# vga-group/tauray

Hardware: AMD Instinct MI355X
Metric: Mray/s (closest-hit + shadow rays traced) @1920x1080, 4 bounces, 1 spp (higher is better)
Workload: dtype f32

## Files before the change

### include/trhip.h

```cpp
#ifndef TRHIP_H
#define TRHIP_H
#include <stddef.h>
#include <stdint.h>

#ifdef __cplusplus
extern "C" {
#endif

typedef struct trhip_device trhip_device;
typedef struct trhip_pt trhip_pt;

int trhip_device_create(int hip_device, trhip_device** out);
void trhip_device_destroy(trhip_device* dev);
const char* trhip_last_error(void);
int trhip_malloc(trhip_device* dev, size_t bytes, void** out);
int trhip_free(trhip_device* dev, void* ptr);
int trhip_upload(trhip_device* dev, void* dst_dev, const void* src_host, size_t bytes, void* stream);
int trhip_download(trhip_device* dev, void* dst_host, const void* src_dev, size_t bytes, void* stream);
int trhip_memset(trhip_device* dev, void* dst_dev, int value, size_t bytes, void* stream);
int trhip_sync(trhip_device* dev, void* stream);
int trhip_stream_create(trhip_device* dev, void** stream_out);
int trhip_stream_destroy(trhip_device* dev, void* stream);
int trhip_stream_wait(trhip_device* dev, void* stream, void* on);
int trhip_stream_pipe_class(trhip_device* dev, void* stream, int32_t* pipe_class_out);
// ... 121 lines not shown
    int32_t mis_mode;
    float russian_roulette_delta;
    float indirect_clamping;
    float regularization_gamma;
    int32_t depth_of_field;
    float nee_point, nee_directional, nee_envmap, nee_triangles;
    int32_t bounce_mode;
    int32_t tri_light_mode;
    int32_t hide_lights;
    int32_t use_white_albedo_on_first_bounce;
    int32_t transparent_background;
    int32_t pre_transformed_vertices;
} trhip_pt_options;

typedef struct trhip_distribution {
    uint32_t size_x, size_y;
    int32_t strategy;
    uint32_t index, count;
    uint32_t primary;
} trhip_distribution;

typedef struct trhip_counters {
    uint64_t closest_rays, shadow_rays;
    uint64_t node_visits, tri_tests, alpha_tests, surface_hits;
    uint64_t stack_overflows;
} trhip_counters;

typedef struct trhip_timings {
    float path_tracing_ms;
    float trace_closest_ms, trace_shadow_ms, shade_ms, raygen_ms, resolve_ms;
    uint32_t trace_closest_launches, trace_shadow_launches, shade_launches, frames;
} trhip_timings;

int trhip_pt_create(trhip_device* dev, const trhip_pt_options* opt, trhip_pt** out);
int trhip_direct_create(trhip_device* dev, const trhip_pt_options* opt, trhip_pt** out);
void trhip_pt_destroy(trhip_pt* pt);
int trhip_pt_set_distribution(trhip_pt* pt, const trhip_distribution* dist);
int trhip_pt_reset_accumulation(trhip_pt* pt, int reset_sample_counter);
int trhip_pt_set_frame_counter(trhip_pt* pt, uint32_t frame_counter);
int trhip_pt_set_frame_batch(trhip_pt* pt, uint32_t frames);
int trhip_pt_set_lanes(trhip_pt* pt, int lanes);
int trhip_pt_set_frame_slots(trhip_pt* pt, int slots);
int trhip_pt_get_lane_pipes(trhip_pt* pt, int32_t* lanes_out, int32_t pipe_classes_out[4]);
int trhip_pt_set_shard(trhip_pt* pt, uint32_t viewport_base, uint32_t viewport_stride, uint32_t sample_base, uint32_t sample_stride);
int trhip_pt_render(trhip_pt* pt, void* color_dev, uint32_t target_w, uint32_t target_h, uint32_t viewports, void* stream);
typedef struct trhip_pt_targets {
    void* color;
    void* diffuse;
    void* reflection;
    void* albedo;
    void* material;
    void* normal;
    void* pos;
    void* instance_id;
    void* screen_motion;
} trhip_pt_targets;
int trhip_pt_render_targets(trhip_pt* pt, const trhip_pt_targets* targets, uint32_t target_w, uint32_t target_h, uint32_t viewports, void* stream);
int trhip_pt_set_shading_arithmetic(trhip_pt* pt, int ieee);
int trhip_pt_set_specialization(trhip_pt* pt, int enable);
int trhip_pt_precompile(const trhip_pt_options* opt, int shade_tris, int ieee, int count_work, const char* arch);
typedef struct trhip_program_info { int32_t kind, ieee; uint64_t identity; char key[240]; } trhip_program_info;
int trhip_pt_get_program(trhip_pt* pt, trhip_program_info* out);
uint64_t trhip_build_id(void);
const char* trhip_kernel_cache_dir(void);
int trhip_pt_set_profiling(trhip_pt* pt, int count_work, int detailed_timing);
int trhip_pt_get_counters(trhip_pt* pt, trhip_counters* out);
int trhip_pt_reset_counters(trhip_pt* pt);
int trhip_pt_get_timings(trhip_pt* pt, trhip_timings* out);
typedef struct trhip_phase_counters {
    uint64_t lane_node_phases, lane_tri_phases, quad_node_phases, quad_tri_phases;
    uint64_t lane_node_phases_le16, lane_node_visits_le16;
    uint64_t lane_node_phase_hist[8];
    uint64_t closest_node_visits;
} trhip_phase_counters;
int trhip_pt_get_phase_counters(trhip_pt* pt, trhip_phase_counters* out);
typedef struct trhip_light_counters { uint64_t sphere_tests, node_visits, walk_fallbacks; } trhip_light_counters;
int trhip_pt_get_light_counters(trhip_pt* pt, trhip_light_counters* out);
int trhip_pt_get_max_stack_depth(trhip_pt* pt, uint32_t* out);
#define TRHIP_TERMINAL_QUERY_AUTO 0
#define TRHIP_TERMINAL_QUERY_OFF 1
int trhip_pt_set_terminal_query(trhip_pt* pt, int mode);
typedef struct trhip_terminal_counters { uint64_t blocked_rays, fallback_rays; uint32_t in_effect, emitter_triangles, threshold, pad; } trhip_terminal_counters;
int trhip_pt_get_terminal_counters(trhip_pt* pt, trhip_terminal_counters* out);
int trhip_calibrate_valu(trhip_device* dev, float* ginst_per_s);
int trhip_calibrate_l1(trhip_device* dev, float* gaccesses_per_s);

int trhip_feature_render(trhip_device* dev, int feature, const trhip_distribution* dist, int projection,
                         uint32_t viewport, float min_ray_dist, const float default_value[4],
                         void* color_dev, uint32_t target_w, uint32_t target_h, void* stream);

int trhip_trace_closest(trhip_device* dev, uint32_t n, const void* rays_dev, const void* seeds_dev,
                        int include_lights, void* hits_dev, void* stream);
int trhip_trace_terminal(trhip_device* dev, uint32_t n, const void* rays_dev, const void* seeds_dev, const void* fallback_dev,
                         void* hits_dev, void* stream);
int trhip_trace_shadow(trhip_device* dev, uint32_t n, const void* rays_dev, void* visibility_dev, void* stream);

int trhip_stitch(trhip_device* dev, const trhip_distribution* partial_dist, const void* partial_dev,
                 uint32_t partial_w, uint32_t partial_h, void* primary_dev, uint32_t viewports,
                 float blend_ratio, void* stream);
int trhip_stitch_batch(trhip_device* dev, uint32_t count, const trhip_distribution* partial_dists, const void* const* partials_dev,
                       const uint32_t* partial_ws, const uint32_t* partial_hs, void* primary_dev, uint32_t viewports,
                       float blend_ratio, void* stream);

typedef struct trhip_tonemap_info {
    int32_t op;
    float exposure, gamma;
    int32_t alpha_grid_background;
} trhip_tonemap_info;
int trhip_tonemap(trhip_device* dev, const void* in_dev, void* out_dev, uint32_t width, uint32_t height,
                  uint32_t layers, const trhip_tonemap_info* info, void* stream);
int trhip_pt_set_fused_tonemap(trhip_pt* pt, void* display_dev, const trhip_tonemap_info* info);

typedef struct trhip_bmfr trhip_bmfr;
#define TRHIP_BMFR_DIFFUSE_ONLY 0
#define TRHIP_BMFR_DIFFUSE_SPECULAR 1
typedef struct trhip_bmfr_options {
    int32_t settings;
    float noise_amount;
} trhip_bmfr_options;
typedef struct trhip_bmfr_features {
    void* color;
    void* diffuse;
    void* albedo;
    void* normal;
    void* pos;
    void* screen_motion;
    void* instance_id;
} trhip_bmfr_features;
typedef struct trhip_bmfr_timings {
    float preprocess_ms, fit_ms, weighted_sum_ms, accumulate_output_ms, total_ms;
    uint32_t frames;
} trhip_bmfr_timings;
int trhip_bmfr_create(trhip_device* dev, const trhip_bmfr_options* opt, uint32_t width, uint32_t height, uint32_t layers, trhip_bmfr** out);
void trhip_bmfr_destroy(trhip_bmfr* bmfr);
int trhip_bmfr_run(trhip_bmfr* bmfr, const trhip_bmfr_features* features, uint32_t frame_counter, void* stream);
int trhip_bmfr_reset_history(trhip_bmfr* bmfr);
int trhip_bmfr_get_timings(trhip_bmfr* bmfr, trhip_bmfr_timings* out);
int trhip_bmfr_fit_blocks(trhip_device* dev, uint32_t blocks, uint32_t channels, const float* matrix_dev, float* weights_dev, void* stream);
#define TRHIP_BMFR_NOISY_DIFFUSE 0
#define TRHIP_BMFR_NOISY_SPECULAR 1
#define TRHIP_BMFR_FILTERED_DIFFUSE 2
#define TRHIP_BMFR_FILTERED_SPECULAR 3
#define TRHIP_BMFR_FEATURE_ROWS 4
#define TRHIP_BMFR_WEIGHTS 5
#define TRHIP_BMFR_MIN_MAX 6
#define TRHIP_BMFR_ACCEPT_BITS 7
#define TRHIP_BMFR_BLOCK_OFFSETS 8
#define TRHIP_BMFR_PREVIOUS_NORMAL 9
#define TRHIP_BMFR_PREVIOUS_POS 10
int trhip_bmfr_download(trhip_bmfr* bmfr, int which, void* host, size_t bytes);

typedef struct trhip_gbuffer_targets {
    void* normal;
    void* pos;
    void* instance_id;
} trhip_gbuffer_targets;
int trhip_gbuffer_render(trhip_device* dev, int projection, const uint32_t* viewports, uint32_t count, float min_ray_dist,
                         const trhip_gbuffer_targets* targets, uint32_t width, uint32_t height, void* stream);
typedef struct trhip_reprojection_images {
    void* color;
    void* normal;
    void* pos;
    void* instance_id;
    void* screen_motion;
} trhip_reprojection_images;
typedef struct trhip_reprojection_timings { float total_ms; uint32_t frames; } trhip_reprojection_timings;
// ... 22 lines not shown
    float alpha;
    float gamma;
    int32_t edge_dilation, anti_shimmer;
    uint32_t base_camera_index;
    int32_t projection;
} trhip_taa_options;
typedef struct trhip_taa_images {
    const void* src;
    void* dst;
    const void* screen_motion;
    const void* pos;
    const void* instance_id;
} trhip_taa_images;
typedef struct trhip_taa_timings {
    float total_ms;
    uint32_t frames;
    char name[64];
} trhip_taa_timings;
int trhip_taa_create(trhip_device* dev, const trhip_taa_options* opt, uint32_t width, uint32_t height, uint32_t layers, trhip_taa** out);
void trhip_taa_destroy(trhip_taa* stage);
int trhip_taa_run(trhip_taa* stage, const trhip_taa_images* images, void* stream);
int trhip_taa_reset_history(trhip_taa* stage);
int trhip_taa_get_timings(trhip_taa* stage, trhip_taa_timings* out);
#define TRHIP_TAA_HISTORY 0
#define TRHIP_TAA_DECISIONS 1
int trhip_taa_download(trhip_taa* stage, int which, void* host, size_t bytes);

typedef struct trhip_lkg trhip_lkg;
typedef struct trhip_lkg_options {
    uint32_t viewport_count;
    float pitch, tilt, center;
    int32_t invert;
    int32_t record_view_indices;
} trhip_lkg_options;
typedef struct trhip_lkg_timings {
    float total_ms;
    uint32_t frames;
    char name[64];
} trhip_lkg_timings;
int trhip_lkg_create(trhip_device* dev, const trhip_lkg_options* opt, uint32_t view_w, uint32_t view_h, uint32_t out_w, uint32_t out_h, trhip_lkg** out);
void trhip_lkg_destroy(trhip_lkg* stage);
int trhip_lkg_run(trhip_lkg* stage, const void* src, void* dst, void* dst_rgba8, void* stream);
int trhip_lkg_get_timings(trhip_lkg* stage, trhip_lkg_timings* out);
#define TRHIP_LKG_VIEW_INDICES 0
int trhip_lkg_download(trhip_lkg* stage, int which, void* host, size_t bytes);

typedef struct trhip_sh trhip_sh;
typedef struct trhip_sh_options {
    int32_t order;
    uint32_t resolution[3];
    uint32_t samples_per_probe;
    float temporal_ratio;
} trhip_sh_options;
typedef struct trhip_sh_grid_data {
    float transform[16], normal_transform[16];
    uint32_t grid_size[3];
    float mix_ratio;
    float cell_scale[3];
    float rotation_x, rotation_y;
} trhip_sh_grid_data;
typedef struct trhip_sh_timings {
    float total_ms;
    uint32_t frames;
    char name[64];
    float raygen_ms, trace_closest_ms, trace_shadow_ms, shade_ms, project_ms;
} trhip_sh_timings;
int trhip_sh_create(trhip_device* dev, const trhip_pt_options* path, const trhip_sh_options* opt, trhip_sh** out);
void trhip_sh_destroy(trhip_sh* stage);
int trhip_sh_set_transform(trhip_sh* stage, const float transform[16], const float scaling[3]);
int trhip_sh_set_frame_counter(trhip_sh* stage, uint32_t frame_counter);
int trhip_sh_reset_history(trhip_sh* stage);
int trhip_sh_set_lanes(trhip_sh* stage, int lanes);
int trhip_sh_set_batch_probes(trhip_sh* stage, uint32_t probes);
int trhip_sh_set_shading_arithmetic(trhip_sh* stage, int ieee);
int trhip_sh_get_grid_data(trhip_sh* stage, trhip_sh_grid_data* out);
int trhip_sh_pack_grid_data(const float transform[16], const float scaling[3], const uint32_t resolution[3], uint32_t samples_per_probe,
                            uint32_t frame_counter, uint32_t history_length, float temporal_ratio, trhip_sh_grid_data* out);
int trhip_sh_render(trhip_sh* stage, void* stream);
int trhip_sh_get_grids(trhip_sh* stage, void** grid_dev, void** grid_half_dev);
#define TRHIP_SH_GRID 0
#define TRHIP_SH_GRID_HALF 1
int trhip_sh_download(trhip_sh* stage, int which, void* host, size_t bytes);
int trhip_sh_get_counters(trhip_sh* stage, trhip_counters* out);
int trhip_sh_get_timings(trhip_sh* stage, trhip_sh_timings* out);
int trhip_sh_set_profiling(trhip_sh* stage, int count_work, int detailed_timing);
int trhip_sh_reset_counters(trhip_sh* stage);

typedef struct trhip_dshgi trhip_dshgi;
typedef struct trhip_dshgi_options {
    int32_t order;
    int32_t use_probe_visibility;
    int32_t record_surface;
} trhip_dshgi_options;
typedef struct trhip_dshgi_grid {
    const void* grid_half_dev;
    uint32_t resolution[3];
    float transform[16];
    float scaling[3];
} trhip_dshgi_grid;
typedef struct trhip_dshgi_surface {
    float pos[3], smooth_normal[3], mapped_normal[3], view[3], albedo[4];
    float metallic, roughness, f0, transmittance;
    int32_t grid, instance_id;
} trhip_dshgi_surface;
typedef struct trhip_dshgi_timings {
    float total_ms;
    uint32_t frames;
    char name[64];
} trhip_dshgi_timings;
int trhip_dshgi_create(trhip_device* dev, const trhip_dshgi_options* opt, uint32_t width, uint32_t height, uint32_t layers, trhip_dshgi** out);
void trhip_dshgi_destroy(trhip_dshgi* stage);
int trhip_dshgi_set_grids(trhip_dshgi* stage, const trhip_dshgi_grid* grids, uint32_t count);
int trhip_dshgi_set_instance_grids(trhip_dshgi* stage, const int32_t* instance_grids, uint32_t count);
int trhip_dshgi_set_brdf_integration(trhip_dshgi* stage, const void* table_dev, uint32_t w, uint32_t h);
int trhip_dshgi_render(trhip_dshgi* stage, int projection, const uint32_t* viewports, uint32_t count, float min_ray_dist,
                       const void* direct_color_dev, void* out_color_dev, void* stream);
int trhip_dshgi_get_timings(trhip_dshgi* stage, trhip_dshgi_timings* out);
#define TRHIP_DSHGI_INDIRECT 0
#define TRHIP_DSHGI_SURFACE 1
int trhip_dshgi_download(trhip_dshgi* stage, int which, void* host, size_t bytes);
int trhip_dshgi_pick_grid(const float* transforms, const float* scalings, const uint32_t* resolutions, const float* radii, uint32_t count,
                          const float position[3], int32_t* index);
int trhip_brdf_integration_generate(trhip_device* dev, uint32_t size, uint32_t samples, void* out_dev_rg32f, void* stream);

typedef struct trhip_restir_di trhip_restir_di;
typedef struct trhip_restir_di_options {
    uint32_t candidates;
    uint32_t spatial_samples;
    float search_radius;
    float max_confidence;
    int32_t temporal_reuse;
    float min_ray_dist;
    uint32_t rng_seed;
    int32_t record;
} trhip_restir_di_options;
typedef struct trhip_restir_di_surface {
    float pos[3]; int32_t instance_id;
    float mapped_normal[3], metallic;
    float flat_normal[3], roughness;
    float view[3], transmittance;
    float albedo[4];
    float emission[3], f0;
    float ior_in, ior_out, pad[2];
} trhip_restir_di_surface;
typedef struct trhip_restir_di_reservoir {
    float uc_weight, target_function; uint32_t light; float confidence;
    float light_data[2]; uint32_t pad[2];
} trhip_restir_di_reservoir;
typedef struct trhip_restir_di_candidate {
    uint32_t light; float light_data[2], pdf;
    float contribution[3], visibility;
    float weight, draw; uint32_t selected, pad;
} trhip_restir_di_candidate;
typedef struct trhip_restir_di_temporal {
    int32_t px, py; uint32_t reuse; float prev_confidence;
    float target, weight, draw; uint32_t selected;
} trhip_restir_di_temporal;
typedef struct trhip_restir_di_spatial {
    int32_t px, py; uint32_t good, selected;
    float target_n, visibility_n, jacobian_n, m;
    float wi, draw, target_c, visibility_c;
    float jacobian_c, mis_canonical, pad[2];
} trhip_restir_di_spatial;
typedef struct trhip_restir_di_final {
    float contribution[3], visibility;
    float canonical_m, wi, draw; uint32_t selected;
// ... 70 lines not shown
```

### tauray_amd/_lib.py

```python
from __future__ import annotations

import ctypes as C
import os

os.environ.setdefault("GPU_MAX_HW_QUEUES", "8")
os.environ.setdefault("HSA_ENABLE_IPC_MODE_LEGACY", "0")

_HERE = os.path.dirname(os.path.abspath(__file__))
LIB_PATH = os.environ.get("TRHIP_LIB", os.path.join(_HERE, "libtrhip.so"))


class TrhipError(RuntimeError):
    pass


class SceneDescC(C.Structure):
    _fields_ = [
        ("instances", C.c_void_p), ("spans", C.c_void_p), ("instance_count", C.c_uint32),
        ("vertices", C.c_void_p), ("vertex_count", C.c_uint32),
        ("indices", C.c_void_p), ("index_count", C.c_uint32),
        ("point_lights", C.c_void_p), ("point_light_count", C.c_uint32),
        ("directional_lights", C.c_void_p), ("directional_light_count", C.c_uint32),
        ("texture_infos", C.c_void_p), ("texture_count", C.c_uint32), ("texels", C.c_void_p),
        ("envmap", C.c_void_p), ("envmap_width", C.c_uint32), ("envmap_height", C.c_uint32),
        ("alias_table", C.c_void_p), ("environment_factor", C.c_float * 4),
        ("cameras", C.c_void_p), ("camera_count", C.c_uint32),
        ("non_opaque", C.c_void_p), ("gather_emissive_triangles", C.c_uint32)]


class AccelInfoC(C.Structure):
    _fields_ = [("triangle_count", C.c_uint32), ("node_count", C.c_uint32), ("tri_light_count", C.c_uint32),
                ("build_ms", C.c_float), ("bounds_min", C.c_float * 3), ("bounds_max", C.c_float * 3),
                ("node_bytes", C.c_uint32), ("leaf_count", C.c_uint32)]


class AccelLayoutC(C.Structure):
    _fields_ = [("strategy", C.c_int32), ("blas_count", C.c_uint32), ("tlas_leaf_count", C.c_uint32), ("blas_updated", C.c_uint32),
                ("node_bytes", C.c_uint64), ("record_bytes", C.c_uint64), ("blas_ms", C.c_float), ("tlas_ms", C.c_float)]


AS_ALL_MERGED, AS_PER_MESH, AS_STATIC_MERGED_DYNAMIC_PER_MESH = 0, 1, 2


class LightAccelInfoC(C.Structure):
    _fields_ = [("requested", C.c_int32), ("in_effect", C.c_int32), ("sphere_lights", C.c_uint32), ("tree_lights", C.c_uint32),
                ("node_count", C.c_uint32), ("auto_threshold", C.c_uint32), ("tree_bytes", C.c_uint64), ("last_ms", C.c_float),
                ("last_was_refit", C.c_int32)]


class LightCountersC(C.Structure):
    _fields_ = [("sphere_tests", C.c_uint64), ("node_visits", C.c_uint64), ("walk_fallbacks", C.c_uint64)]


LIGHT_ACCEL_AUTO, LIGHT_ACCEL_LOOP, LIGHT_ACCEL_TREE = 0, 1, 2


class TerminalCountersC(C.Structure):
    _fields_ = [("blocked_rays", C.c_uint64), ("fallback_rays", C.c_uint64), ("in_effect", C.c_uint32), ("emitter_triangles", C.c_uint32),
                ("threshold", C.c_uint32), ("pad", C.c_uint32)]


TERMINAL_QUERY_AUTO, TERMINAL_QUERY_OFF = 0, 1
HIT_BLOCKED = -2


class PtOptionsC(C.Structure):
    _fields_ = [
        ("max_bounces", C.c_int32), ("min_ray_dist", C.c_float), ("rng_seed", C.c_uint32), ("sampler", C.c_int32),
        ("samples_per_pixel", C.c_int32), ("samples_per_pass", C.c_int32), ("projection", C.c_int32),
        ("film", C.c_int32), ("film_radius", C.c_float), ("mis_mode", C.c_int32),
        ("russian_roulette_delta", C.c_float), ("indirect_clamping", C.c_float), ("regularization_gamma", C.c_float),
        ("depth_of_field", C.c_int32), ("nee_point", C.c_float), ("nee_directional", C.c_float),
        ("nee_envmap", C.c_float), ("nee_triangles", C.c_float), ("bounce_mode", C.c_int32),
        ("tri_light_mode", C.c_int32), ("hide_lights", C.c_int32), ("use_white_albedo_on_first_bounce", C.c_int32),
        ("transparent_background", C.c_int32), ("pre_transformed_vertices", C.c_int32)]


class DistributionC(C.Structure):
    _fields_ = [("size_x", C.c_uint32), ("size_y", C.c_uint32), ("strategy", C.c_int32),
                ("index", C.c_uint32), ("count", C.c_uint32), ("primary", C.c_uint32)]


class CountersC(C.Structure):
    _fields_ = [(n, C.c_uint64) for n in ("closest_rays", "shadow_rays", "node_visits", "tri_tests", "alpha_tests",
                                          "surface_hits", "stack_overflows")]


class TimingsC(C.Structure):
    _fields_ = ([(n, C.c_float) for n in ("path_tracing_ms", "trace_closest_ms", "trace_shadow_ms", "shade_ms", "raygen_ms", "resolve_ms")]
                + [(n, C.c_uint32) for n in ("trace_closest_launches", "trace_shadow_launches", "shade_launches", "frames")])


class PhaseCountersC(C.Structure):
    _fields_ = ([(n, C.c_uint64) for n in ("lane_node_phases", "lane_tri_phases", "quad_node_phases", "quad_tri_phases",
                                           "lane_node_phases_le16", "lane_node_visits_le16")] + [("lane_node_phase_hist", C.c_uint64 * 8),
                                                                                                 ("closest_node_visits", C.c_uint64)])


class ProgramInfoC(C.Structure):
    _fields_ = [("kind", C.c_int32), ("ieee", C.c_int32), ("identity", C.c_uint64), ("key", C.c_char * 240)]


class PtTargetsC(C.Structure):
    _fields_ = [(n, C.c_void_p) for n in ("color", "diffuse", "reflection", "albedo", "material", "normal", "pos", "instance_id", "screen_motion")]


class TonemapInfoC(C.Structure):
    _fields_ = [("op", C.c_int32), ("exposure", C.c_float), ("gamma", C.c_float), ("alpha_grid_background", C.c_int32)]


class BmfrOptionsC(C.Structure):
    _fields_ = [("settings", C.c_int32), ("noise_amount", C.c_float)]


class BmfrFeaturesC(C.Structure):
    _fields_ = [(n, C.c_void_p) for n in ("color", "diffuse", "albedo", "normal", "pos", "screen_motion", "instance_id")]


class BmfrTimingsC(C.Structure):
    _fields_ = ([(n, C.c_float) for n in ("preprocess_ms", "fit_ms", "weighted_sum_ms", "accumulate_output_ms", "total_ms")]
                + [("frames", C.c_uint32)])


BMFR_DIFFUSE_ONLY, BMFR_DIFFUSE_SPECULAR = 0, 1
(BMFR_NOISY_DIFFUSE, BMFR_NOISY_SPECULAR, BMFR_FILTERED_DIFFUSE, BMFR_FILTERED_SPECULAR, BMFR_FEATURE_ROWS, BMFR_WEIGHTS, BMFR_MIN_MAX,
 BMFR_ACCEPT_BITS, BMFR_BLOCK_OFFSETS, BMFR_PREVIOUS_NORMAL, BMFR_PREVIOUS_POS) = range(11)


class GbufferTargetsC(C.Structure):
    _fields_ = [(n, C.c_void_p) for n in ("normal", "pos", "instance_id")]


class ReprojectionImagesC(C.Structure):
    _fields_ = [(n, C.c_void_p) for n in ("color", "normal", "pos", "instance_id", "screen_motion")]


class ReprojectionTimingsC(C.Structure):
    _fields_ = [("total_ms", C.c_float), ("frames", C.c_uint32)]


REPROJECTION_DECISIONS, REPROJECTION_PREVIOUS_COLOR, REPROJECTION_PREVIOUS_NORMAL, REPROJECTION_PREVIOUS_POS = range(4)
REPROJ_NONE, REPROJ_REPROJECTED, REPROJ_SKY_COPY = 0, 1, 2
REPROJECTION_RECORD = [("kind", "u1"), ("slot", "u1"), ("bits", "u1"), ("zero", "u1"), ("ox", "<i2"), ("oy", "<i2")]


class TaaOptionsC(C.Structure):
# ... 63 lines not shown
    _fields_ = [("candidates", C.c_uint32), ("spatial_samples", C.c_uint32), ("search_radius", C.c_float), ("max_confidence", C.c_float),
                ("temporal_reuse", C.c_int32), ("min_ray_dist", C.c_float), ("rng_seed", C.c_uint32), ("record", C.c_int32)]


class RestirDiTimingsC(C.Structure):
    _fields_ = [("canonical_ms", C.c_float), ("spatial_ms", C.c_float), ("total_ms", C.c_float), ("frames", C.c_uint32),
                ("canonical_name", C.c_char * 64), ("spatial_name", C.c_char * 64)]


(RESTIR_DI_SURFACE, RESTIR_DI_CANONICAL, RESTIR_DI_HISTORY, RESTIR_DI_CANDIDATES, RESTIR_DI_TEMPORAL, RESTIR_DI_SPATIAL,
 RESTIR_DI_FINAL) = range(7)
RESTIR_DI_NULL_INDEX = (1 << 30) - 1
RESTIR_DI_SURFACE_DTYPE = [("pos", "<f4", 3), ("instance_id", "<i4"), ("mapped_normal", "<f4", 3), ("metallic", "<f4"), ("flat_normal", "<f4", 3),
                           ("roughness", "<f4"), ("view", "<f4", 3), ("transmittance", "<f4"), ("albedo", "<f4", 4), ("emission", "<f4", 3),
                           ("f0", "<f4"), ("ior_in", "<f4"), ("ior_out", "<f4"), ("pad", "<f4", 2)]
RESTIR_DI_RESERVOIR_DTYPE = [("uc_weight", "<f4"), ("target_function", "<f4"), ("light", "<u4"), ("confidence", "<f4"), ("light_data", "<f4", 2),
                             ("pad", "<u4", 2)]
RESTIR_DI_CANDIDATE_DTYPE = [("light", "<u4"), ("light_data", "<f4", 2), ("pdf", "<f4"), ("contribution", "<f4", 3), ("visibility", "<f4"),
                             ("weight", "<f4"), ("draw", "<f4"), ("selected", "<u4"), ("pad", "<u4")]
RESTIR_DI_TEMPORAL_DTYPE = [("px", "<i4"), ("py", "<i4"), ("reuse", "<u4"), ("prev_confidence", "<f4"), ("target", "<f4"), ("weight", "<f4"),
                            ("draw", "<f4"), ("selected", "<u4")]
RESTIR_DI_SPATIAL_DTYPE = [("px", "<i4"), ("py", "<i4"), ("good", "<u4"), ("selected", "<u4"), ("target_n", "<f4"), ("visibility_n", "<f4"),
                           ("jacobian_n", "<f4"), ("m", "<f4"), ("wi", "<f4"), ("draw", "<f4"), ("target_c", "<f4"), ("visibility_c", "<f4"),
                           ("jacobian_c", "<f4"), ("mis_canonical", "<f4"), ("pad", "<f4", 2)]
RESTIR_DI_FINAL_DTYPE = [("contribution", "<f4", 3), ("visibility", "<f4"), ("canonical_m", "<f4"), ("wi", "<f4"), ("draw", "<f4"),
                         ("selected", "<u4")]


class RestirGiOptionsC(C.Structure):
    _fields_ = [("spatial_samples", C.c_uint32), ("search_radius", C.c_float), ("max_confidence", C.c_float), ("temporal_reuse", C.c_int32),
                ("min_ray_dist", C.c_float), ("rng_seed", C.c_uint32), ("record", C.c_int32)]


class RestirGiTimingsC(C.Structure):
    _fields_ = [("initial_ms", C.c_float), ("temporal_ms", C.c_float), ("spatial_ms", C.c_float), ("total_ms", C.c_float), ("frames", C.c_uint32),
                ("initial_name", C.c_char * 64), ("temporal_name", C.c_char * 64), ("spatial_name", C.c_char * 64)]


(RESTIR_GI_SURFACE, RESTIR_GI_CANONICAL, RESTIR_GI_HISTORY, RESTIR_GI_INITIAL, RESTIR_GI_SECONDARY, RESTIR_GI_LIGHT, RESTIR_GI_TEMPORAL,
 RESTIR_GI_SPATIAL, RESTIR_GI_FINAL) = range(9)
RESTIR_GI_SAMPLER_W = 0x80000000
RESTIR_GI_RESERVOIR_DTYPE = [("x_s", "<f4", 3), ("uc_weight", "<f4"), ("n_s", "<f4", 3), ("target_function", "<f4"), ("L_o", "<f4", 3),
                             ("confidence", "<f4")]
RESTIR_GI_INITIAL_DTYPE = [("draw", "<f4", 2), ("pdf", "<f4"), ("traced", "<u4"), ("dir", "<f4", 3), ("t", "<f4"), ("instance_id", "<i4"),
                           ("primitive_id", "<i4"), ("u", "<f4"), ("v", "<f4"), ("light_draw", "<u4", 4), ("L_o", "<f4", 3), ("target", "<f4"),
                           ("weight", "<f4"), ("sel_draw", "<f4"), ("selected", "<u4"), ("pad", "<u4")]


_vp, _u32, _i, _f = C.c_void_p, C.c_uint32, C.c_int, C.c_float
SYMBOLS = {
    "trhip_image_decode": (_i, [_vp, C.c_size_t, C.POINTER(_u32), C.POINTER(_u32), C.POINTER(_u32), C.POINTER(C.POINTER(C.c_uint8))]),
    "trhip_image_free": (None, [C.POINTER(C.c_uint8)]),
    "trhip_exr_decode": (_i, [_vp, C.c_size_t, C.POINTER(_u32), C.POINTER(_u32), C.POINTER(_u32), C.POINTER(C.POINTER(C.c_float))]),
    "trhip_exr_encode": (_i, [_vp, _u32, _u32, _i, _i, _i, C.POINTER(C.POINTER(C.c_uint8)), C.POINTER(C.c_size_t)]),
    "trhip_exr_free": (None, [_vp]),
    "trhip_device_create": (_i, [_i, C.POINTER(_vp)]),
    "trhip_device_destroy": (None, [_vp]),
    "trhip_last_error": (C.c_char_p, []),
    "trhip_malloc": (_i, [_vp, C.c_size_t, C.POINTER(_vp)]),
    "trhip_image_decode_texels": (_i, [C.c_char_p, C.c_size_t, C.POINTER(C.c_uint32), C.POINTER(C.c_uint32), C.POINTER(C.c_uint32), C.POINTER(C.c_uint32), C.POINTER(C.POINTER(C.c_uint8))]),
    "trhip_free": (_i, [_vp, _vp]),
    "trhip_upload": (_i, [_vp, _vp, _vp, C.c_size_t, _vp]),
    "trhip_download": (_i, [_vp, _vp, _vp, C.c_size_t, _vp]),
    "trhip_memset": (_i, [_vp, _vp, _i, C.c_size_t, _vp]),
    "trhip_sync": (_i, [_vp, _vp]),
    "trhip_copy_peer": (_i, [_vp, _vp, _vp, _vp, C.c_size_t, _vp]),
    "trhip_scene_upload": (_i, [_vp, C.POINTER(SceneDescC)]),
    "trhip_scene_update_cameras": (_i, [_vp, _vp, _u32]),
    "trhip_scene_set_previous_cameras": (_i, [_vp, _vp, _u32]),
    "trhip_scene_update_instances": (_i, [_vp, _vp, _u32]),
    "trhip_scene_build_accel": (_i, [_vp, C.POINTER(AccelInfoC)]),
    "trhip_scene_refit_accel": (_i, [_vp, C.POINTER(AccelInfoC)]),
    "trhip_pt_set_frame_batch": (_i, [_vp, C.c_uint32]),
    "trhip_scene_update_lights": (_i, [_vp, _vp, C.c_uint32, _vp, C.c_uint32]),
    "trhip_scene_set_build_mode": (_i, [_vp, _i]),
    "trhip_scene_set_accel_strategy": (_i, [_vp, _i]),
    "trhip_scene_set_dynamic_instances": (_i, [_vp, _vp, _u32]),
    "trhip_scene_get_accel_layout": (_i, [_vp, C.POINTER(AccelLayoutC)]),
    "trhip_scene_set_light_accel": (_i, [_vp, _i]),
    "trhip_scene_get_light_accel": (_i, [_vp, C.POINTER(LightAccelInfoC)]),
    "trhip_pt_get_light_counters": (_i, [_vp, C.POINTER(LightCountersC)]),
    "trhip_pt_set_terminal_query": (_i, [_vp, _i]),
    "trhip_pt_get_terminal_counters": (_i, [_vp, C.POINTER(TerminalCountersC)]),
    "trhip_pt_get_max_stack_depth": (_i, [_vp, C.POINTER(C.c_uint32)]),
    "trhip_trace_terminal": (_i, [_vp, _u32, _vp, _vp, _vp, _vp, _vp]),
    "trhip_stitch_batch": (_i, [_vp, _u32, _vp, _vp, _vp, _vp, _vp, _u32, C.c_float, _vp]),
    "trhip_stream_create": (_i, [_vp, C.POINTER(C.c_void_p)]),
    "trhip_stream_destroy": (_i, [_vp, _vp]),
    "trhip_stream_pipe_class": (_i, [_vp, _vp, C.POINTER(C.c_int32)]),
    "trhip_device_get_info": (_i, [_vp, _vp]),
    "trhip_build_id": (C.c_uint64, []),
    "trhip_stream_wait": (_i, [_vp, _vp, _vp]),
    "trhip_stream_wait_peer": (_i, [_vp, _vp, _vp, _vp]),
    "trhip_pt_set_frame_counter": (_i, [_vp, _u32]),
    "trhip_pt_set_lanes": (_i, [_vp, C.c_int]),
    "trhip_pt_set_frame_slots": (_i, [_vp, C.c_int]),
    "trhip_pt_set_fused_tonemap": (_i, [_vp, _vp, _vp]),
    "trhip_pt_get_lane_pipes": (_i, [_vp, C.POINTER(C.c_int32), C.POINTER(C.c_int32)]),
    "trhip_pt_set_shading_arithmetic": (_i, [_vp, C.c_int]),
    "trhip_pt_set_specialization": (_i, [_vp, C.c_int]),
    "trhip_pt_precompile": (_i, [C.POINTER(PtOptionsC), C.c_int, C.c_int, C.c_int, C.c_char_p]),
    "trhip_kernel_cache_dir": (C.c_char_p, []),
    "trhip_pt_set_shard": (_i, [_vp, _u32, _u32, _u32, _u32]),
    "trhip_scene_set_skin": (_i, [_vp, _u32, _vp, _vp, _u32]),
    "trhip_scene_skin": (_i, [_vp, _u32, _vp, _u32]),
    "trhip_scene_set_morph_targets": (_i, [_vp, _u32, _u32, _vp, _vp, _vp, _u32]),
    "trhip_scene_morph": (_i, [_vp, _u32, _vp, _u32]),
    "trhip_scene_get_vertices": (_i, [_vp, _u32, _vp, _u32]),
    "trhip_scene_set_deformation_motion": (_i, [_vp, _i]),
    "trhip_scene_latch_positions": (_i, [_vp]),
    "trhip_scene_get_previous_positions": (_i, [_vp, _u32, _vp, _u32]),
    "trhip_scene_get_tri_lights": (_i, [_vp, _vp, _u32]),
    "trhip_pt_create": (_i, [_vp, C.POINTER(PtOptionsC), C.POINTER(_vp)]),
    "trhip_direct_create": (_i, [_vp, C.POINTER(PtOptionsC), C.POINTER(_vp)]),
    "trhip_pt_destroy": (None, [_vp]),
    "trhip_pt_set_distribution": (_i, [_vp, C.POINTER(DistributionC)]),
    "trhip_pt_reset_accumulation": (_i, [_vp, _i]),
    "trhip_pt_render": (_i, [_vp, _vp, _u32, _u32, _u32, _vp]),
    "trhip_pt_render_targets": (_i, [_vp, C.POINTER(PtTargetsC), _u32, _u32, _u32, _vp]),
    "trhip_pt_set_profiling": (_i, [_vp, _i, _i]),
    "trhip_pt_get_counters": (_i, [_vp, C.POINTER(CountersC)]),
    "trhip_pt_reset_counters": (_i, [_vp]),
    "trhip_pt_get_timings": (_i, [_vp, C.POINTER(TimingsC)]),
    "trhip_pt_get_phase_counters": (_i, [_vp, C.POINTER(PhaseCountersC)]),
    "trhip_pt_get_program": (_i, [_vp, C.POINTER(ProgramInfoC)]),
    "trhip_calibrate_valu": (_i, [_vp, C.POINTER(C.c_float)]),
    "trhip_calibrate_l1": (_i, [_vp, C.POINTER(C.c_float)]),
    "trhip_feature_render": (_i, [_vp, _i, C.POINTER(DistributionC), _i, _u32, _f, C.POINTER(_f), _vp, _u32, _u32, _vp]),
    "trhip_trace_closest": (_i, [_vp, _u32, _vp, _vp, _i, _vp, _vp]),
    "trhip_trace_shadow": (_i, [_vp, _u32, _vp, _vp, _vp]),
    "trhip_stitch": (_i, [_vp, C.POINTER(DistributionC), _vp, _u32, _u32, _vp, _u32, _f, _vp]),
    "trhip_tonemap": (_i, [_vp, _vp, _vp, _u32, _u32, _u32, C.POINTER(TonemapInfoC), _vp]),
    "trhip_bmfr_create": (_i, [_vp, C.POINTER(BmfrOptionsC), _u32, _u32, _u32, C.POINTER(_vp)]),
    "trhip_bmfr_destroy": (None, [_vp]),
    "trhip_bmfr_run": (_i, [_vp, C.POINTER(BmfrFeaturesC), _u32, _vp]),
    "trhip_bmfr_reset_history": (_i, [_vp]),
    "trhip_bmfr_get_timings": (_i, [_vp, C.POINTER(BmfrTimingsC)]),
    "trhip_bmfr_fit_blocks": (_i, [_vp, _u32, _u32, _vp, _vp, _vp]),
    "trhip_bmfr_download": (_i, [_vp, _i, _vp, C.c_size_t]),
    "trhip_gbuffer_render": (_i, [_vp, _i, C.POINTER(_u32), _u32, _f, C.POINTER(GbufferTargetsC), _u32, _u32, _vp]),
    "trhip_spatial_reprojection_create": (_i, [_vp, _u32, _u32, _u32, C.POINTER(_u32), _u32, C.POINTER(_f), C.POINTER(_vp)]),
    "trhip_spatial_reprojection_destroy": (None, [_vp]),
    "trhip_spatial_reprojection_run": (_i, [_vp, C.POINTER(ReprojectionImagesC), C.POINTER(ReprojectionImagesC), _vp, _vp]),
    "trhip_spatial_reprojection_get_timings": (_i, [_vp, C.POINTER(ReprojectionTimingsC)]),
    "trhip_spatial_reprojection_download": (_i, [_vp, _i, _vp, C.c_size_t]),
    "trhip_temporal_reprojection_create": (_i, [_vp, _u32, _u32, _u32, _f, C.POINTER(_vp)]),
    "trhip_temporal_reprojection_destroy": (None, [_vp]),
    "trhip_temporal_reprojection_run": (_i, [_vp, C.POINTER(ReprojectionImagesC), _vp]),
    "trhip_temporal_reprojection_reset_history": (_i, [_vp]),
    "trhip_temporal_reprojection_get_timings": (_i, [_vp, C.POINTER(ReprojectionTimingsC)]),
    "trhip_temporal_reprojection_download": (_i, [_vp, _i, _vp, C.c_size_t]),
    "trhip_taa_create": (_i, [_vp, C.POINTER(TaaOptionsC), _u32, _u32, _u32, C.POINTER(_vp)]),
    "trhip_taa_destroy": (None, [_vp]),
    "trhip_taa_run": (_i, [_vp, C.POINTER(TaaImagesC), _vp]),
    "trhip_taa_reset_history": (_i, [_vp]),
    "trhip_taa_get_timings": (_i, [_vp, C.POINTER(TaaTimingsC)]),
    "trhip_taa_download": (_i, [_vp, _i, _vp, C.c_size_t]),
    "trhip_lkg_create": (_i, [_vp, C.POINTER(LkgOptionsC), _u32, _u32, _u32, _u32, C.POINTER(_vp)]),
    "trhip_lkg_destroy": (None, [_vp]),
    "trhip_lkg_run": (_i, [_vp, _vp, _vp, _vp, _vp]),
    "trhip_lkg_get_timings": (_i, [_vp, C.POINTER(LkgTimingsC)]),
    "trhip_lkg_download": (_i, [_vp, _i, _vp, C.c_size_t]),
    "trhip_sh_create": (_i, [_vp, C.POINTER(PtOptionsC), C.POINTER(ShOptionsC), C.POINTER(_vp)]),
    "trhip_sh_destroy": (None, [_vp]),
    "trhip_sh_set_transform": (_i, [_vp, C.POINTER(_f), C.POINTER(_f)]),
    "trhip_sh_set_frame_counter": (_i, [_vp, _u32]),
    "trhip_sh_reset_history": (_i, [_vp]),
    "trhip_sh_set_lanes": (_i, [_vp, _i]),
    "trhip_sh_set_batch_probes": (_i, [_vp, _u32]),
    "trhip_sh_set_shading_arithmetic": (_i, [_vp, _i]),
    "trhip_sh_get_grid_data": (_i, [_vp, C.POINTER(ShGridDataC)]),
    "trhip_sh_pack_grid_data": (_i, [C.POINTER(_f), C.POINTER(_f), C.POINTER(_u32), _u32, _u32, _u32, _f, C.POINTER(ShGridDataC)]),
    "trhip_sh_render": (_i, [_vp, _vp]),
    "trhip_sh_get_grids": (_i, [_vp, C.POINTER(_vp), C.POINTER(_vp)]),
    "trhip_sh_download": (_i, [_vp, _i, _vp, C.c_size_t]),
    "trhip_sh_get_counters": (_i, [_vp, C.POINTER(CountersC)]),
    "trhip_sh_get_timings": (_i, [_vp, C.POINTER(ShTimingsC)]),
    "trhip_sh_set_profiling": (_i, [_vp, _i, _i]),
    "trhip_sh_reset_counters": (_i, [_vp]),
    "trhip_dshgi_create": (_i, [_vp, C.POINTER(DshgiOptionsC), _u32, _u32, _u32, C.POINTER(_vp)]),
    "trhip_dshgi_destroy": (None, [_vp]),
    "trhip_dshgi_set_grids": (_i, [_vp, C.POINTER(DshgiGridC), _u32]),
    "trhip_dshgi_set_instance_grids": (_i, [_vp, C.POINTER(C.c_int32), _u32]),
    "trhip_dshgi_set_brdf_integration": (_i, [_vp, _vp, _u32, _u32]),
    "trhip_dshgi_render": (_i, [_vp, _i, C.POINTER(_u32), _u32, _f, _vp, _vp, _vp]),
    "trhip_dshgi_get_timings": (_i, [_vp, C.POINTER(DshgiTimingsC)]),
    "trhip_dshgi_download": (_i, [_vp, _i, _vp, C.c_size_t]),
    "trhip_dshgi_pick_grid": (_i, [C.POINTER(_f), C.POINTER(_f), C.POINTER(_u32), C.POINTER(_f), _u32, C.POINTER(_f), C.POINTER(C.c_int32)]),
    "trhip_brdf_integration_generate": (_i, [_vp, _u32, _u32, _vp, _vp]),
    "trhip_restir_di_create": (_i, [_vp, C.POINTER(RestirDiOptionsC), _u32, _u32, _u32, C.POINTER(_vp)]),
    "trhip_restir_di_destroy": (None, [_vp]),
    "trhip_restir_di_reset": (_i, [_vp]),
    "trhip_restir_di_render": (_i, [_vp, _i, C.POINTER(_u32), _u32, _vp, _vp]),
    "trhip_restir_di_get_timings": (_i, [_vp, C.POINTER(RestirDiTimingsC)]),
    "trhip_restir_di_download": (_i, [_vp, _i, _vp, C.c_size_t]),
    "trhip_restir_gi_create": (_i, [_vp, C.POINTER(RestirGiOptionsC), _u32, _u32, _u32, C.POINTER(_vp)]),
    "trhip_restir_gi_destroy": (None, [_vp]),
    "trhip_restir_gi_reset": (_i, [_vp]),
    "trhip_restir_gi_render": (_i, [_vp, _i, C.POINTER(_u32), _u32, _vp, _vp, _vp]),
    "trhip_restir_gi_get_timings": (_i, [_vp, C.POINTER(RestirGiTimingsC)]),
    "trhip_restir_gi_download": (_i, [_vp, _i, _vp, C.c_size_t]),
}

_LIB = None


def lib():
    global _LIB
    if _LIB is None:
        if not os.path.exists(LIB_PATH):
            raise TrhipError(f"{LIB_PATH} is missing: build it with `make -C tauray_amd/csrc` (or __graft_entry__.build())")
        L = C.CDLL(LIB_PATH)
        for name, (res, args) in SYMBOLS.items():
            try:
                fn = getattr(L, name)
            except AttributeError:
                if "TRHIP_LIB" not in os.environ:
                    raise
                continue
            fn.restype = res
            fn.argtypes = args
        _LIB = L
    return _LIB


def check(rc):
    if rc != 0:
        raise TrhipError(lib().trhip_last_error().decode("utf-8", "replace"))
```

### tauray_amd/csrc/api.hip

```cpp
#include <cstdlib>
#include <cstring>
#include <mutex>
#include <string>
#include <vector>

#include "pt.h"
#include "trace.h"
#include "first_hit.h"
#include "trace_quad.h"
#include "specialize.h"
#include "tonemap.h"
#include "../../include/tauray_image.hh"
#include "../../include/tauray_exr.hh"

namespace tr {

static thread_local std::string g_error;
int set_error(const std::string& msg) { g_error = msg; return 1; }

#define HIPCHK(x) do { hipError_t e_ = (x); if (e_ != hipSuccess) return set_error(std::string(#x) + ": " + hipGetErrorString(e_)); } while (0)

namespace {

constexpr int KB = TR_BLOCK;
// ... 842 lines not shown
}
int trhip_pt_set_frame_batch(trhip_pt* pt, uint32_t frames) {
    if (!pt) return set_error("null trhip_pt");
    if (frames == 0) return set_error("trhip_pt_set_frame_batch: at least one frame per launch");
    pt->stage->frame_batch = frames;
    return 0;
}
int trhip_pt_set_lanes(trhip_pt* pt, int lanes) {
    if (!pt) return set_error("null trhip_pt");
    if (lanes < 0) return set_error("trhip_pt_set_lanes: lanes must be >= 0");
    pt->stage->lanes = lanes;
    return 0;
}
int trhip_pt_set_frame_slots(trhip_pt* pt, int slots) {
    if (!pt) return set_error("null trhip_pt");
    if (slots < 0) return set_error("trhip_pt_set_frame_slots: slots must be >= 0");
    pt->stage->frame_slots = slots;
    return 0;
}
int trhip_pt_set_fused_tonemap(trhip_pt* pt, void* display_dev, const trhip_tonemap_info* info) {
    if (!pt) return set_error("null trhip_pt");
    if (display_dev && !info) return set_error("trhip_pt_set_fused_tonemap: null info");
    if (display_dev && pt->stage->direct) return set_error("trhip_pt_set_fused_tonemap: the direct stage resolves its samples in a kernel of its own; run trhip_tonemap");
    pt->stage->tm_display = display_dev;
    if (info) { pt->stage->tm_info = *info; if (info->op == 0) pt->stage->tm_info.gamma = 1.0f; }
    return 0;
}
int trhip_pt_get_lane_pipes(trhip_pt* pt, int32_t* lanes_out, int32_t pipe_classes_out[4]) {
    if (!pt || !lanes_out || !pipe_classes_out) return set_error("trhip_pt_get_lane_pipes: null argument");
    *lanes_out = pt->stage->last_lanes;
    for (int l = 0; l < 4; ++l) pipe_classes_out[l] = l < pt->stage->last_lanes ? pt->stage->last_lane_pipes[l] : -1;
    return 0;
}
int trhip_pt_set_shading_arithmetic(trhip_pt* pt, int ieee) {
    if (!pt) return set_error("null trhip_pt");
    pt->stage->ieee_shading = ieee ? 1 : 0;
    return 0;
}
int trhip_pt_set_specialization(trhip_pt* pt, int enable) {
    if (!pt) return set_error("null trhip_pt");
    pt->stage->specialize = enable ? 1 : 0;
    return 0;
}
int trhip_pt_precompile(const trhip_pt_options* opt, int shade_tris, int ieee, int count_work, const char* arch) {
    if (!opt) return set_error("trhip_pt_precompile: null options");
    if (is_cli_default_set(*opt) && shade_tris) return 0;
    SpecRequest rq{*opt, shade_tris != 0 && !opt->pre_transformed_vertices, ieee != 0, count_work != 0, SPEC_SHADE, false};
    std::string why;
    for (int program : {SPEC_SHADE, SPEC_RAYGEN}) {
        rq.program = program;
        if (spec_precompile(rq, arch, &why)) return set_error("trhip_pt_precompile: " + why);
    }
    return 0;
}
const char* trhip_kernel_cache_dir(void) {
    static const std::string dir = spec_cache_dir();
    return dir.c_str();
}
int trhip_pt_set_profiling(trhip_pt* pt, int count_work, int detailed_timing) {
    if (!pt) return set_error("null trhip_pt");
    pt->stage->count_work = count_work; pt->stage->detailed_timing = detailed_timing;
    return 0;
}
int trhip_pt_get_counters(trhip_pt* pt, trhip_counters* out) { if (!pt) return set_error("null trhip_pt"); DEVCHK(pt->dev); return pt->stage->get_counters(out, pt->stage->last_stream); }
int trhip_pt_get_light_counters(trhip_pt* pt, trhip_light_counters* out) {
    if (!pt) return set_error("null trhip_pt");
    if (!out) return set_error("trhip_pt_get_light_counters: null output");
    DEVCHK(pt->dev);
    return pt->stage->get_light_counters(out, pt->stage->last_stream);
}
int trhip_pt_get_max_stack_depth(trhip_pt* pt, uint32_t* out) {
    if (!pt) return set_error("null trhip_pt");
    if (!out) return set_error("trhip_pt_get_max_stack_depth: null output");
    DEVCHK(pt->dev);
    return pt->stage->get_max_stack_depth(out, pt->stage->last_stream);
}
int trhip_pt_set_terminal_query(trhip_pt* pt, int mode) {
    if (!pt) return set_error("null trhip_pt");
    if (mode != TRHIP_TERMINAL_QUERY_AUTO && mode != TRHIP_TERMINAL_QUERY_OFF)
        return set_error("trhip_pt_set_terminal_query: unknown mode " + std::to_string(mode) + " (0 auto, 1 off)");
    pt->stage->terminal_query = mode;
    return 0;
}
int trhip_pt_get_terminal_counters(trhip_pt* pt, trhip_terminal_counters* out) {
    if (!pt) return set_error("null trhip_pt");
    if (!out) return set_error("trhip_pt_get_terminal_counters: null output");
    DEVCHK(pt->dev);
    if (pt->stage->terminal_query_in_effect() < 0) return set_error("trhip_pt_get_terminal_counters: TRHIP_TERMINAL_QUERY is not auto or off");
    return pt->stage->get_terminal_counters(out, pt->stage->last_stream);
}
int trhip_pt_reset_counters(trhip_pt* pt) { if (!pt) return set_error("null trhip_pt"); DEVCHK(pt->dev); HIPCHK(hipStreamSynchronize(pt->stage->last_stream)); return pt->stage->reset_counters(); }
int trhip_pt_get_timings(trhip_pt* pt, trhip_timings* out) { if (!pt) return set_error("null trhip_pt"); DEVCHK(pt->dev); return pt->stage->get_timings(out); }
int trhip_pt_get_program(trhip_pt* pt, trhip_program_info* out) { if (!pt) return set_error("null trhip_pt"); if (!out) return set_error("trhip_pt_get_program: null out"); DEVCHK(pt->dev); return pt->stage->get_program(out); }
int trhip_pt_get_phase_counters(trhip_pt* pt, trhip_phase_counters* out) { if (!pt) return set_error("null trhip_pt"); DEVCHK(pt->dev); return pt->stage->get_phase_counters(out, pt->stage->last_stream); }

int trhip_calibrate_valu(trhip_device* dev, float* ginst_per_s) {
    DEVCHK(dev);
    if (!ginst_per_s) return set_error("trhip_calibrate_valu: null out");
    int cus = 256;
    HIPCHK(hipDeviceGetAttribute(&cus, hipDeviceAttributeMultiprocessorCount, dev->hip_device));
    const int blocks = cus * 8, iters = 4096;
    hipEvent_t a, b;
    HIPCHK(hipEventCreate(&a)); HIPCHK(hipEventCreate(&b));
    float best = 0.0f;
    for (int rep = 0; rep < 4; ++rep) {
        HIPCHK(hipEventRecord(a, nullptr));
        hipLaunchKernelGGL(k_calibrate_fma, dim3(blocks), dim3(KB), 0, nullptr, reinterpret_cast<float*>(dev->overflow_flag), iters, 1.0001f, 0.5f);
        HIPCHK(hipEventRecord(b, nullptr));
        HIPCHK(hipEventSynchronize(b));
        float ms = 0;
        HIPCHK(hipEventElapsedTime(&ms, a, b));
        const float g = (float)((double)blocks * (KB / 64) * (double)iters * 64.0 / ((double)ms * 1e6));
        if (rep > 0 && g > best) best = g;
    }
    (void)hipEventDestroy(a); (void)hipEventDestroy(b);
    *ginst_per_s = best;
    return 0;
}

int trhip_calibrate_l1(trhip_device* dev, float* gaccesses_per_s) {
    DEVCHK(dev);
    if (!gaccesses_per_s) return set_error("trhip_calibrate_l1: null out");
    int cus = 256;
    HIPCHK(hipDeviceGetAttribute(&cus, hipDeviceAttributeMultiprocessorCount, dev->hip_device));
    const int blocks = cus * 4, iters = 400;
    char* buf = nullptr;
    HIPCHK(hipMalloc(&buf, 16384 + 64));
    HIPCHK(hipMemset(buf, 0, 16384 + 64));
    hipEvent_t a, b;
    HIPCHK(hipEventCreate(&a)); HIPCHK(hipEventCreate(&b));
    float best = 0.0f;
    for (int rep = 0; rep < 4; ++rep) {
        HIPCHK(hipEventRecord(a, nullptr));
        hipLaunchKernelGGL(k_calibrate_l1, dim3(blocks), dim3(KB), 0, nullptr, buf, iters, reinterpret_cast<float*>(dev->overflow_flag));
        HIPCHK(hipEventRecord(b, nullptr));
        HIPCHK(hipEventSynchronize(b));
        float ms = 0;
        HIPCHK(hipEventElapsedTime(&ms, a, b));
        const float g = (float)((double)blocks * (KB / 64) * (double)iters * 8.0 * 64.0 / ((double)ms * 1e6));
        if (rep > 0 && g > best) best = g;
    }
    (void)hipEventDestroy(a); (void)hipEventDestroy(b);
    (void)hipFree(buf);
    *gaccesses_per_s = best;
    return 0;
}

static LaunchCtx make_launch(const trhip_distribution& d) {
    LaunchCtx L{};
    uint lw, lh;
    get_ray_count(d, lw, lh);
    L.size_x = d.size_x; L.size_y = d.size_y; L.strategy = d.strategy; L.index = d.index; L.primary = d.primary;
    L.count = d.count;
    if (d.strategy == 2) { uint n = d.size_x * d.size_y, b = 31; while ((n >> b) < 128 && b > 0) b--; L.count = b; }
    L.launch_w = lw; L.launch_h = lh;
    return L;
}

int trhip_feature_render(trhip_device* dev, int feature, const trhip_distribution* dist, int projection, uint32_t viewport,
                         float min_ray_dist, const float default_value[4], void* color_dev, uint32_t target_w, uint32_t target_h, void* stream) {
    DEVCHK(dev);
    if (!dev->scene.accel_built) return set_error("trhip_feature_render: call trhip_scene_build_accel first");
    if (viewport >= dev->scene.camera_count) return set_error("trhip_feature_render: viewport out of range");
    LaunchCtx L = make_launch(*dist);
    size_t n = (size_t)L.launch_w * L.launch_h;
    if (n == 0) return 0;
// ... 97 lines not shown
```

### tauray_amd/csrc/path_tracer.hip

```cpp
#include <cstdio>
#include <cstdlib>
#include <type_traits>
#include <vector>

#include "pt_kernels.h"
#include "resolve_kernel.h"
#include "specialize.h"
#include "build_id.inc"

namespace tr {

namespace {

#ifndef TR_CLOSEST_WAVES
#define TR_CLOSEST_WAVES 6
#endif
#ifndef TR_SHADOW_WAVES
#define TR_SHADOW_WAVES 8
#endif
#ifndef TR_TERMINAL_WAVES
#define TR_TERMINAL_WAVES TR_CLOSEST_WAVES
#endif
#ifndef TR_CLOSEST_WAVES_2L
#define TR_CLOSEST_WAVES_2L 5
#endif
#ifndef TR_SHADOW_WAVES_2L
#define TR_SHADOW_WAVES_2L 6
#endif

template <bool COUNT, bool SOLO, bool WIDE = true, bool TWO_LEVEL = false>
__global__ __launch_bounds__(KB, TWO_LEVEL ? TR_CLOSEST_WAVES_2L : TR_CLOSEST_WAVES) void k_trace_closest(SceneView sv, PtParams P, PathBuffers pb, int bounce, const uint* queue,
                                                      uint* bc) {
    if (!WIDE) sv.wide_textures = 0;
    __shared__ int s_stack_rows[TR_STACK_WORDS];
    int* const s_stack = s_stack_rows + TR_STACK_ROW0;
    __shared__ int s_owner[(KB / 64) * TR_OWNER_WORDS];
    TL(__shared__ uint s_tl[(KB / 64) * TL_WORDS]; for (uint i = threadIdx.x; i < (KB / 64) * TL_WORDS; i += KB) s_tl[i] = 0; __syncthreads();)
    const QuadCtx qc = make_quad_ctx(s_stack, s_owner, pb TL(, s_tl));
    const uint n = queue ? bc[BC_QUEUE] : P.n_ids;
    TraceStats st = {};
    uint rays = 0, max_vis = 0;
    int overflow = 0;
    const uint wave_id = (blockIdx.x * KB + threadIdx.x) >> 6, n_waves = (gridDim.x * KB) >> 6;
    bool first = true;
    while (true) {
        uint base = 0;
        if (first) base = wave_id * 64u;
        else {
            if (n <= n_waves * 64u) break;
            if ((threadIdx.x & 63) == 0) base = n_waves * 64u + atomicAdd(&bc[BC_CUR_CLOSEST], 64u);
            base = __shfl(base, 0);
        }
        first = false;
        if (base >= n) break;
        closest_lane<COUNT, TWO_LEVEL>(sv, P, pb, bounce, queue, base + (threadIdx.x & 63), n, s_stack + threadIdx.x, qc, st, overflow, max_vis, rays);
    }
    flush_trace_counters<COUNT>(P, pb, overflow, 1000 + bounce, rays, 0u, st, max_vis);
    TL(__syncthreads(); for (uint i = threadIdx.x; i < (KB / 64) * TL_WORDS; i += KB) if (s_tl[i]) atomicAdd(&g_timeline[i % TL_WORDS], (unsigned long long)s_tl[i]);)
}

template <bool COUNT, bool WIDE = true, bool TWO_LEVEL = false>
__global__ __launch_bounds__(KB, TWO_LEVEL ? TR_SHADOW_WAVES_2L : TR_SHADOW_WAVES) void k_trace_shadow(SceneView sv, PtParams P, PathBuffers pb, uint* bc) {
    if (!WIDE) sv.wide_textures = 0;
    __shared__ int s_stack_rows[TR_STACK_WORDS];
    int* const s_stack = s_stack_rows + TR_STACK_ROW0;
    __shared__ int s_owner[(KB / 64) * TR_OWNER_WORDS];
    const QuadCtx qc = make_quad_ctx(s_stack, s_owner, pb);
    const uint n = bc[BC_SHADOW];
    TraceStats st = {};
    uint rays = 0;
    int overflow = 0;
    const uint wave_id = (blockIdx.x * KB + threadIdx.x) >> 6, n_waves = (gridDim.x * KB) >> 6;
    bool first = true;
    while (true) {
        uint base = 0;
        if (first) base = wave_id * 64u;
        else {
            if (n <= n_waves * 64u) break;
            if ((threadIdx.x & 63) == 0) base = n_waves * 64u + atomicAdd(&bc[BC_CUR_SHADOW], 64u);
            base = __shfl(base, 0);
        }
        first = false;
        if (base >= n) break;
        shadow_lane<COUNT, TWO_LEVEL>(sv, P, pb, base + (threadIdx.x & 63), n, s_stack + threadIdx.x, qc, st, overflow, rays);
    }
    flush_trace_counters<COUNT>(P, pb, overflow, 2000, 0u, rays, st, 0u);
}

template <bool WIDE, bool TWO_LEVEL = false>
__global__ __launch_bounds__(KB, TWO_LEVEL ? TR_CLOSEST_WAVES_2L : TR_CLOSEST_WAVES) void k_trace_fused(SceneView sv, PtParams P, PathBuffers pb, int bounce, const uint* queue,
                                                                      uint* bc, uint* bc_prev) {
    if (!WIDE) sv.wide_textures = 0;
    __shared__ int s_stack_rows[TR_STACK_WORDS];
    int* const s_stack = s_stack_rows + TR_STACK_ROW0;
    __shared__ int s_owner[(KB / 64) * TR_OWNER_WORDS];
    const QuadCtx qc = make_quad_ctx(s_stack, s_owner, pb);
    const uint nc = bc[BC_QUEUE], ns = bc_prev[BC_SHADOW];
    const uint chunks_c = (nc + 63u) >> 6, total = chunks_c + ((ns + 63u) >> 6);
    TraceStats st = {};
    uint closest_rays = 0, shadow_rays = 0, max_vis = 0;
    int overflow = 0;
    const uint wave_id = (blockIdx.x * KB + threadIdx.x) >> 6, n_waves = (gridDim.x * KB) >> 6;
    bool first = true;
    while (true) {
        uint g = 0;
        if (first) g = wave_id;
        else {
            if (total <= n_waves) break;
            if ((threadIdx.x & 63) == 0) g = n_waves + atomicAdd(&bc[BC_CUR_CLOSEST], 1u);
            g = __shfl(g, 0);
        }
        first = false;
        if (g >= total) break;
        const uint lane = threadIdx.x & 63;
        if (g < chunks_c) closest_lane<false, TWO_LEVEL>(sv, P, pb, bounce, queue, (g << 6) + lane, nc, s_stack + threadIdx.x, qc, st, overflow, max_vis, closest_rays);
        else shadow_lane<false, TWO_LEVEL>(sv, P, pb, ((g - chunks_c) << 6) + lane, ns, s_stack + threadIdx.x, qc, st, overflow, shadow_rays);
    }
    flush_trace_counters<false>(P, pb, overflow, 3000 + bounce, closest_rays, shadow_rays, st, max_vis);
}


template <bool COUNT, bool SOLO, bool WIDE = true>
__global__ __launch_bounds__(KB, TR_TERMINAL_WAVES) void k_trace_closest_terminal(SceneView sv, PtParams P, PathBuffers pb, int bounce, const uint* queue, uint* bc,
                                                                                   uint* next_queue) {
    if (!WIDE) sv.wide_textures = 0;
    __shared__ int s_stack_rows[TR_STACK_WORDS];
    int* const s_stack = s_stack_rows + TR_STACK_ROW0;
    __shared__ int s_owner[(KB / 64) * TR_OWNER_WORDS];
    TL(__shared__ uint s_tl[(KB / 64) * TL_WORDS]; for (uint i = threadIdx.x; i < (KB / 64) * TL_WORDS; i += KB) s_tl[i] = 0; __syncthreads();)
    const QuadCtx qc = make_quad_ctx(s_stack, s_owner, pb TL(, s_tl));
    const uint n = bc[BC_QUEUE];
    TerminalCounts tc = {0u, 0u};
    TraceStats st = {};
    uint rays = 0, max_vis = 0;
    int overflow = 0;
    const uint wave_id = (blockIdx.x * KB + threadIdx.x) >> 6, n_waves = (gridDim.x * KB) >> 6;
    bool first = true;
    while (true) {
        uint base = 0;
        if (first) base = wave_id * 64u;
        else {
            if (n <= n_waves * 64u) break;
// ... 263 lines not shown
    flush_trace_counters<COUNT>(P, pb, overflow, 5000, 0u, rays, st, 0u);
}

__global__ void k_direct_next_sample(uint* bc) { bc[BC_SHADOW] = 0; }

__global__ __launch_bounds__(KB) void k_resolve_direct(PtParams P, PathBuffers pb) {
    uint i = blockIdx.x * KB + threadIdx.x;
    if (i >= P.n_ids) return;
    i += P.id_offset;
    uint lx, ly, lz;
    launch_coord(P.L, i, lx, ly, lz);
    int wx, wy;
    if (!get_write_pixel_pos(P.L, lx, ly, wx, wy)) return;
    if ((uint)wx >= P.target_w || (uint)wy >= P.target_h) return;
    const float spp = (float)P.opt.samples_per_pass;
    const size_t idx = ((size_t)lz * P.target_h + (uint)wy) * P.target_w + (uint)wx;
    const uint prev_samples = P.samples_accumulated + P.previous_samples;
    const float keep = prev_samples != 0 ? (float)prev_samples / (float)((uint)P.opt.samples_per_pass + prev_samples) : 0.0f;
    auto accumulate = [&](void* image, f4 value) {
        f4* target = reinterpret_cast<f4*>(image);
        if (prev_samples != 0) value = mix4(value, target[idx], keep);
        target[idx] = value;
    };
    if (P.T.color) { const f4 c = pb.first_emis[i]; accumulate(P.T.color, F4(c.x / spp, c.y / spp, c.z / spp, P.opt.transparent_background ? c.w : 1.0f)); }
    if (P.T.diffuse) { const f4 d = pb.diffuse[i]; accumulate(P.T.diffuse, F4(d.x / spp, d.y / spp, d.z / spp, d.w / spp)); }
    if (P.T.reflection) accumulate(P.T.reflection, pb.reflection[i]);
}

uint calculate_shuffled_strips_b(uint sx, uint sy) {
    uint n = sx * sy, b = 31;
    while ((n >> b) < 128 && b > 0) b--;
    return b;
}

#define HIPCHK(x) do { hipError_t e_ = (x); if (e_ != hipSuccess) return set_error(std::string(#x) + ": " + hipGetErrorString(e_)); } while (0)

}

void launch_shade_fast(bool cli, bool count, bool last, uint blocks, hipStream_t stream, const SceneView& sv, const PtParams& P, const PathBuffers& pb, int bounce,
                       const uint* queue, uint* bc, uint* next_queue);
void launch_sh_raygen(uint blocks, hipStream_t stream, const PtParams& P, const PathBuffers& pb, const ShProbeBatch& batch);

void get_ray_count(const trhip_distribution& d, uint& w, uint& h) {
    if (d.strategy == 0) { w = d.size_x; h = d.size_y; }
    else if (d.strategy == 1) { w = d.size_x; h = (d.size_y - d.index + d.count - 1) / d.count; }
    else { w = d.count; h = 1; }
}

#ifndef TR_PT_LANES
#define TR_PT_LANES 4
#endif
constexpr int PT_LANES = TR_PT_LANES;
static uint trace_grid_cap() {
    static const uint cap = getenv("TRHIP_GRID_BLOCKS") ? (uint)atoi(getenv("TRHIP_GRID_BLOCKS")) : 256u * 8u;
    return cap;
}
static uint fused_grid_factor() {
    static const uint f = getenv("TRHIP_FUSED_GRID_FACTOR") ? (uint)std::max(1, atoi(getenv("TRHIP_FUSED_GRID_FACTOR"))) : 2u;
    return f;
}
static size_t qspill_words(size_t blocks) { return std::max<size_t>(blocks, 1) * (KB / 64) * 16u * TR_QSPILL; }
struct TimedSpan { int kind; hipEvent_t a, b; };
enum { T_CLOSEST = 0, T_SHADOW = 1, T_SHADE = 2, T_RAYGEN = 3, T_RESOLVE = 4, T_KINDS = 5 };

struct PtStage::Impl {
    PathBuffers pb{};
    size_t capacity = 0;
    float prev_frame_ms = 0.0f;
    size_t qspill_lane_words = 0;
    size_t qspill_regions = 0;
    hipEvent_t ev[2]{};
    bool ev_init = false;
    std::vector<hipEvent_t> pool;
    std::vector<TimedSpan> pending;
    float acc_ms[T_KINDS] = {0, 0, 0, 0, 0};
    uint acc_launches[T_KINDS] = {0, 0, 0, 0, 0};
    uint frames = 0;
    int main_cls = -1, main_tries = 0;
    hipStream_t side = nullptr;
    hipEvent_t ev_fork = nullptr, ev_join = nullptr;
    hipStream_t lane_stream[PT_LANES] = {};
    hipEvent_t lane_join[PT_LANES] = {};
    hipEvent_t pass_done[PT_LANES] = {};
    hipEvent_t get_event() {
        if (!pool.empty()) { hipEvent_t e = pool.back(); pool.pop_back(); return e; }
        hipEvent_t e; (void)hipEventCreateWithFlags(&e, hipEventDisableSystemFence); return e;
    }
};

PtStage::PtStage(DeviceScene* scene, const trhip_pt_options& o) : scene(scene), opt(o), impl(new Impl()) {
    dist = trhip_distribution{0, 0, 0, 0, 1, 1};
}

PtStage::~PtStage() {
    free_buffers();
    if (impl->pb.counters) (void)hipFree(impl->pb.counters);
    if (impl->pb.bounce) (void)hipFree(impl->pb.bounce);
    if (impl->pb.qspill) (void)hipFree(impl->pb.qspill);
    if (impl->ev_init) for (auto& e : impl->ev) (void)hipEventDestroy(e);
    for (auto& sp : impl->pending) { (void)hipEventDestroy(sp.a); (void)hipEventDestroy(sp.b); }
    for (auto& e : impl->pool) (void)hipEventDestroy(e);
    if (impl->side) { stream_pool_release(impl->side); (void)hipEventDestroy(impl->ev_fork); (void)hipEventDestroy(impl->ev_join); }
    for (int l = 2; l < PT_LANES; ++l) if (impl->lane_stream[l]) { stream_pool_release(impl->lane_stream[l]); (void)hipEventDestroy(impl->lane_join[l]); }
    for (auto& e : impl->pass_done) if (e) (void)hipEventDestroy(e);
    delete impl;
}

void PtStage::free_buffers() {
    PathBuffers& pb = impl->pb;
    void* ptrs[] = {pb.org_pdf, pb.dir_reg, pb.atten_alpha, pb.diffuse, pb.reflection, pb.plobes, pb.first_mat, pb.first_emis, pb.rng, pb.misc, pb.hit,
                    pb.sum_color, pb.sum_diffuse, pb.sum_reflection, pb.sh_org_tmax, pb.sh_dir_id, pb.sh_contrib, pb.sh_lobes, pb.sh_cweight, pb.queue[0], pb.queue[1], pb.first_dist};
    for (void* p : ptrs) if (p) (void)hipFree(p);
    uint *counters = pb.counters, *bounce = pb.bounce;
    int* qspill = pb.qspill;
    pb = PathBuffers{};
    pb.counters = counters; pb.bounce = bounce; pb.qspill = qspill;
    impl->capacity = 0;
}

int PtStage::ensure_buffers(size_t n, bool lobe_sums) {
    PathBuffers& pb = impl->pb;
    if (!pb.counters) {
        HIPCHK(hipMalloc(&pb.counters, PT_LANES * CNT_WORDS * sizeof(uint)));
        HIPCHK(hipMemset(pb.counters, 0, PT_LANES * CNT_WORDS * sizeof(uint)));
        HIPCHK(hipMalloc(&pb.bounce, (size_t)PT_LANES * BC_STRIDE * ((size_t)opt.max_bounces + 2u) * sizeof(uint)));
    }
    if (!impl->ev_init) { for (auto& e : impl->ev) HIPCHK(hipEventCreateWithFlags(&e, hipEventDisableSystemFence)); impl->ev_init = true; }
    if (n <= impl->capacity && (!lobe_sums || pb.sum_diffuse)) return 0;
    free_buffers();
    HIPCHK(hipMalloc(&pb.org_pdf, n * 16)); HIPCHK(hipMalloc(&pb.dir_reg, n * 16)); HIPCHK(hipMalloc(&pb.atten_alpha, n * 16));
    HIPCHK(hipMalloc(&pb.diffuse, n * 16)); HIPCHK(hipMalloc(&pb.reflection, n * 16)); HIPCHK(hipMalloc(&pb.plobes, n * 8));
    HIPCHK(hipMalloc(&pb.first_mat, n * 16)); HIPCHK(hipMalloc(&pb.first_emis, n * 16)); HIPCHK(hipMalloc(&pb.rng, n * 16));
    HIPCHK(hipMalloc(&pb.misc, n * 16)); HIPCHK(hipMalloc(&pb.hit, n * 16)); HIPCHK(hipMalloc(&pb.sum_color, n * 16));
    HIPCHK(hipMalloc(&pb.sh_org_tmax, n * 16)); HIPCHK(hipMalloc(&pb.sh_dir_id, n * 16)); HIPCHK(hipMalloc(&pb.sh_contrib, n * 16));
    HIPCHK(hipMalloc(&pb.sh_lobes, n * 8));
    if (lobe_sums) { HIPCHK(hipMalloc(&pb.sum_diffuse, n * 16)); HIPCHK(hipMalloc(&pb.sum_reflection, n * 16)); }
    HIPCHK(hipMalloc(&pb.queue[0], n * 4)); HIPCHK(hipMalloc(&pb.queue[1], n * 4));
    impl->capacity = n;
    return 0;
}

static int ensure_qspill(PathBuffers& pb, size_t& lane_words, size_t& regions_have, size_t regions, size_t blocks) {
    const size_t words = qspill_words(blocks);
    if (words <= lane_words && regions <= regions_have) return 0;
    if (pb.qspill) HIPCHK(hipFree(pb.qspill));
    pb.qspill = nullptr;
    lane_words = std::max(lane_words, words);
    regions_have = std::max(regions_have, regions);
    HIPCHK(hipMalloc(&pb.qspill, regions_have * lane_words * sizeof(int)));
    return 0;
}

PtStage::Program PtStage::choose_program() {
    static const bool cli_instances = !(getenv("TRHIP_SHADE_CLI") && atoi(getenv("TRHIP_SHADE_CLI")) == 0);
    const bool wide = scene->wide_textures != 0;
    const bool cli_set = cli_instances && !probe_mode && is_cli_default_set(opt) && scene->shade_tris != nullptr && !wide;
    static const bool shade_fast_env = !(getenv("TRHIP_SHADE_FAST") && atoi(getenv("TRHIP_SHADE_FAST")) == 0);
    const bool shade_fast = ieee_shading < 0 ? shade_fast_env : ieee_shading == 0;
    static const bool specialize_env = !(getenv("TRHIP_SPECIALIZE") && atoi(getenv("TRHIP_SPECIALIZE")) == 0);
    const SpecKernels *spec_shade = nullptr, *spec_raygen = nullptr;
    if (!cli_set && !direct && !probe_mode && (specialize < 0 ? specialize_env : specialize != 0)) {
        SpecRequest rq{opt, scene->shade_tris != nullptr && !opt.pre_transformed_vertices, !shade_fast, count_work != 0, SPEC_SHADE, wide};
        std::string why;
        spec_shade = spec_kernels(rq, &why);
        if (spec_shade) { rq.program = SPEC_RAYGEN; spec_raygen = spec_kernels(rq, &why); }
        if (!spec_shade || !spec_raygen) {
            static bool warned = false;
            if (!warned) fprintf(stderr, "[trhip] no specialised shading program for {%s}: %s - rendering with the general kernels\n", spec_key(rq).c_str(), why.c_str());
            warned = true;
            spec_shade = nullptr; spec_raygen = nullptr;
        }
    }
    return Program{cli_set, shade_fast, wide, spec_shade, spec_raygen};
}

int PtStage::get_program(trhip_program_info* out) {
    memset(out, 0, sizeof(*out));
    const Program p = choose_program();
    out->kind = p.shade ? 2 : (p.cli_set ? 1 : 0);
    out->ieee = p.shade_fast ? 0 : 1;
    SpecRequest rq{opt, scene->shade_tris != nullptr && !opt.pre_transformed_vertices, !p.shade_fast, count_work != 0, SPEC_SHADE, p.wide};
    const std::string key = (out->kind == 2 ? "compiled: " : out->kind == 1 ? "command-line set, ahead of time: " : "general kernels: ") + spec_key(rq);
    snprintf(out->key, sizeof(out->key), "%s", key.c_str());
    unsigned long long h = spec_sources_hash();
    const unsigned long long build = TRHIP_BUILD_ID;
    h = spec_fnv1a(h, &build, sizeof(build));
    h = spec_fnv1a(h, &out->kind, sizeof(out->kind)); h = spec_fnv1a(h, &out->ieee, sizeof(out->ieee));
    const int dir = direct ? 1 : 0;
    h = spec_fnv1a(h, &dir, sizeof(dir));
    if (out->kind != 0) { const std::string k = spec_key(rq); h = spec_fnv1a(h, k.c_str(), k.size()); }
    if (p.shade) { h = spec_fnv1a(h, &p.shade->code_hash, 8); h = spec_fnv1a(h, &p.raygen->code_hash, 8); }
    out->identity = h;
    return 0;
}

int PtStage::render(const trhip_pt_targets& targets, uint target_w, uint target_h, uint viewports, hipStream_t stream) {
    if (!scene->accel_built) return set_error("trhip_pt_render: call trhip_scene_build_accel first");
    const bool probe = probes != nullptr;
    if (probe != probe_mode) return set_error("trhip_pt_render: a probe stage renders batches of probes (trhip_sh_render), a camera stage pixels");
    if (viewports == 0 || viewports % frame_batch != 0) return set_error("trhip_pt_render: the layers of a launch are a whole number of frames (trhip_pt_set_frame_batch)");
    const uint frame_views = viewports / frame_batch;
    if (!probe && (uint64_t)shard_vp_base + (uint64_t)(frame_views - 1) * shard_vp_stride >= scene->camera_count)
        return set_error("trhip_pt_render: viewport count exceeds uploaded cameras");
    if (frame_batch > 1 && (accumulated_samples != 0 || direct)) return set_error("trhip_pt_render: a frame batch renders independent frames of the path tracer (reset the accumulation first)");
    if (opt.samples_per_pass <= 0 || opt.samples_per_pixel % opt.samples_per_pass != 0)
        return set_error("trhip_pt_render: samples_per_pixel must be a multiple of samples_per_pass");
    if (!probe && (dist.size_x == 0 || dist.size_y == 0)) return set_error("trhip_pt_render: distribution not set");
    PtParams P{};
    P.opt = opt;
    uint lw, lh;
    if (probe) { lw = probes->n_paths(); lh = 1; }
    else get_ray_count(dist, lw, lh);
    if (probe) { P.opt.hide_lights = 1; P.clamp_first_bounce = 1; }
    P.L.size_x = dist.size_x; P.L.size_y = dist.size_y; P.L.strategy = dist.strategy; P.L.index = dist.index;
    P.L.count = dist.strategy == 2 ? calculate_shuffled_strips_b(dist.size_x, dist.size_y) : dist.count;
    P.L.primary = dist.primary; P.L.launch_w = lw; P.L.launch_h = lh;
    P.viewports = viewports;
    const size_t n = (size_t)lw * lh * viewports;
    if (n == 0) return 0;
    if (n > 0xFFFFFFF0ull) return set_error("trhip_pt_render: launch too large");
    P.n_launch = (uint)n; P.id_offset = 0; P.n_ids = (uint)n;
    P.max_sobol_bounces = (uint)(opt.max_bounces > 8 ? 8 : opt.max_bounces);
    P.sample_counter = frame_counter * (uint)opt.samples_per_pixel * shard_sample_stride;
    P.vp_base = shard_vp_base; P.vp_stride = shard_vp_stride;
    P.frame_views = frame_views; P.frame_counter_step = (uint)opt.samples_per_pixel * shard_sample_stride;
    { uint s = opt.rng_seed; P.rng_seed = s != 0 ? pcg(s) : 0; }
    P.samples_accumulated = accumulated_samples;
    P.target_w = target_w; P.target_h = target_h;
    P.nee_point = opt.nee_point > 0; P.nee_dir = opt.nee_directional > 0; P.nee_env = opt.nee_envmap > 0; P.nee_tri = opt.nee_triangles > 0;
    nee_probabilities(*scene, opt.nee_point, opt.nee_triangles, opt.nee_directional, opt.nee_envmap, P.prob_point, P.prob_tri, P.prob_dir, P.prob_env);
    P.count_work = 1;
    P.bounce_words = (uint)BC_STRIDE * ((uint)opt.max_bounces + 2u);
    P.fused_resolve = opt.samples_per_pass == 1;
    P.T = targets;
    P.tm_display = nullptr; P.tm_op = tm_info.op; P.tm_exposure = tm_info.exposure; P.tm_gamma = tm_info.gamma; P.tm_grid = tm_info.alpha_grid_background;
    const bool timing = detailed_timing != 0;
    static const bool sample_lanes_enabled = !(getenv("TRHIP_SAMPLE_LANES") && atoi(getenv("TRHIP_SAMPLE_LANES")) == 0);
    const int passes_total = opt.samples_per_pixel / opt.samples_per_pass;
    const int sample_lane_count = std::min(passes_total, PT_LANES);
    const bool sample_lanes = sample_lanes_enabled && !direct && !timing && lanes == 0 && opt.samples_per_pass == 1 && passes_total >= 2 &&
                              n * (size_t)sample_lane_count * 224u <= ((size_t)8 << 30);
    if (int rc = ensure_buffers(sample_lanes ? n * (size_t)sample_lane_count : n, targets.diffuse || targets.reflection)) return rc;
    PathBuffers& pb = impl->pb;
    if (probe && !pb.first_dist) HIPCHK(hipMalloc(&pb.first_dist, impl->capacity * sizeof(float)));
    SceneView sv = scene->view();
    if (opt.pre_transformed_vertices) {
        if (int rc = ensure_world_vertices(*scene, stream)) return rc;
        sv.vertices = scene->world_vertices; sv.spans = scene->world_spans;
    }
    const bool count = count_work != 0;
    const bool two_level = scene->two_level;
    const int tq_in_effect = terminal_query_in_effect();
    if (tq_in_effect < 0) return set_error("trhip_pt_render: TRHIP_TERMINAL_QUERY is not auto or off");
    const bool terminal_query = tq_in_effect != 0;
    const Program prog = choose_program();
    const bool wide = prog.wide, cli_set = prog.cli_set, shade_fast = prog.shade_fast;
    const SpecKernels *spec_shade = prog.shade, *spec_raygen = prog.raygen;
    auto launch_raygen = [&](uint blocks, hipStream_t on, const PtParams& LP, const PathBuffers& lb) {
        if (probe) launch_sh_raygen(blocks, on, LP, lb, *probes);
        else if (spec_raygen) {
            SceneView a0 = sv; PtParams a1 = LP; PathBuffers a2 = lb;
            void* args[] = {&a0, &a1, &a2};
            (void)hipModuleLaunchKernel(spec_raygen->raygen, blocks, 1, 1, KB, 1, 1, 0, on, args, nullptr);
        } else hipLaunchKernelGGL(k_raygen<SpecGeneral>, dim3(blocks), dim3(KB), 0, on, sv, LP, lb);
    };
    auto launch_shade = [&](bool count, bool last, uint blocks, hipStream_t on, const PtParams& LP, const PathBuffers& lb, int bounce, const uint* q, uint* bc, uint* qn) {
        if (spec_shade) {
            SceneView a0 = sv; PtParams a1 = LP; PathBuffers a2 = lb;
            void* args[] = {&a0, &a1, &a2, &bounce, &q, &bc, &qn};
            (void)hipModuleLaunchKernel(last ? spec_shade->shade_last : spec_shade->shade, blocks, 1, 1, KB, 1, 1, 0, on, args, nullptr);
        } else if (shade_fast) launch_shade_fast(cli_set, count, last, blocks, on, sv, LP, lb, bounce, q, bc, qn);
        else if (last) {
            if (count) hipLaunchKernelGGL((k_shade<true, true>), dim3(blocks), dim3(KB), 0, on, sv, LP, lb, bounce, q, bc, qn);
            else if (cli_set) hipLaunchKernelGGL((k_shade<false, true, SpecCli>), dim3(blocks), dim3(KB), 0, on, sv, LP, lb, bounce, q, bc, qn);
            else hipLaunchKernelGGL((k_shade<false, true>), dim3(blocks), dim3(KB), 0, on, sv, LP, lb, bounce, q, bc, qn);
        }
        else if (count) hipLaunchKernelGGL((k_shade<true, false>), dim3(blocks), dim3(KB), 0, on, sv, LP, lb, bounce, q, bc, qn);
        else if (cli_set) hipLaunchKernelGGL((k_shade<false, false, SpecCli>), dim3(blocks), dim3(KB), 0, on, sv, LP, lb, bounce, q, bc, qn);
        else hipLaunchKernelGGL((k_shade<false, false>), dim3(blocks), dim3(KB), 0, on, sv, LP, lb, bounce, q, bc, qn);
    };
    static const int lanes_env = getenv("TRHIP_LANES") ? atoi(getenv("TRHIP_LANES")) : PT_LANES;
    static const bool overlap_enabled = !(getenv("TRHIP_OVERLAP") && atoi(getenv("TRHIP_OVERLAP")) == 0);
    static const size_t lanes_min_paths = getenv("TRHIP_LANES_MIN_PATHS") ? (size_t)atol(getenv("TRHIP_LANES_MIN_PATHS")) : (size_t)100000;
    static const size_t slots2_min_paths = getenv("TRHIP_SLOTS2_MIN_PATHS") ? (size_t)atol(getenv("TRHIP_SLOTS2_MIN_PATHS")) : (size_t)50000;
    const int auto_lanes = frame_slots >= 3 ? 1
                         : frame_slots == 2 ? (n < slots2_min_paths ? 1 : std::min(lanes_env, 2))
                         : (n < lanes_min_paths ? 1 : std::max(1, std::min(n < 2 * lanes_min_paths ? std::min(lanes_env, 2) : lanes_env, PT_LANES)));
    const int n_lanes = sample_lanes ? sample_lane_count : (timing ? 1 : (lanes > 0 ? std::min(lanes, PT_LANES) : auto_lanes));
    static const bool fused_enabled = !(getenv("TRHIP_FUSED") && atoi(getenv("TRHIP_FUSED")) == 0);
    const bool first_hit_targets = targets.albedo || targets.material || targets.normal || targets.pos || targets.instance_id || targets.screen_motion;
    const bool fused = fused_enabled && !timing && !count;
    const bool overlap = overlap_enabled && !timing && !fused && n_lanes == 1;
    if (!direct && (overlap || n_lanes > 1)) {
        int main_cls = -1;
        if (stream == last_main && impl->main_cls >= 0) main_cls = impl->main_cls;
        else if (stream != last_main || impl->main_tries < 16) {
            (void)stream_pool_class(stream, &main_cls, false);
            impl->main_tries = stream != last_main ? 1 : impl->main_tries + 1;
        }
        const bool main_changed = stream != last_main || main_cls != impl->main_cls;
        impl->main_cls = main_cls;
        if (main_changed && main_cls >= 0 && impl->side) {
            bool collide = false;
            for (int l = 1; l < PT_LANES; ++l) {
                hipStream_t ls = l == 1 ? impl->side : impl->lane_stream[l];
                int c = -1;
                if (ls && stream_pool_class(ls, &c, false) == 0 && c == main_cls) collide = true;
            }
            if (collide) {
                stream_pool_release(impl->side); impl->side = nullptr;
                (void)hipEventDestroy(impl->ev_fork); (void)hipEventDestroy(impl->ev_join);
                for (int l = 2; l < PT_LANES; ++l) if (impl->lane_stream[l]) { stream_pool_release(impl->lane_stream[l]); impl->lane_stream[l] = nullptr; (void)hipEventDestroy(impl->lane_join[l]); }
            }
        }
        if (!impl->side) {
            if (int rc = stream_pool_acquire(&impl->side, &stream, 1)) return rc;
            HIPCHK(hipEventCreateWithFlags(&impl->ev_fork, hipEventDisableTiming));
            HIPCHK(hipEventCreateWithFlags(&impl->ev_join, hipEventDisableTiming));
        }
        for (int l = 2; l < n_lanes; ++l) if (!impl->lane_stream[l]) {
            hipStream_t taken[PT_LANES] = {stream, impl->side};
            for (int k = 2; k < l; ++k) taken[k] = impl->lane_stream[k];
            if (int rc = stream_pool_acquire(&impl->lane_stream[l], taken, l)) return rc;
            HIPCHK(hipEventCreateWithFlags(&impl->lane_join[l], hipEventDisableTiming));
        }
    }
    if (n_lanes != last_lanes || stream != last_main || impl->main_cls != last_lane_pipes[0]) {
        last_lanes = n_lanes; last_main = stream;
        bool shared = false;
        for (int l = 0; l < n_lanes && l < 4; ++l) {
            int c = -1;
            if (l == 0) { c = impl->main_cls; if (c < 0) { (void)stream_pool_class(stream, &c, false); impl->main_cls = c; } }
            else (void)stream_pool_class(l == 1 ? impl->side : impl->lane_stream[l], &c, false);
            last_lane_pipes[l] = c;
            for (int k = 0; k < l; ++k) if (c >= 0 && last_lane_pipes[k] == c) shared = true;
        }
        static bool warned = false;
        if (shared && !warned && getenv("TRHIP_DEBUG") && atoi(getenv("TRHIP_DEBUG")) != 0) {
            warned = true;
            fprintf(stderr, "trhip: %d lanes of a frame on pipes %d %d %d %d - two lanes share a hardware pipe and will not overlap "
                            "(GPU_MAX_HW_QUEUES=%s; include/trhip.h, \"process requirements\")\n", n_lanes, last_lane_pipes[0], last_lane_pipes[1],
                    last_lane_pipes[2], last_lane_pipes[3], getenv("GPU_MAX_HW_QUEUES") ? getenv("GPU_MAX_HW_QUEUES") : "unset");
        }
    }
    const bool pixel_lanes = n_lanes >= 3 && !sample_lanes;
    const bool few_slots = (n_lanes == 1 && (frame_slots == 2 || frame_slots == 3)) || (n_lanes == 2 && frame_slots == 2);
    const uint grid_cap = (!timing && !getenv("TRHIP_GRID_BLOCKS")) ? ((pixel_lanes || few_slots) ? 768u : 1024u) : trace_grid_cap();
    static const uint n_cu = [] { int dev = 0, cu = 256; (void)hipGetDevice(&dev); (void)hipDeviceGetAttribute(&cu, hipDeviceAttributeMultiprocessorCount, dev); return (uint)std::max(cu, 1); }();
    const uint closest_cap = (timing && !getenv("TRHIP_GRID_BLOCKS")) ? std::min(n_cu * (uint)TR_CLOSEST_WAVES, trace_grid_cap()) : grid_cap;
    const uint shadow_cap = (timing && !getenv("TRHIP_GRID_BLOCKS")) ? std::min(n_cu * (uint)TR_SHADOW_WAVES, trace_grid_cap()) : grid_cap;
    {
        const size_t lane_paths = sample_lanes ? n : (n + (size_t)n_lanes - 1) / (size_t)n_lanes;
        const size_t lane_blocks = std::min<size_t>(std::max(std::max(closest_cap, shadow_cap), grid_cap), fused_grid_factor() * ((lane_paths + KB - 1) / KB) + 1);
        if (int rc = ensure_qspill(impl->pb, impl->qspill_lane_words, impl->qspill_regions, (size_t)std::max(n_lanes, overlap ? 2 : 1), lane_blocks)) return rc;
    }
    auto& ev = impl->ev;
    auto timed = [&](int kind, hipStream_t on, auto&& launch) {
        if (!timing) { launch(); return; }
        TimedSpan sp{kind, impl->get_event(), impl->get_event()};
        (void)hipEventRecord(sp.a, on);
        launch();
        (void)hipEventRecord(sp.b, on);
        impl->pending.push_back(sp);
    };
    if (timing_pending) {
        float ms = 0;
        if (hipEventElapsedTime(&ms, ev[0], ev[1]) == hipSuccess) impl->prev_frame_ms = ms;
        else (void)hipGetLastError();
    }
    HIPCHK(hipEventRecord(ev[0], stream));
    if (direct) {
        if (!pb.sh_cweight) HIPCHK(hipMalloc(&pb.sh_cweight, impl->capacity * 16));
        PtParams LP = P;
        LP.opt.hide_lights = 1;
        LP.opt.mis_mode = 0;
        PathBuffers lb = pb;
        const uint blocks_all = (LP.n_ids + KB - 1) / KB;
        const uint blocks_q = blocks_all < grid_cap ? blocks_all : grid_cap;
        const int passes = opt.samples_per_pixel / opt.samples_per_pass;
        for (int pass = 0; pass < passes; ++pass) {
            LP.previous_samples = (uint)pass * (uint)opt.samples_per_pass;
            LP.sample_in_pass = 0;
            LP.rng_sample = shard_sample_base + shard_sample_stride * LP.previous_samples;
            timed(T_RAYGEN, stream, [&] { hipLaunchKernelGGL(k_raygen<SpecGeneral>, dim3(blocks_all), dim3(KB), 0, stream, sv, LP, lb); });
            timed(T_CLOSEST, stream, [&] {
                auto kc = two_level ? (count ? k_trace_closest<true, false, true, true> : k_trace_closest<false, false, true, true>)
                                    : (count ? k_trace_closest<true, false> : k_trace_closest<false, false>);
                hipLaunchKernelGGL(kc, dim3(blocks_q), dim3(KB), 0, stream, sv, LP, lb, 0, (const uint*)nullptr, lb.bounce);
            });
            for (int smp = 0; smp < opt.samples_per_pass; ++smp) {
                if (smp > 0) hipLaunchKernelGGL(k_direct_next_sample, dim3(1), dim3(1), 0, stream, lb.bounce);
                timed(T_SHADE, stream, [&] {
                    if (count) hipLaunchKernelGGL(k_direct<true>, dim3(blocks_q), dim3(KB), 0, stream, sv, LP, lb, smp, lb.bounce);
                    else hipLaunchKernelGGL(k_direct<false>, dim3(blocks_q), dim3(KB), 0, stream, sv, LP, lb, smp, lb.bounce);
                });
                timed(T_SHADOW, stream, [&] {
                    auto ks = two_level ? (count ? k_trace_shadow_direct<true, true> : k_trace_shadow_direct<false, true>)
                                        : (count ? k_trace_shadow_direct<true> : k_trace_shadow_direct<false>);
                    hipLaunchKernelGGL(ks, dim3(blocks_q), dim3(KB), 0, stream, sv, LP, lb, lb.bounce);
                });
            }
            timed(T_RESOLVE, stream, [&] { hipLaunchKernelGGL(k_resolve_direct, dim3(blocks_all), dim3(KB), 0, stream, LP, lb); });
        }
        HIPCHK(hipEventRecord(ev[1], stream));
        HIPCHK(hipGetLastError());
        timing_pending = true;
        impl->frames++;
        frame_counter++;
        accumulated_samples += (uint)opt.samples_per_pixel;
        return 0;
    }
    static const int slices_env = getenv("TRHIP_LANE_SLICES") ? std::max(1, std::min(atoi(getenv("TRHIP_LANE_SLICES")), 4)) : 1;
    const int n_slices = (sample_lanes || n_lanes < 2) ? n_lanes : n_lanes * slices_env;
    const uint per_lane = sample_lanes ? (uint)n : (uint)((((n + n_slices - 1) / n_slices + 63) / 64) * 64);
    {
        const size_t tiles = n / 64;
        const bool even = !sample_lanes && viewports == 1 && (lw & 7u) == 0 && (lh & 7u) == 0 && n_slices > 1 && tiles % (size_t)n_slices == 0 &&
                          (size_t)per_lane * (size_t)n_slices == n;
        P.L.tile_lanes = even ? (uint)n_slices : 1u;
        P.L.tiles_per_lane = even ? (uint)(tiles / (size_t)n_slices) : 0u;
    }
    if (sample_lanes) for (int l = 0; l < n_lanes; ++l) if (!impl->pass_done[l]) HIPCHK(hipEventCreateWithFlags(&impl->pass_done[l], hipEventDisableTiming));
    struct LaneCtx { hipStream_t ls; PtParams LP; PathBuffers lb; uint blocks_all, blocks_q, blocks_f; bool shadow_in_flight; };
    LaneCtx lane_ctx[PT_LANES * 4];
    int lanes_used = 0;
    for (int slice = 0; slice < n_slices; ++slice) {
        const int lane = slice % n_lanes;
        LaneCtx& c = lane_ctx[slice];
        c.ls = lane == 0 ? stream : (lane == 1 ? impl->side : impl->lane_stream[lane]);
        c.LP = P;
        c.LP.id_offset = sample_lanes ? 0u : (uint)slice * per_lane;
        if (c.LP.id_offset >= n) break;
        c.LP.n_ids = std::min(per_lane, (uint)n - c.LP.id_offset);
        PathBuffers& lb = c.lb;
        lb = pb;
        lb.counters = pb.counters + lane * CNT_WORDS;
        lb.bounce = pb.bounce + (size_t)lane * P.bounce_words;
        lb.qspill = pb.qspill + (size_t)lane * impl->qspill_lane_words;
        const size_t q0 = sample_lanes ? (size_t)lane * n : (size_t)c.LP.id_offset;
        lb.queue[0] = pb.queue[0] + q0; lb.queue[1] = pb.queue[1] + q0;
        lb.sh_org_tmax = pb.sh_org_tmax + q0; lb.sh_dir_id = pb.sh_dir_id + q0;
        lb.sh_contrib = pb.sh_contrib + q0; lb.sh_lobes = pb.sh_lobes + q0;
        if (sample_lanes) {
            const size_t o = (size_t)lane * n;
            lb.org_pdf += o; lb.dir_reg += o; lb.atten_alpha += o; lb.diffuse += o; lb.reflection += o; lb.plobes += o; lb.first_mat += o; lb.first_emis += o;
            lb.rng += o; lb.misc += o; lb.hit += o;
        }
        c.blocks_all = (c.LP.n_ids + KB - 1) / KB;
        c.blocks_q = c.blocks_all < grid_cap ? c.blocks_all : grid_cap;
        c.blocks_f = std::min(grid_cap, c.blocks_all * fused_grid_factor());
        c.shadow_in_flight = false;
        lanes_used = slice + 1;
    }
    const int passes = passes_total;
    bool merged_raygen = false;
    auto enqueue_pass = [&](int lane, int pass, int only) -> int {
        LaneCtx& c = lane_ctx[lane];
        const hipStream_t ls = c.ls;
        PtParams& LP = c.LP;
        PathBuffers& lb = c.lb;
        const uint blocks_all = c.blocks_all, blocks_q = c.blocks_q, blocks_f = c.blocks_f;
        bool& shadow_in_flight = c.shadow_in_flight;
        {
            LP.previous_samples = (uint)pass * (uint)opt.samples_per_pass;
            for (int s = 0; s < opt.samples_per_pass; ++s) {
                LP.sample_in_pass = (uint)s;
                LP.rng_sample = shard_sample_base + shard_sample_stride * (LP.previous_samples + LP.sample_in_pass);
                if ((only == -2 || only == -1) && !merged_raygen) timed(T_RAYGEN, ls, [&] {
                    launch_raygen(blocks_all, ls, LP, lb);
                });
                for (int bounce = 0; bounce < opt.max_bounces; ++bounce) {
                    if (only != -2 && only != bounce) continue;
                    const uint* q = bounce == 0 ? nullptr : lb.queue[bounce & 1];
                    uint* qn = lb.queue[(bounce + 1) & 1];
                    uint* bc = lb.bounce + BC_STRIDE * bounce;
                    const bool tq = terminal_query && bounce == opt.max_bounces - 1;
                    if (fused && tq) {
                        hipLaunchKernelGGL((wide ? k_trace_fused_terminal<true> : k_trace_fused_terminal<false>), dim3(blocks_f), dim3(KB), 0, ls, sv, LP, lb, bounce, q, bc, bc - BC_STRIDE, qn);
                    } else if (fused && bounce > 0) {
                        hipLaunchKernelGGL((two_level ? k_trace_fused<true, true> : (wide ? k_trace_fused<true> : k_trace_fused<false>)), dim3(blocks_f), dim3(KB), 0, ls, sv, LP, lb, bounce, q, bc, bc - BC_STRIDE);
                    } else {
                        timed(T_CLOSEST, ls, [&] {
                            if (tq) {
                                auto kt = count ? k_trace_closest_terminal<true, false> : (timing ? (wide ? k_trace_closest_terminal<false, true, true> : k_trace_closest_terminal<false, true, false>)
                                                                                                  : (wide ? k_trace_closest_terminal<false, false, true> : k_trace_closest_terminal<false, false, false>));
                                hipLaunchKernelGGL(kt, dim3(std::min(blocks_all, closest_cap)), dim3(KB), 0, ls, sv, LP, lb, bounce, q, bc, qn);
                                return;
                            }
                            auto kc = two_level ? (count ? k_trace_closest<true, false, true, true> : k_trace_closest<false, false, true, true>)
                                    : count ? k_trace_closest<true, false> : (timing ? (wide ? k_trace_closest<false, true, true> : k_trace_closest<false, true, false>)
                                                                                     : (wide ? k_trace_closest<false, false, true> : k_trace_closest<false, false, false>));
                            hipLaunchKernelGGL(kc, dim3(std::min(blocks_all, closest_cap)), dim3(KB), 0, ls, sv, LP, lb, bounce, q, bc);
                        });
                    }
                    if (shadow_in_flight) { HIPCHK(hipStreamWaitEvent(ls, impl->ev_join, 0)); shadow_in_flight = false; }
                    timed(T_SHADE, ls, [&] {
                        static const uint shade_cap_env = getenv("TRHIP_SHADE_BLOCKS") ? (uint)atoi(getenv("TRHIP_SHADE_BLOCKS")) : 0u;
                        const uint shade_cap = shade_cap_env ? shade_cap_env : ((pixel_lanes || (n_lanes == 2 && frame_slots == 2)) ? 768u : 2048u);
                        const uint blocks_s = timing ? blocks_q : (blocks_all < shade_cap ? blocks_all : shade_cap);
                        static const bool last_variant = !(getenv("TRHIP_SHADE_LAST") && atoi(getenv("TRHIP_SHADE_LAST")) == 0);
                        const bool last = last_variant && bounce == opt.max_bounces - 1;
                        if (tq) launch_shade(count, last, blocks_s, ls, LP, lb, bounce, qn, bc + BC_STRIDE, const_cast<uint*>(q));
                        else launch_shade(count, last, blocks_s, ls, LP, lb, bounce, q, bc, qn);
                    });
                    if (bounce == 0 && first_hit_targets && s == opt.samples_per_pass - 1 && LP.samples_accumulated + LP.previous_samples == 0)
                        hipLaunchKernelGGL(k_first_hit_gbuffer, dim3(blocks_all), dim3(KB), 0, ls, sv, LP, lb);
                    if (bounce < opt.max_bounces - 1 && !fused) {
                        hipStream_t ss = ls;
                        if (overlap) {
                            HIPCHK(hipEventRecord(impl->ev_fork, ls));
                            HIPCHK(hipStreamWaitEvent(impl->side, impl->ev_fork, 0));
                            ss = impl->side;
                        }
                        timed(T_SHADOW, ss, [&] {
                            auto ks = two_level ? (count ? k_trace_shadow<true, true, true> : k_trace_shadow<false, true, true>)
                                                : count ? k_trace_shadow<true> : (wide ? k_trace_shadow<false, true> : k_trace_shadow<false, false>);
                            PathBuffers sb = lb;
                            if (overlap) sb.qspill = pb.qspill + impl->qspill_lane_words;
                            hipLaunchKernelGGL(ks, dim3(std::min(blocks_all, shadow_cap)), dim3(KB), 0, ss, sv, LP, sb, bc);
                        });
                        if (overlap) { HIPCHK(hipEventRecord(impl->ev_join, impl->side)); shadow_in_flight = true; }
                    }
                }
                if (only != -2 && only != opt.max_bounces) continue;
                if (shadow_in_flight) { HIPCHK(hipStreamWaitEvent(ls, impl->ev_join, 0)); shadow_in_flight = false; }
                if (!LP.fused_resolve) hipLaunchKernelGGL(k_accumulate_sample, dim3(blocks_all), dim3(KB), 0, ls, LP, lb);
            }
            if (only != -2 && only != opt.max_bounces) return 0;
            if (sample_lanes && pass > 0) HIPCHK(hipStreamWaitEvent(ls, impl->pass_done[(pass - 1) % n_lanes], 0));
            LP.tm_display = (pass == passes - 1 && !direct) ? reinterpret_cast<f4*>(tm_display) : nullptr;
            if (!probe) timed(T_RESOLVE, ls, [&] { hipLaunchKernelGGL(k_resolve, dim3(blocks_all), dim3(KB), 0, ls, LP, lb); });
            if (sample_lanes && pass + 1 < passes) HIPCHK(hipEventRecord(impl->pass_done[lane], ls));
        }
        return 0;
    };
    static const char* order_env = getenv("TRHIP_ENQUEUE");
    const bool interleave = order_env ? strcmp(order_env, "lanes") != 0 : (impl->prev_frame_ms > 0.0f && impl->prev_frame_ms < 3.0f);
    static const bool merged_raygen_enabled = !(getenv("TRHIP_MERGED_RAYGEN") && atoi(getenv("TRHIP_MERGED_RAYGEN")) == 0);
    merged_raygen = merged_raygen_enabled && interleave && !sample_lanes && lanes_used > 1 && lanes_used == n_lanes && passes == 1 &&
                               opt.samples_per_pass == 1;
    if (merged_raygen) {
        PtParams RP = lane_ctx[0].LP;
        RP.id_offset = 0; RP.n_ids = (uint)n;
        RP.bounce_words = P.bounce_words * (uint)n_lanes;
        RP.previous_samples = 0; RP.sample_in_pass = 0;
        RP.rng_sample = shard_sample_base;
        launch_raygen((RP.n_ids + KB - 1) / KB, stream, RP, lane_ctx[0].lb);
    }
    if (n_lanes > 1) {
        HIPCHK(hipEventRecord(impl->ev_fork, stream));
        HIPCHK(hipStreamWaitEvent(impl->side, impl->ev_fork, 0));
        for (int l = 2; l < n_lanes; ++l) HIPCHK(hipStreamWaitEvent(impl->lane_stream[l], impl->ev_fork, 0));
    }
    if (sample_lanes) {
        for (int pass = 0; pass < passes; ++pass) if (int rc = enqueue_pass(pass % lanes_used, pass, -2)) return rc;
    } else if (interleave && lanes_used > 1 && passes == 1 && opt.samples_per_pass == 1) {
        static const int skew = (order_env && !strncmp(order_env, "skew", 4)) ? atoi(order_env + 4) : 0;
        const int n_steps = opt.max_bounces + 2;
        for (int first = 0; first < lanes_used; first += n_lanes) {
            const int here = std::min(n_lanes, lanes_used - first);
            for (int t = 0; t < n_steps + skew * (here - 1); ++t)
                for (int lane = 0; lane < here; ++lane) {
                    const int step = t - skew * lane;
                    if (step < 0 || step >= n_steps) continue;
                    if (int rc = enqueue_pass(first + lane, 0, step - 1)) return rc;
                }
        }
    } else {
        for (int lane = 0; lane < lanes_used; ++lane)
            for (int pass = 0; pass < passes; ++pass) if (int rc = enqueue_pass(lane, pass, -2)) return rc;
    }
    if (n_lanes > 1) {
        HIPCHK(hipEventRecord(impl->ev_join, impl->side));
        HIPCHK(hipStreamWaitEvent(stream, impl->ev_join, 0));
        for (int l = 2; l < n_lanes; ++l) {
            HIPCHK(hipEventRecord(impl->lane_join[l], impl->lane_stream[l]));
            HIPCHK(hipStreamWaitEvent(stream, impl->lane_join[l], 0));
        }
    }
    HIPCHK(hipEventRecord(ev[1], stream));
    HIPCHK(hipGetLastError());
    timing_pending = true;
    impl->frames++;
    frame_counter += frame_batch;
    accumulated_samples += (uint)opt.samples_per_pixel;
    return 0;
}

const PathBuffers* PtStage::path_buffers() const { return &impl->pb; }

int PtStage::get_counters(trhip_counters* out, hipStream_t stream) {
    memset(out, 0, sizeof(*out));
    if (!impl->pb.counters) return 0;
    HIPCHK(hipStreamSynchronize(stream));
    uint hl[PT_LANES][CNT_WORDS];
    HIPCHK(hipMemcpy(hl, impl->pb.counters, sizeof(hl), hipMemcpyDeviceToHost));
    uint* h = hl[0];
    auto rd = [&](int i) { uint64_t v = 0; for (int l = 0; l < PT_LANES; ++l) v += (uint64_t)hl[l][i] | ((uint64_t)hl[l][i + 1] << 32); return v; };
    out->closest_rays = rd(CNT_CLOSEST); out->shadow_rays = rd(CNT_SHADOWRAYS); out->node_visits = rd(CNT_NODES);
    out->tri_tests = rd(CNT_TRIS); out->alpha_tests = rd(CNT_ALPHA); out->surface_hits = rd(CNT_SURF);
    for (int l = 1; l < PT_LANES; ++l) { h[CNT_OVERFLOW] |= hl[l][CNT_OVERFLOW]; h[CNT_MAXSP] = std::max(h[CNT_MAXSP], hl[l][CNT_MAXSP]); h[CNT_MAXVIS] = std::max(h[CNT_MAXVIS], hl[l][CNT_MAXVIS]); }
    out->stack_overflows = h[CNT_OVERFLOW];
    if (getenv("TRHIP_DEBUG"))
        fprintf(stderr, "[trhip] closest-hit loop: %llu node phases (%llu with <= 16 active rays serving %llu visits, %llu with <= 8), %llu triangle phases; quad tail: %llu node phases, %llu triangle phases; %llu node visits\n",
                (unsigned long long)rd(CNT_PH_NODE), (unsigned long long)rd(CNT_PH_NODE16), (unsigned long long)rd(CNT_LV_NODE16), (unsigned long long)rd(CNT_PH_NODE8),
                (unsigned long long)rd(CNT_PH_TRI), (unsigned long long)rd(CNT_PH_QNODE), (unsigned long long)rd(CNT_PH_QTRI), (unsigned long long)rd(CNT_NODES));
    if (getenv("TRHIP_DEBUG")) {
        fprintf(stderr, "[trhip] per-lane node phases by live rays (1-8, 9-16, ..., 57-64):");
        for (int b = 0; b < 8; ++b) fprintf(stderr, " %llu", (unsigned long long)rd(CNT_PH_HIST + 2 * b));
        fprintf(stderr, "\n");
    }
    if (getenv("TRHIP_DEBUG")) { float* f = (float*)(h + CNT_DBG); fprintf(stderr, "[trhip] overflow %u src %u; max stack depth %u; max node visits per ray %u; worst ray o=(%g %g %g) d=(%g %g %g) bounce %g id %g pdf %g reg %g\n", h[CNT_OVERFLOW], h[CNT_DBG + 12], h[CNT_MAXSP], h[CNT_MAXVIS], f[0], f[1], f[2], f[3], f[4], f[5], f[6], f[7], f[8], f[9]); }
    return 0;
}

int PtStage::get_phase_counters(trhip_phase_counters* out, hipStream_t stream) {
    memset(out, 0, sizeof(*out));
    if (!impl->pb.counters) return 0;
    HIPCHK(hipStreamSynchronize(stream));
    uint hl[PT_LANES][CNT_WORDS];
    HIPCHK(hipMemcpy(hl, impl->pb.counters, sizeof(hl), hipMemcpyDeviceToHost));
    auto rd = [&](int i) { uint64_t v = 0; for (int l = 0; l < PT_LANES; ++l) v += (uint64_t)hl[l][i] | ((uint64_t)hl[l][i + 1] << 32); return v; };
    out->lane_node_phases = rd(CNT_PH_NODE); out->lane_tri_phases = rd(CNT_PH_TRI);
    out->quad_node_phases = rd(CNT_PH_QNODE); out->quad_tri_phases = rd(CNT_PH_QTRI);
    out->lane_node_phases_le16 = rd(CNT_PH_NODE16); out->lane_node_visits_le16 = rd(CNT_LV_NODE16);
    out->closest_node_visits = rd(CNT_CNODES);
    for (int b = 0; b < 8; ++b) out->lane_node_phase_hist[b] = rd(CNT_PH_HIST + 2 * b);
    return 0;
}

int PtStage::get_light_counters(trhip_light_counters* out, hipStream_t stream) {
    memset(out, 0, sizeof(*out));
    if (!impl->pb.counters) return 0;
    HIPCHK(hipStreamSynchronize(stream));
    uint hl[PT_LANES][CNT_WORDS];
    HIPCHK(hipMemcpy(hl, impl->pb.counters, sizeof(hl), hipMemcpyDeviceToHost));
    auto rd = [&](int i) { uint64_t v = 0; for (int l = 0; l < PT_LANES; ++l) v += (uint64_t)hl[l][i] | ((uint64_t)hl[l][i + 1] << 32); return v; };
    out->sphere_tests = rd(CNT_LTESTS); out->node_visits = rd(CNT_LNODES); out->walk_fallbacks = rd(CNT_LFALLBACKS);
    return 0;
}

int PtStage::get_max_stack_depth(uint32_t* out, hipStream_t stream) {
    *out = 0;
    if (!impl->pb.counters) return 0;
    HIPCHK(hipStreamSynchronize(stream));
    uint hl[PT_LANES][CNT_WORDS];
    HIPCHK(hipMemcpy(hl, impl->pb.counters, sizeof(hl), hipMemcpyDeviceToHost));
    for (int l = 0; l < PT_LANES; ++l) *out = std::max(*out, hl[l][CNT_MAXSP]);
    return 0;
}

int PtStage::terminal_query_in_effect() const {
    int mode = terminal_query;
    if (mode < 0) {
        const char* e = getenv("TRHIP_TERMINAL_QUERY");
        std::string v = e ? e : "";
        for (char& c : v) c = (char)tolower((unsigned char)c);
        if (v.empty() || v == "auto") mode = TRHIP_TERMINAL_QUERY_AUTO;
        else if (v == "off") mode = TRHIP_TERMINAL_QUERY_OFF;
        else return -1;
    }
    if (mode != TRHIP_TERMINAL_QUERY_AUTO) return 0;
    return (!direct && opt.max_bounces >= 2 && scene->accel_built && !scene->two_level && scene->tris && scene->emitter_count <= TR_EMITTER_MAX &&
            scene->sphere_light_count() == 0) ? 1 : 0;
}

int PtStage::get_terminal_counters(trhip_terminal_counters* out, hipStream_t stream) {
    memset(out, 0, sizeof(*out));
    out->in_effect = terminal_query_in_effect() > 0 ? 1u : 0u;
    out->emitter_triangles = scene->emitter_count;
    out->threshold = TR_EMITTER_MAX;
    if (!impl->pb.counters) return 0;
    HIPCHK(hipStreamSynchronize(stream));
    uint hl[PT_LANES][CNT_WORDS];
    HIPCHK(hipMemcpy(hl, impl->pb.counters, sizeof(hl), hipMemcpyDeviceToHost));
    auto rd = [&](int i) { uint64_t v = 0; for (int l = 0; l < PT_LANES; ++l) v += (uint64_t)hl[l][i] | ((uint64_t)hl[l][i + 1] << 32); return v; };
    out->blocked_rays = rd(CNT_TQ_BLOCKED); out->fallback_rays = rd(CNT_TQ_FALLBACK);
    return 0;
}

int PtStage::reset_counters() {
    if (impl->pb.counters) HIPCHK(hipMemset(impl->pb.counters, 0, PT_LANES * CNT_WORDS * sizeof(uint)));
    if (int rc = resolve_pending()) return rc;
    for (int k = 0; k < T_KINDS; ++k) { impl->acc_ms[k] = 0; impl->acc_launches[k] = 0; }
    impl->frames = 0;
    return 0;
}

int PtStage::resolve_pending() {
    for (auto& sp : impl->pending) {
        HIPCHK(hipEventSynchronize(sp.b));
        float ms = 0;
        HIPCHK(hipEventElapsedTime(&ms, sp.a, sp.b));
        impl->acc_ms[sp.kind] += ms;
        impl->acc_launches[sp.kind]++;
        impl->pool.push_back(sp.a); impl->pool.push_back(sp.b);
    }
    impl->pending.clear();
    return 0;
}

int PtStage::get_timings(trhip_timings* out) {
    memset(out, 0, sizeof(*out));
    if (timing_pending) {
        HIPCHK(hipEventSynchronize(impl->ev[1]));
        HIPCHK(hipEventElapsedTime(&out->path_tracing_ms, impl->ev[0], impl->ev[1]));
    }
    if (int rc = resolve_pending()) return rc;
    out->trace_closest_ms = impl->acc_ms[T_CLOSEST]; out->trace_shadow_ms = impl->acc_ms[T_SHADOW]; out->shade_ms = impl->acc_ms[T_SHADE];
    out->raygen_ms = impl->acc_ms[T_RAYGEN]; out->resolve_ms = impl->acc_ms[T_RESOLVE];
    out->trace_closest_launches = impl->acc_launches[T_CLOSEST]; out->trace_shadow_launches = impl->acc_launches[T_SHADOW];
    out->shade_launches = impl->acc_launches[T_SHADE]; out->frames = impl->frames;
    return 0;
}

}

extern "C" uint64_t trhip_build_id(void) { return (uint64_t)TRHIP_BUILD_ID; }

#if TR_TIMELINE
extern "C" int trhip_debug_timeline(unsigned long long* out, int reset) {
    if (hipDeviceSynchronize() != hipSuccess) return 1;
    if (out && hipMemcpyFromSymbol(out, HIP_SYMBOL(tr::g_timeline), sizeof(unsigned long long) * tr::TL_WORDS) != hipSuccess) return 1;
    if (reset) { static unsigned long long zero[tr::TL_WORDS]; if (hipMemcpyToSymbol(HIP_SYMBOL(tr::g_timeline), zero, sizeof(zero)) != hipSuccess) return 1; }
    return 0;
}
#endif
```

### tauray_amd/csrc/pt.h

```cpp
#pragma once
#include "build.h"
#include "sh_probes.h"

namespace tr {

void get_ray_count(const trhip_distribution& d, uint& w, uint& h);

inline void nee_probabilities(const DeviceScene& scene, float w_point, float w_tri, float w_dir, float w_env, float& prob_point, float& prob_tri,
                              float& prob_dir, float& prob_env) {
    float point = (w_point > 0 && scene.point_light_count > 0) ? w_point : 0.0f;
    float tri = (w_tri > 0 && scene.tri_light_count > 0) ? w_tri : 0.0f;
    float dir = (w_dir > 0 && scene.directional_light_count > 0) ? w_dir : 0.0f;
    float env = (w_env > 0 && scene.environment_proj >= 0) ? w_env : 0.0f;
    float sum = point + tri + dir + env;
    float inv_sum = sum <= 0.0f ? 0.0f : (1.0f / sum + 1e-5f);
    prob_point = point * inv_sum; prob_tri = tri * inv_sum; prob_dir = dir * inv_sum; prob_env = env * inv_sum;
}

int stream_pool_acquire(hipStream_t* out, const hipStream_t* overlap_with = nullptr, int n_overlap = 0);
void stream_pool_release(hipStream_t s);
int stream_pool_class(hipStream_t s, int* cls, bool blocking = false);
int stream_pool_pipe_classes(int* classes_out, int* streams_out);

struct PathBuffers;

class PtStage {
public:
    PtStage(DeviceScene* scene, const trhip_pt_options& opt);
    ~PtStage();
    int render(const trhip_pt_targets& targets, uint target_w, uint target_h, uint viewports, hipStream_t stream);
    int get_counters(trhip_counters* out, hipStream_t stream);
    int reset_counters();
    int get_timings(trhip_timings* out);
    int get_phase_counters(trhip_phase_counters* out, hipStream_t stream);
    int get_light_counters(trhip_light_counters* out, hipStream_t stream);
    int get_max_stack_depth(uint32_t* out, hipStream_t stream);
    int get_terminal_counters(trhip_terminal_counters* out, hipStream_t stream);
    int get_program(trhip_program_info* out);
    int terminal_query_in_effect() const;

    DeviceScene* scene;
    trhip_pt_options opt;
    trhip_distribution dist;
    uint frame_counter = 0;
    uint accumulated_samples = 0;
    int count_work = 0, detailed_timing = 0;
    uint shard_vp_base = 0, shard_vp_stride = 1, shard_sample_base = 0, shard_sample_stride = 1;
    int frame_slots = 0;
    int lanes = 0;
    int last_lanes = 0, last_lane_pipes[4] = {-1, -1, -1, -1};
    hipStream_t last_main = nullptr;
    void* tm_display = nullptr;
    trhip_tonemap_info tm_info{};
    uint frame_batch = 1;
    int ieee_shading = -1;
    int specialize = -1;
    int terminal_query = -1;
    bool direct = false;
    bool probe_mode = false;
    const ShProbeBatch* probes = nullptr;
    const PathBuffers* path_buffers() const;
    hipStream_t last_stream = nullptr;

    struct Program { bool cli_set, shade_fast, wide; const struct SpecKernels *shade, *raygen; };
    Program choose_program();

private:
    struct Impl;
    Impl* impl;
    bool timing_pending = false;
    int ensure_buffers(size_t n, bool lobe_sums);
    int resolve_pending();
    void free_buffers();
};

}
```

### tauray_amd/csrc/resolve_kernel.h

```cpp
#pragma once
#include "pt_state.h"
#include "tonemap.h"

namespace tr {

namespace {

TR_DEV f4 sample_color(const PtParams& P, f4 d, f4 r, f4 fm, f4 fe) {
    const f3 albedo = P.opt.use_white_albedo_on_first_bounce ? F3(1) : F3(fm);
    const float metallic = fm.w;
    const float approx_fresnel = 0.02f;
    const f3 dd = F3(d) * albedo * (1 - metallic);
    const f3 rr = F3(r) * mix3(F3(approx_fresnel), albedo, metallic) / mixf(approx_fresnel, 1.0f, metallic);
    return F4(F3(fe) + (dd + rr), fe.w);
}

TR_DEV void accumulate_sample_path(const PtParams& P, const PathBuffers& pb, uint i) {
    u4 misc = pb.misc[i];
    if (misc.w & 1u) return;
    const f4 s = pb.sum_color[i], d = pb.diffuse[i], r = pb.reflection[i];
    const f4 c = sample_color(P, d, r, pb.first_mat[i], pb.first_emis[i]);
    pb.sum_color[i] = F4(s.x + c.x, s.y + c.y, s.z + c.z, c.w);
    if (pb.sum_diffuse) {
        const f4 sd = pb.sum_diffuse[i], sr = pb.sum_reflection[i];
        pb.sum_diffuse[i] = F4(sd.x + d.x, sd.y + d.y, sd.z + d.z, sd.w + d.w);
        pb.sum_reflection[i] = F4(sr.x + r.x, sr.y + r.y, sr.z + r.z, sr.w + r.w);
    }
}

TR_DEV void resolve_path(const PtParams& P, const PathBuffers& pb, uint i) {
    uint lx, ly, lz;
    launch_coord(P.L, i, lx, ly, lz);
    int wx, wy;
    if (!get_write_pixel_pos(P.L, lx, ly, wx, wy)) return;
    if ((uint)wx >= P.target_w || (uint)wy >= P.target_h) return;
    const float spp = (float)P.opt.samples_per_pass;
    const size_t idx = ((size_t)lz * P.target_h + (uint)wy) * P.target_w + (uint)wx;
    const uint prev_samples = P.samples_accumulated + P.previous_samples;
    const float keep = prev_samples != 0 ? (float)prev_samples / (float)((uint)P.opt.samples_per_pass + prev_samples) : 0.0f;
    auto accumulate = [&](void* image, f4 value) {
        f4* target = reinterpret_cast<f4*>(image);
        if (prev_samples != 0) value = mix4(value, target[idx], keep);
        target[idx] = value;
        if (P.tm_display && image == P.T.color) P.tm_display[idx] = tonemap_pixel(value, P.tm_op, P.tm_exposure, P.tm_gamma, P.tm_grid, (uint)wx, (uint)wy);
    };
    if (P.fused_resolve) {
        const f4 d = pb.diffuse[i], r = pb.reflection[i];
        if (P.T.color) {
            const f4 c = sample_color(P, d, r, pb.first_mat[i], pb.first_emis[i]);
            accumulate(P.T.color, F4(c.x, c.y, c.z, P.opt.transparent_background ? c.w : 1.0f));
        }
        if (P.T.diffuse) accumulate(P.T.diffuse, d);
        if (P.T.reflection) accumulate(P.T.reflection, r);
        return;
    }
    if (P.T.color) {
        const f4 s = pb.sum_color[i];
        accumulate(P.T.color, F4(s.x / spp, s.y / spp, s.z / spp, P.opt.transparent_background ? s.w : 1.0f));
    }
    if (P.T.diffuse) { const f4 s = pb.sum_diffuse[i]; accumulate(P.T.diffuse, F4(s.x / spp, s.y / spp, s.z / spp, s.w / spp)); }
    if (P.T.reflection) { const f4 s = pb.sum_reflection[i]; accumulate(P.T.reflection, F4(s.x / spp, s.y / spp, s.z / spp, s.w / spp)); }
}

__global__ __launch_bounds__(KB) void k_accumulate_sample(PtParams P, PathBuffers pb) {
    const uint i = blockIdx.x * KB + threadIdx.x;
    if (i < P.n_ids) accumulate_sample_path(P, pb, i + P.id_offset);
}
__global__ __launch_bounds__(KB) void k_resolve(PtParams P, PathBuffers pb) {
    const uint i = blockIdx.x * KB + threadIdx.x;
    if (i < P.n_ids) resolve_path(P, pb, i + P.id_offset);
}

}

}
```

### tauray_amd/csrc/sh_probes.hip

```cpp
#include <algorithm>
#include <cmath>
#include <cstring>
#include <string>

#include "pt_state.h"
#include "pt.h"
#include "sh_probes.h"
#include "stage_host.h"

namespace tr {
namespace {

__global__ __launch_bounds__(KB) void k_sh_raygen(PtParams P, PathBuffers pb, ShProbeBatch B) {
    if (blockIdx.x == 0) for (uint k = threadIdx.x; k < P.bounce_words; k += KB) pb.bounce[k] = 0;
    uint i = blockIdx.x * KB + threadIdx.x;
    if (i >= P.n_ids) return;
    i += P.id_offset;
    uint q, s;
    sh_path_of_id(B, i, q, s);
    const ShGridData& G = B.grid;
    const uint p = B.probe_base + q;
    const uint x = p % G.grid_size[0], y = (p / G.grid_size[0]) % G.grid_size[1], z = p / (G.grid_size[0] * G.grid_size[1]);
    LocalSampler ls = init_local_sampler(u4{x, y, z, s}, B.sample_counter, B.rng_seed, SAMPLER_UNIFORM);
    f3 offset = F3(0.0f);
// ... 246 lines not shown
    m4 t;
    memcpy(&t, transform, sizeof(t));
    unpack_grid_data(pack_grid_data(t, F3(scaling[0], scaling[1], scaling[2]), resolution, samples_per_probe, frame_counter, history_length, temporal_ratio), out);
    return 0;
}

int trhip_sh_render(trhip_sh* s, void* stream) {
    if (!s) return set_error("trhip_sh_render: null stage");
    DEVCHK(s->hip_device);
    DeviceScene* scene = device_scene(s->dev);
    if (int r = check_scene_ready("trhip_sh_render", scene->instance_count, scene->accel_built)) return r;
    hipStream_t st = (hipStream_t)stream;
    s->last_stream = st;
    const uint32_t n = s->opt.samples_per_probe;
    const size_t probes = s->probes();
    const uint32_t fit = SH_MAX_BATCH_PATHS / n;
    const uint32_t per_batch = (uint32_t)std::min<size_t>(probes, s->batch_probes ? s->batch_probes : fit);
    ShProjectParams PP{};
    PP.batch.grid = grid_data_of(s, s->history_length + 1);
    PP.batch.samples = n;
    PP.batch.sample_counter = s->frame_counter * n;
    { uint seed = s->path.rng_seed; PP.batch.rng_seed = seed != 0 ? pcg(seed) : 0; }
    PP.coef_mult = (4.0f * SH_PI) / (float)n;
    PP.previous = s->grid; PP.grid = s->grid; PP.grid_half = s->grid_half;
    const bool timing = s->pt->detailed_timing != 0;
    size_t used_events = 0;
    auto project_event = [&]() -> hipError_t {
        if (used_events == s->project_events.size()) { hipEvent_t e; if (hipError_t r = hipEventCreate(&e)) return r; s->project_events.push_back(e); }
        return hipEventRecord(s->project_events[used_events++], st);
    };
    HIPCHK(hipEventRecord(s->ev[0], st));
    for (size_t base = 0; base < probes; base += per_batch) {
        PP.batch.probe_base = (uint32_t)base;
        PP.batch.n_probes = (uint32_t)std::min<size_t>(per_batch, probes - base);
        s->pt->probes = &PP.batch;
        const int rc = s->pt->render(trhip_pt_targets{}, 0, 0, 1, st);
        s->pt->probes = nullptr;
        if (rc) return rc;
        const PathBuffers pb = *s->pt->path_buffers();
        const dim3 grid(PP.batch.n_probes), block(SH_BLOCK);
        if (timing) HIPCHK(project_event());
        switch (s->opt.order) {
            case 0: hipLaunchKernelGGL(k_sh_project<0>, grid, block, 0, st, pb, PP); break;
            case 1: hipLaunchKernelGGL(k_sh_project<1>, grid, block, 0, st, pb, PP); break;
            case 2: hipLaunchKernelGGL(k_sh_project<2>, grid, block, 0, st, pb, PP); break;
            case 3: hipLaunchKernelGGL(k_sh_project<3>, grid, block, 0, st, pb, PP); break;
            default: hipLaunchKernelGGL(k_sh_project<4>, grid, block, 0, st, pb, PP); break;
        }
        if (timing) HIPCHK(project_event());
    }
    s->timed_events = used_events;
    HIPCHK(hipEventRecord(s->ev[1], st));
    HIPCHK(hipGetLastError());
    s->history_length += 1;
    s->frame_counter += 1;
    s->frames += 1;
    return 0;
}

int trhip_sh_get_grids(trhip_sh* s, void** grid_dev, void** grid_half_dev) {
    if (!s) return set_error("trhip_sh_get_grids: null stage");
    if (grid_dev) *grid_dev = s->grid;
    if (grid_half_dev) *grid_half_dev = s->grid_half;
    return 0;
}

int trhip_sh_download(trhip_sh* s, int which, void* host, size_t bytes) {
    return stage_download("trhip_sh_download", s, host, bytes, [&](const void*& src, size_t& size) {
        switch (which) {
            case TRHIP_SH_GRID: src = s->grid; size = s->entries() * sizeof(f4); break;
            case TRHIP_SH_GRID_HALF: src = s->grid_half; size = s->entries() * 4 * sizeof(__half); break;
            default: return set_error("trhip_sh_download: unknown buffer");
        }
        return 0;
    });
}

int trhip_sh_get_counters(trhip_sh* s, trhip_counters* out) {
    if (!s || !out) return set_error("trhip_sh_get_counters: null argument");
    DEVCHK(s->hip_device);
    return s->pt->get_counters(out, s->last_stream);
}

int trhip_sh_set_profiling(trhip_sh* s, int count_work, int detailed_timing) {
    if (!s) return set_error("trhip_sh_set_profiling: null stage");
    s->pt->count_work = count_work; s->pt->detailed_timing = detailed_timing;
    if (!detailed_timing) s->timed_events = 0;
    return 0;
}

int trhip_sh_get_timings(trhip_sh* s, trhip_sh_timings* out) {
    if (int r = stage_total_ms("trhip_sh_get_timings", s, out)) return r;
    snprintf(out->name, sizeof(out->name), "SH path tracing");
    if (s->frames == 0) return 0;
    trhip_timings t;
    if (int r = s->pt->get_timings(&t)) return r;
    out->raygen_ms = t.raygen_ms; out->trace_closest_ms = t.trace_closest_ms; out->trace_shadow_ms = t.trace_shadow_ms; out->shade_ms = t.shade_ms;
    for (size_t i = 0; i + 1 < s->timed_events; i += 2) {
        float ms = 0.0f;
        HIPCHK(hipEventElapsedTime(&ms, s->project_events[i], s->project_events[i + 1]));
        out->project_ms += ms;
    }
    return 0;
}

int trhip_sh_reset_counters(trhip_sh* s) {
    if (!s) return set_error("trhip_sh_reset_counters: null stage");
    DEVCHK(s->hip_device);
    HIPCHK(hipStreamSynchronize(s->last_stream));
    return s->pt->reset_counters();
}

}
```

### tauray_amd/csrc/shade_kernel.h

```cpp
#pragma once
#include "pt_state.h"

namespace tr {

namespace {

TR_DEV float bsdf_mis_pdf(const SceneView& sv, const PtParams& P, float pl_pdf, float dl_pdf, float tri_pdf, float env_pdf, float bsdf_pdf) {
    if (bsdf_pdf == 0.0f) return 1.0f;
    float avg_nee_pdf =
        dl_pdf * P.prob_dir / (float)max(sv.directional_light_count, 1u) +
        tri_pdf * P.prob_tri / (float)max(sv.tri_light_count, 1u) +
        env_pdf * P.prob_env +
        pl_pdf * P.prob_point / (float)max(sv.point_light_count, 1u);
    if (P.opt.mis_mode == 2) return (avg_nee_pdf * avg_nee_pdf + bsdf_pdf * bsdf_pdf) / bsdf_pdf;
    if (P.opt.mis_mode == 1) return avg_nee_pdf + bsdf_pdf;
    return avg_nee_pdf > 0 ? __builtin_huge_valf() : bsdf_pdf;
}
TR_DEV float nee_mis_pdf(const PtParams& P, float nee_pdf, float bsdf_pdf) {
    if (nee_pdf <= 0.0f) return -nee_pdf;
    if (P.opt.mis_mode == 2) return (nee_pdf * nee_pdf + bsdf_pdf * bsdf_pdf) / nee_pdf;
    if (P.opt.mis_mode == 1) return nee_pdf + bsdf_pdf;
    return nee_pdf;
}
TR_DEV float clamp_contribution_mul(const PtParams& P, f3 contrib) {
// ... 79 lines not shown
        out_length = ray_plane_intersection_dist(out_dir, A, B, C);
        if (isinf(tri_pdf) || tri_pdf <= 0 || out_length <= P.opt.min_ray_dist || any_nan(out_dir)) {
            pdf = 1.0f; out_dir = F3(0);
            return F3(0);
        }
        if (emission_tex_id >= 0) {
            f3 bary = get_barycentric_coords(out_dir * out_length, A, B, C);
            f2 uv = bary.x * unpack_half2x16(r3.x) + bary.y * unpack_half2x16(r3.y) + bary.z * unpack_half2x16(r3.z);
            color = color * F3(sample_texture(sv, emission_tex_id, uv));
        }
        out_length -= P.opt.min_ray_dist;
        pdf = P.prob_tri * tri_pdf / light_count;
        STL(STL_L_TRI);
        return color;
    }
    if (kind == ENV) {
        const AliasEntry at = {r0.x, r0.y, TR_F(r0.z), TR_F(r0.w)};
        f3 color = sample_environment_map(sv, rnd, alias_i, at, out_dir, out_length, pdf);
        pdf *= P.prob_env;
        STL(STL_L_ENV);
        return color;
    }
    if (kind == DIR) {
        DirectionalLight dl;
        dl.color = F3(TR_F(r0.x), TR_F(r0.y), TR_F(r0.z)); dl.shadow_map_index = (int)r0.w; dl.dir = F3(TR_F(r1.x), TR_F(r1.y), TR_F(r1.z)); dl.dir_cutoff = TR_F(r1.w);
        out_length = __builtin_huge_valf();
        out_dir = sample_cone(F2(u.x, u.y), -dl.dir, dl.dir_cutoff);
        pdf = dl.dir_cutoff >= 1.0f ? -1.0f : 1.0f / (2.0f * TR_PI * (1.0f - dl.dir_cutoff));
        f3 color = pdf > 0 ? dl.color * pdf : dl.color;
        pdf *= P.prob_dir / light_count;
        STL(STL_L_DIR);
        return color;
    }
#undef TR_F
    out_dir = F3(0); out_length = 0; pdf = 1.0f;
    return F3(0);
}

TR_DEV void correct_lobes_for_normal_map(f3 sample_dir, f3 geometric_normal, Lobes& l) {
    if (dot(geometric_normal, sample_dir) < 0) { l.diffuse = 0; l.dielectric_reflection = 0; l.metallic_reflection = 0; }
    else l.transmission = 0;
}

#ifndef TR_SHADE_WAVES
#define TR_SHADE_WAVES 3
#endif
#ifndef TR_SHADE_LAST_WAVES
#define TR_SHADE_LAST_WAVES 5
#endif
struct SpecGeneral {
    static constexpr bool pinned = false, shade_tris = false, wide_textures = true;
    TR_DEV static void pin(PtParams&) {}
};
struct SpecCli {
    static constexpr bool pinned = true, shade_tris = true, wide_textures = false;
    TR_DEV static void pin(PtParams& P) {
        P.opt.sampler = 0; P.opt.film = 0; P.opt.mis_mode = 2; P.opt.bounce_mode = 2; P.opt.tri_light_mode = 1;
        P.opt.russian_roulette_delta = 0.0f; P.opt.indirect_clamping = 0.0f; P.opt.regularization_gamma = 0.0f;
        P.opt.depth_of_field = 0; P.opt.hide_lights = 0; P.opt.use_white_albedo_on_first_bounce = 0; P.opt.transparent_background = 0;
        P.opt.pre_transformed_vertices = 0;
        P.clamp_first_bounce = 0;
    }
};
#ifdef TR_SPEC_SAMPLER
struct SpecMacros {
    static constexpr bool pinned = true, shade_tris = TR_SPEC_SHADE_TRIS != 0, wide_textures = TR_SPEC_WIDE_TEXTURES != 0;
    TR_DEV static void pin(PtParams& P) {
        P.opt.sampler = TR_SPEC_SAMPLER; P.opt.film = TR_SPEC_FILM; P.opt.mis_mode = TR_SPEC_MIS; P.opt.bounce_mode = TR_SPEC_BOUNCE_MODE;
        P.opt.tri_light_mode = TR_SPEC_TRI_LIGHT_MODE; P.opt.projection = TR_SPEC_PROJECTION;
        if (!TR_SPEC_ROULETTE) P.opt.russian_roulette_delta = 0.0f;
        if (!TR_SPEC_CLAMPING) P.opt.indirect_clamping = 0.0f;
        if (!TR_SPEC_REGULARIZATION) P.opt.regularization_gamma = 0.0f;
        P.opt.depth_of_field = TR_SPEC_DOF; P.opt.hide_lights = TR_SPEC_HIDE_LIGHTS; P.opt.use_white_albedo_on_first_bounce = TR_SPEC_WHITE_ALBEDO;
        P.opt.transparent_background = TR_SPEC_TRANSPARENT; P.opt.pre_transformed_vertices = TR_SPEC_PRE_TRANSFORMED;
        P.nee_point = TR_SPEC_NEE_POINT; P.nee_tri = TR_SPEC_NEE_TRI; P.nee_dir = TR_SPEC_NEE_DIR; P.nee_env = TR_SPEC_NEE_ENV;
        if (!TR_SPEC_NEE_POINT) P.prob_point = 0.0f;
        if (!TR_SPEC_NEE_TRI) P.prob_tri = 0.0f;
        if (!TR_SPEC_NEE_DIR) P.prob_dir = 0.0f;
        if (!TR_SPEC_NEE_ENV) P.prob_env = 0.0f;
        P.clamp_first_bounce = 0;
    }
};
#endif
struct ShadeOut {
    bool alive = false;
    bool want_shadow = false;
    f3 sh_o = {0, 0, 0}, sh_d = {0, 0, 0}, sh_c = {0, 0, 0};
    f2 sh_w = {0, 0};
    float sh_tmax = 0, sh_lum = 0;
};

template <bool COUNT, bool LAST, typename S>
TR_DEV void shade_path(const SceneView& sv, const PtParams& P, const PathBuffers& pb, int bounce, uint id, u4 misc, ShadeOut& o, uint& surf) {
    bool& alive = o.alive;
    bool& want_shadow = o.want_shadow;
    f3 &sh_o = o.sh_o, &sh_d = o.sh_d, &sh_c = o.sh_c;
    f2& sh_w = o.sh_w;
    float &sh_tmax = o.sh_tmax, &sh_lum = o.sh_lum;
        const f4 o4 = pb.org_pdf[id], d4 = pb.dir_reg[id], a4 = pb.atten_alpha[id];
        const int4 h = pb.hit[id];
        f3 pos = F3(o4), view = F3(d4);
        float bsdf_pdf = o4.w, regularization = d4.w;
        f3 attenuation = F3(a4);
        f4 dif = F4(0), ref = F4(0);
        bool have = bounce == 0;
        f2 pl = bounce == 0 ? F2(0.0f, 1.0f) : pb.plobes[id];
        u4 rs = pb.rng[id];
        STL(STL_STATE);

        SampledMaterial mat;
        mat.albedo = F4(0); mat.metallic = 1; mat.roughness = 0; mat.emission = F3(0);
        mat.transmittance = 0; mat.ior_in = 1; mat.ior_out = 1; mat.f0 = 0;
        SurfacePoint v;
        v.pos = pos; v.hard_normal = F3(0); v.smooth_normal = F3(0); v.mapped_normal = F3(0); v.tri_light_pdf = 0;
        float pl_pdf = 0, dl_pdf = 0, tri_pdf = 0, env_pdf = 0;
        f3 light = F3(0);
        bool surface = false;
        if (h.x >= 0) {
            surface = true;
            if (COUNT) surf++;
            shade_surface(sv, h.x, h.y, __int_as_float(h.z), __int_as_float(h.w), view, pos, P.nee_tri != 0, P.opt.tri_light_mode, P.opt.pre_transformed_vertices != 0, v, mat, S::shade_tris);
            mat.albedo.w = 1.0f;
            if (P.nee_tri) {
                tri_pdf = v.tri_light_pdf;
                light = mat.emission;
                mat.emission = F3(0);
            }
        } else if (h.y >= 0) {
            const PointLight pl = sv.point_lights[h.y];
            f3 c = get_spotlight_intensity(pl, view) * pl.color / (pl.radius * pl.radius * TR_PI);
            if (P.nee_point) { light = c; pl_pdf = sample_point_light_pdf(pl, pos); }
            else mat.emission = c;
            v.pos = pos + __int_as_float(h.z) * view;
            v.mapped_normal = normalize(v.pos - pl.pos);
            mat.albedo = F4(0, 0, 0, 1);
        } else {
            f4 c = sv.environment_factor;
            if (sv.environment_proj >= 0) {
                f2 uv;
                uv.y = asinf(-view.y) / TR_PI + 0.5f;
                uv.x = atan2f(view.z, view.x) / (2 * TR_PI) + 0.5f;
                f4 t = sample_envmap(sv, uv);
                c.x *= t.x; c.y *= t.y; c.z *= t.z;
            }
            for (uint i = 0; i < sv.directional_light_count; ++i) {
                const DirectionalLight dl = sv.directional_lights[i];
                if (dl.dir_cutoff >= 1.0f) continue;
                float visible = stepf(dl.dir_cutoff, dot(view, -dl.dir));
                f3 dc = visible * dl.color / (2.0f * TR_PI * (1.0f - dl.dir_cutoff));
                if (P.nee_dir) { light += dc; dl_pdf += visible * sample_directional_light_pdf(dl); }
                else mat.emission += dc;
            }
            v.pos = pos;
            v.mapped_normal = -view;
            mat.albedo = F4(0);
            if (P.nee_env) {
                light += F3(c);
                env_pdf = sv.environment_proj >= 0 ? sample_environment_map_pdf(sv, view) : 0.0f;
            } else mat.emission += F3(c);
        }
        if (!surface) { STL(STL_NOSURFACE); }
        if (bounce == 0 && pb.first_dist) pb.first_dist[id] = length(v.pos - pos);
        const bool terminal = LAST || !surface || bounce == P.opt.max_bounces - 1;

        float mis_pdf = bsdf_mis_pdf(sv, P, pl_pdf, dl_pdf, tri_pdf, env_pdf, bsdf_pdf);
        float mis_weight = 1.0f;
// ... 98 lines not shown

struct ShadeKernArgs { SceneView sv; PtParams P; PathBuffers pb; int bounce; const uint* queue; uint* bc; uint* next_queue; };
#ifndef TR_SHADE_FRESH_ARGS
#define TR_SHADE_FRESH_ARGS 1
#endif
template <typename T>
TR_DEV void load_kernarg(T& dst, const T __attribute__((address_space(4)))* src) {
    static_assert(sizeof(T) % 4 == 0, "kernel arguments are whole words");
    uint* d = reinterpret_cast<uint*>(&dst);
    const uint __attribute__((address_space(4)))* s = (const uint __attribute__((address_space(4)))*)src;
#pragma unroll
    for (uint i = 0; i < sizeof(T) / 4; ++i) d[i] = s[i];
}

template <bool COUNT, bool LAST, typename S>
TR_DEV void shade_bounce(const SceneView& sv_, const PtParams& P_, const PathBuffers& pb, int bounce, const uint* queue, uint* bc, uint* next_queue) {
    PtParams P = P_;
    S::pin(P);
    SceneView sv = sv_;
    if (!S::wide_textures) sv.wide_textures = 0;
    const bool misc_needed = !S::pinned || P.opt.sampler == SAMPLER_SOBOL_Z2 || P.opt.sampler == SAMPLER_SOBOL_Z3;
    const uint n = queue ? bc[BC_QUEUE] : P.n_ids;
    const uint n_round = LAST ? n : ((n + (uint)KB - 1u) & ~((uint)KB - 1u));
    uint surf = 0;
#if TR_SHADE_TIMELINE
    stl_begin();
#endif
    for (uint qi = blockIdx.x * KB + threadIdx.x; qi < n_round; qi += gridDim.x * KB) {
#if TR_SHADE_FRESH_ARGS
        typedef const ShadeKernArgs __attribute__((address_space(4)))* KernArgPtr;
        KernArgPtr ka = (KernArgPtr)__builtin_amdgcn_kernarg_segment_ptr();
        asm volatile("" : "+s"(ka));
        PtParams P;
        load_kernarg(P, &ka->P);
        S::pin(P);
        SceneView sv;
        load_kernarg(sv, &ka->sv);
        if (!S::wide_textures) sv.wide_textures = 0;
#endif
        STL(STL_ITER);
        STL(STL_CALIBRATION);
        bool active = qi < n;
        uint id = 0;
        u4 misc = {0, 0, 0, 1};
        if (active) {
            id = queue ? queue[qi] : qi + P.id_offset;
            if (!misc_needed && queue) misc = u4{0u, 0u, id, 0u};
            else { misc = pb.misc[id]; active = !(misc.w & 1u); }
        }
        STL(STL_ID);
        ShadeOut o;
        if (active) shade_path<COUNT, LAST, S>(sv, P, pb, bounce, id, misc, o, surf);
        const bool alive = o.alive, want_shadow = o.want_shadow;
        if (LAST) continue;
        uint sslot, nslot;
        block_append2(&bc[BC_SHADOW], want_shadow, sslot, &bc[BC_STRIDE + BC_QUEUE], alive, nslot);
        STL(STL_APPEND);
        if (want_shadow) {
            pb.sh_org_tmax[sslot] = F4(o.sh_o, o.sh_tmax);
            pb.sh_dir_id[sslot] = F4(o.sh_d, __uint_as_float(id));
            pb.sh_contrib[sslot] = F4(o.sh_c, o.sh_lum);
            pb.sh_lobes[sslot] = o.sh_w;
        }
        if (alive) next_queue[nslot] = id;
        STL(STL_QUEUE);
    }
#if TR_SHADE_TIMELINE
    stl_end(bounce);
#endif
    if (COUNT && P.count_work) {
        for (int off = 32; off > 0; off >>= 1) surf += __shfl_xor(surf, off);
        if ((threadIdx.x & 63) == 0) add64(pb.counters, CNT_SURF, surf);
    }
}

template <typename S>
TR_DEV void raygen_paths(const SceneView& sv, const PtParams& P_, const PathBuffers& pb) {
    PtParams P = P_;
    S::pin(P);
    if (blockIdx.x == 0) for (uint k = threadIdx.x; k < P.bounce_words; k += KB) pb.bounce[k] = 0;
    uint i = blockIdx.x * KB + threadIdx.x;
    if (i >= P.n_ids) return;
    i += P.id_offset;
    uint lx, ly, lz;
    launch_coord(P.L, i, lx, ly, lz);
    int px, py;
    bool valid = get_pixel_pos(P.L, lx, ly, px, py);
    u4 misc = {0, 0, i, valid ? 0u : 1u};
    if (P.sample_in_pass == 0 && !P.fused_resolve) {
        pb.sum_color[i] = F4(0, 0, 0, 1);
        if (pb.sum_diffuse) { pb.sum_diffuse[i] = F4(0); pb.sum_reflection[i] = F4(0); }
    }
    if (!valid) { pb.misc[i] = misc; return; }
    LocalSampler ls = init_local_sampler(u4{(uint)px, (uint)py, global_viewport(P, lz), P.rng_sample}, sample_counter_of(P, lz),
                                         P.rng_seed, P.opt.sampler);
    f2 cam_offset = F2(0.0f);
    if (P.opt.film != 0) {
        f4 r = u4_to_unit(pcg4d(ls.rs));
        if (P.opt.film == 1) cam_offset = F2(r.x, r.y) * 2.0f - 1.0f;
        else cam_offset = sample_blackman_harris_concentric_disk(F2(r.x, r.y)) * 2.0f;
        cam_offset = cam_offset * (2.0f * P.opt.film_radius);
    }
    f2 dof_u = F2(0.5f);
    if (P.opt.depth_of_field) { f4 r = u4_to_unit(pcg4d(ls.rs)); dof_u = F2(r.x, r.y); }
    f3 origin, dir;
    get_screen_camera_ray(P.L, px, py, sv.cameras[global_viewport(P, lz)], P.opt.projection, P.opt.depth_of_field != 0, cam_offset, dof_u, origin, dir);
    misc.x = pcg4d(ls.rs).x;
    misc.y = ls.sobol_index;
    pb.org_pdf[i] = F4(origin, 0.0f);
    pb.dir_reg[i] = F4(dir, 1.0f);
    pb.atten_alpha[i] = F4(1, 1, 1, 1);
    pb.rng[i] = ls.rs;
    pb.misc[i] = misc;
}
template <typename S = SpecGeneral>
__global__ __launch_bounds__(KB) void k_raygen(SceneView sv, PtParams P, PathBuffers pb) { raygen_paths<S>(sv, P, pb); }

constexpr unsigned long long kernarg_next(unsigned long long off, unsigned long long size, unsigned long long align) { return (off + size + align - 1) / align * align; }
#define TR_KERNARG_OFF(m) __builtin_offsetof(ShadeKernArgs, m)
#define TR_ASSERT_SHADE_KERNARGS(kernel) \
    static_assert(__is_same(decltype(&kernel), void (*)(SceneView, PtParams, PathBuffers, int, const uint*, uint*, uint*)), \
                  #kernel " does not have the signature ShadeKernArgs mirrors"); \
    static_assert(TR_KERNARG_OFF(sv) == 0 && \
                  TR_KERNARG_OFF(P) == kernarg_next(TR_KERNARG_OFF(sv), sizeof(SceneView), alignof(PtParams)) && \
                  TR_KERNARG_OFF(pb) == kernarg_next(TR_KERNARG_OFF(P), sizeof(PtParams), alignof(PathBuffers)) && \
                  TR_KERNARG_OFF(bounce) == kernarg_next(TR_KERNARG_OFF(pb), sizeof(PathBuffers), alignof(int)) && \
                  TR_KERNARG_OFF(queue) == kernarg_next(TR_KERNARG_OFF(bounce), sizeof(int), alignof(const uint*)) && \
                  TR_KERNARG_OFF(bc) == kernarg_next(TR_KERNARG_OFF(queue), sizeof(const uint*), alignof(uint*)) && \
                  TR_KERNARG_OFF(next_queue) == kernarg_next(TR_KERNARG_OFF(bc), sizeof(uint*), alignof(uint*)) && \
                  sizeof(ShadeKernArgs) == TR_KERNARG_OFF(next_queue) + sizeof(uint*), \
                  "ShadeKernArgs is not the argument layout of " #kernel)

template <bool COUNT, bool LAST, typename S = SpecGeneral>
__global__ __launch_bounds__(KB, LAST ? TR_SHADE_LAST_WAVES : TR_SHADE_WAVES) void k_shade(SceneView sv, PtParams P, PathBuffers pb, int bounce, const uint* queue,
                                              uint* bc, uint* next_queue) {
    shade_bounce<COUNT, LAST, S>(sv, P, pb, bounce, queue, bc, next_queue);
}
TR_ASSERT_SHADE_KERNARGS((k_shade<false, false>));

}

}
```

### tauray_amd/csrc/trace_lanes.h

```cpp
#pragma once
#include "trace.h"
#include "trace_quad.h"
#include "pt_state.h"

namespace tr {

namespace {

struct TerminalCounts { uint blocked, fallback; };
template <bool COUNT, bool TWO_LEVEL = false, bool TERMINAL = false>
TR_DEV void closest_lane(const SceneView& sv, const PtParams& P, const PathBuffers& pb, int bounce, const uint* queue, uint qi, uint n, int* lds_stack,
                         const QuadCtx& qc, TraceStats& st, int& overflow, uint& max_vis, uint& rays, uint* next_queue = nullptr, uint* next_count = nullptr,
                         TerminalCounts* tc = nullptr) {
    bool valid = qi < n;
    uint id = 0;
    u4 misc = {0, 0, 0, 1};
    f4 o = F4(0), d = F4(0);
    if constexpr (TERMINAL) {
        f4 a = F4(0);
        if (valid) { id = queue[qi]; misc = pb.misc[id]; o = pb.org_pdf[id]; d = pb.dir_reg[id]; a = pb.atten_alpha[id]; }
        for (int b = 0; b < bounce; ++b) pcg(misc.x);
        TerminalRay term = {valid && terminal_early_ok(o.w, F3(a)), false};
        HitRecord hit;
        const uint before = st.nodes;
        trace_closest_wave4<0, COUNT, false, true>(sv, valid, F3(o), F3(d), P.opt.min_ray_dist, __builtin_huge_valf(), misc.x, lds_stack, qc, hit, st, overflow, &term);
        if (COUNT) st.cnodes += st.nodes - before;
        const bool keep = valid && !term.blocked;
        const uint slot = wave_append(next_count, keep);
        if (keep) {
            next_queue[slot] = id;
            pb.hit[id] = make_int4(hit.instance_id, hit.primitive_id, __float_as_int(hit.u), __float_as_int(hit.v));
        }
        if (valid) {
            rays++;
            if (COUNT) { tc->blocked += term.blocked ? 1u : 0u; tc->fallback += term.early ? 0u : 1u; }
        }
        return;
    }
    TL(const unsigned long long tl_chunk = tl_now();)
    if (valid) { id = queue ? queue[qi] : qi + P.id_offset; misc = pb.misc[id]; o = pb.org_pdf[id]; d = pb.dir_reg[id]; valid = !(misc.w & 1u); }
    TL(tl_data_arrived(); tl_misc(qc.tl, 3, tl_now() - tl_chunk);)
    for (int b = 0; b < bounce; ++b) pcg(misc.x);
    HitRecord hit;
    const uint before = st.nodes;
#if TR_QUAD_SWITCH > 0
    trace_closest_wave4<0, COUNT, TWO_LEVEL>(sv, valid, F3(o), F3(d), bounce == 0 ? 0.0f : P.opt.min_ray_dist, __builtin_huge_valf(), misc.x,
                                  lds_stack, qc, hit, st, overflow);
#else
    if (valid) trace_closest4<0, COUNT, TWO_LEVEL>(sv, F3(o), F3(d), bounce == 0 ? 0.0f : P.opt.min_ray_dist, __builtin_huge_valf(),
                                        misc.x, lds_stack, hit, st, overflow);
#endif
    if (COUNT) st.cnodes += st.nodes - before;
    if (!valid) return;
    if (COUNT) {
        const uint vis = st.nodes - before;
        max_vis = max(max_vis, vis);
        if (vis > 100000u && vis > atomicMax(&pb.counters[CNT_MAXVIS], vis)) {
            float* dbg = reinterpret_cast<float*>(pb.counters + CNT_DBG);
            dbg[0] = o.x; dbg[1] = o.y; dbg[2] = o.z; dbg[3] = d.x; dbg[4] = d.y; dbg[5] = d.z; dbg[6] = (float)bounce; dbg[7] = (float)id;
            dbg[8] = o.w; dbg[9] = d.w;
        }
    }
    const float tri_t = hit.instance_id >= 0 ? hit.t : __builtin_huge_valf();
    pb.hit[id] = make_int4(hit.instance_id, hit.primitive_id, __float_as_int(hit.u), __float_as_int(hit.v));
    if (sv.point_light_count != 0 && !(P.opt.hide_lights && bounce == 0)) {
        uint rid = id;
        asm volatile("" : "+v"(rid));
        const f3 lo = F3(pb.org_pdf[rid]), ld = F3(pb.dir_reg[rid]);
        if (ray_is_finite(lo, ld)) {
            const LightHit lh = trace_sphere_lights<COUNT>(sv, lo, ld, bounce == 0 ? 0.0f : P.opt.min_ray_dist, tri_t, lds_stack, st);
            if (lh.light >= 0) pb.hit[rid] = make_int4(-1, lh.light, __float_as_int(lh.t), 0);
        }
    }
    rays++;
    TL(tl_misc(qc.tl, 5, tl_now() - tl_chunk);)
}

TR_DEV QuadCtx make_quad_ctx(int* s_stack, int* s_owner, const PathBuffers& pb TL(, uint* s_tl = nullptr)) {
    QuadCtx qc;
    TL(qc.tl = s_tl ? s_tl + (threadIdx.x >> 6) * TL_WORDS : nullptr;)
    const uint wave = threadIdx.x >> 6;
    qc.wave_stack = s_stack + (threadIdx.x & ~63u);
    qc.owner_tab = s_owner + wave * TR_OWNER_WORDS;
    qc.spill = pb.qspill + ((size_t)blockIdx.x * (KB / 64) + wave) * (16u * TR_QSPILL);
    return qc;
}

template <bool COUNT, bool TWO_LEVEL, typename CONTRIB, typename LOBES>
TR_DEV void shadow_ray(const SceneView& sv, const PtParams& P, const PathBuffers& pb, bool valid, f4 o, f4 d, CONTRIB&& contrib, LOBES&& lobes, int* lds_stack, const QuadCtx& qc,
                       TraceStats& st, int& overflow, uint& rays) {
#if TR_QUAD_SWITCH > 0
    float vis = trace_shadow_wave4<COUNT, TWO_LEVEL>(sv, valid, F3(o), F3(d), P.opt.min_ray_dist, o.w, lds_stack, qc, st, overflow);
#else
    float vis = 1.0f;
    if (valid) vis = trace_shadow4<COUNT, TWO_LEVEL>(sv, F3(o), F3(d), P.opt.min_ray_dist, o.w, lds_stack, st, overflow);
#endif
    if (!valid) return;
    const uint id = __float_as_uint(d.w);
    if (vis != 0.0f) {
        const f4 c = contrib();
        float m = c.w * vis;
        if (c.w > 0.0f && m > P.opt.indirect_clamping) vis *= P.opt.indirect_clamping / m;
        const f3 radiance = F3(c.x * vis, c.y * vis, c.z * vis);
        const f2 w = lobes();
        if (w.x != 0.0f) { f4 d4 = pb.diffuse[id]; d4.x += radiance.x * w.x; d4.y += radiance.y * w.x; d4.z += radiance.z * w.x; pb.diffuse[id] = d4; }
        if (w.y != 0.0f) { f4 r4 = pb.reflection[id]; r4.x += radiance.x * w.y; r4.y += radiance.y * w.y; r4.z += radiance.z * w.y; pb.reflection[id] = r4; }
    }
    rays++;
}
template <bool COUNT, bool TWO_LEVEL = false>
TR_DEV void shadow_lane(const SceneView& sv, const PtParams& P, const PathBuffers& pb, uint qi, uint n, int* lds_stack, const QuadCtx& qc,
                        TraceStats& st, int& overflow, uint& rays) {
    const bool valid = qi < n;
    f4 o = F4(0), d = F4(0);
    if (valid) { o = pb.sh_org_tmax[qi]; d = pb.sh_dir_id[qi]; }
    shadow_ray<COUNT, TWO_LEVEL>(sv, P, pb, valid, o, d, [&] { return pb.sh_contrib[qi]; }, [&] { return pb.sh_lobes[qi]; }, lds_stack, qc, st, overflow, rays);
}

TR_DEV void flush_terminal_counters(const PtParams& P, const PathBuffers& pb, TerminalCounts tc) {
    if (!P.count_work) return;
    for (int off = 32; off > 0; off >>= 1) { tc.blocked += __shfl_xor(tc.blocked, off); tc.fallback += __shfl_xor(tc.fallback, off); }
    if ((threadIdx.x & 63) == 0) {
        add64(pb.counters, CNT_SURF, tc.blocked);
        add64(pb.counters, CNT_TQ_BLOCKED, tc.blocked);
        add64(pb.counters, CNT_TQ_FALLBACK, tc.fallback);
    }
}

template <bool COUNT>
TR_DEV void flush_trace_counters(const PtParams& P, const PathBuffers& pb, int overflow, int overflow_tag, uint closest_rays, uint shadow_rays,
                                 TraceStats st, uint max_vis) {
    if (overflow) { pb.counters[CNT_OVERFLOW] = 1; pb.counters[CNT_DBG + 12] = (uint)overflow_tag; }
    if (!P.count_work) return;
    for (int off = 32; off > 0; off >>= 1) {
        closest_rays += __shfl_xor(closest_rays, off); shadow_rays += __shfl_xor(shadow_rays, off);
        if (COUNT) {
            st.nodes += __shfl_xor(st.nodes, off); st.tris += __shfl_xor(st.tris, off); st.alpha += __shfl_xor(st.alpha, off);
            st.ph_node += __shfl_xor(st.ph_node, off); st.ph_tri += __shfl_xor(st.ph_tri, off); st.ph_node16 += __shfl_xor(st.ph_node16, off);
            st.ph_node8 += __shfl_xor(st.ph_node8, off); st.lv_node16 += __shfl_xor(st.lv_node16, off);
            st.ph_qnode += __shfl_xor(st.ph_qnode, off); st.ph_qtri += __shfl_xor(st.ph_qtri, off); st.cnodes += __shfl_xor(st.cnodes, off);
            st.ltests += __shfl_xor(st.ltests, off); st.lnodes += __shfl_xor(st.lnodes, off); st.lfallbacks += __shfl_xor(st.lfallbacks, off);
            for (int b = 0; b < 8; ++b) st.ph_hist[b] += __shfl_xor(st.ph_hist[b], off);
            st.maxsp = max(st.maxsp, (uint)__shfl_xor(st.maxsp, off)); max_vis = max(max_vis, (uint)__shfl_xor(max_vis, off));
        }
    }
    if ((threadIdx.x & 63) == 0) {
        add64(pb.counters, CNT_CLOSEST, closest_rays);
        add64(pb.counters, CNT_SHADOWRAYS, shadow_rays);
        if (COUNT) {
            add64(pb.counters, CNT_NODES, st.nodes); add64(pb.counters, CNT_TRIS, st.tris); add64(pb.counters, CNT_ALPHA, st.alpha);
            add64(pb.counters, CNT_PH_NODE, st.ph_node); add64(pb.counters, CNT_PH_TRI, st.ph_tri); add64(pb.counters, CNT_PH_NODE16, st.ph_node16);
            add64(pb.counters, CNT_PH_NODE8, st.ph_node8); add64(pb.counters, CNT_LV_NODE16, st.lv_node16);
            add64(pb.counters, CNT_PH_QNODE, st.ph_qnode); add64(pb.counters, CNT_PH_QTRI, st.ph_qtri); add64(pb.counters, CNT_CNODES, st.cnodes);
            add64(pb.counters, CNT_LTESTS, st.ltests); add64(pb.counters, CNT_LNODES, st.lnodes); add64(pb.counters, CNT_LFALLBACKS, st.lfallbacks);
            for (int b = 0; b < 8; ++b) add64(pb.counters, CNT_PH_HIST + 2 * b, st.ph_hist[b]);
            atomicMax(&pb.counters[CNT_MAXSP], st.maxsp); atomicMax(&pb.counters[CNT_MAXVIS], max_vis);
        }
    }
}

// ... 4 lines not shown
```

### tauray_amd/renderer.py

```python
from __future__ import annotations

import ctypes as C
import os
from dataclasses import dataclass, field
from typing import List, Optional

import numpy as np

from . import _lib
from ._lib import (AccelInfoC, AccelLayoutC, CountersC, DistributionC, LightAccelInfoC, LightCountersC, PtOptionsC, TerminalCountersC, SceneDescC, TimingsC,
                   TonemapInfoC, TrhipError, check)
from .distribution import (DISTRIBUTION_DUPLICATE, DISTRIBUTION_SCANLINE, DISTRIBUTION_SHUFFLED_STRIPS, DistributionParams,
                           get_device_distribution_params, get_distribution_target_size)
from .scene import SceneDesc, ShGrid, build_alias_table

FILM_POINT, FILM_BOX, FILM_BLACKMAN_HARRIS = 0, 1, 2
MIS_DISABLED, MIS_BALANCE_HEURISTIC, MIS_POWER_HEURISTIC = 0, 1, 2
BOUNCE_HEMISPHERE, BOUNCE_COSINE_HEMISPHERE, BOUNCE_MATERIAL = 0, 1, 2
TRI_LIGHT_AREA, TRI_LIGHT_SOLID_ANGLE, TRI_LIGHT_HYBRID = 0, 1, 2
SAMPLER_UNIFORM_RANDOM, SAMPLER_SOBOL_OWEN, SAMPLER_SOBOL_Z_ORDER_2D, SAMPLER_SOBOL_Z_ORDER_3D = 0, 1, 2, 3
TONEMAP_LINEAR, TONEMAP_GAMMA_CORRECTION, TONEMAP_FILMIC, TONEMAP_REINHARD, TONEMAP_REINHARD_LUMINANCE = 0, 1, 2, 3, 4
FEATURE_ALBEDO, FEATURE_WORLD_NORMAL, FEATURE_VIEW_NORMAL, FEATURE_WORLD_POS, FEATURE_VIEW_POS, FEATURE_DISTANCE = 0, 1, 2, 3, 4, 5
FEATURE_INSTANCE_ID = 9

# ... 421 lines not shown
    def set_frame_counter(self, frame_counter: int):
        check(_lib.lib().trhip_pt_set_frame_counter(self.h, frame_counter))

    def set_frame_batch(self, frames: int):
        check(_lib.lib().trhip_pt_set_frame_batch(self.h, int(frames)))

    def set_shading_arithmetic(self, ieee: bool):
        check(_lib.lib().trhip_pt_set_shading_arithmetic(self.h, int(bool(ieee))))

    def set_specialization(self, enable: bool):
        check(_lib.lib().trhip_pt_set_specialization(self.h, int(bool(enable))))

    def set_lanes(self, lanes: int):
        check(_lib.lib().trhip_pt_set_lanes(self.h, lanes))

    def set_fused_tonemap(self, display, info):
        check(_lib.lib().trhip_pt_set_fused_tonemap(self.h, None if display is None else _ptr(display), None if info is None else C.byref(info)))

    def lane_pipes(self):
        if not hasattr(_lib.lib(), "trhip_pt_get_lane_pipes"):
            return 0, []
        n = C.c_int32(0)
        cls = (C.c_int32 * 4)()
        check(_lib.lib().trhip_pt_get_lane_pipes(self.h, C.byref(n), cls))
        return n.value, [cls[i] for i in range(n.value)]

    def set_frame_slots(self, slots: int):
        if hasattr(_lib.lib(), "trhip_pt_set_frame_slots"):
            check(_lib.lib().trhip_pt_set_frame_slots(self.h, slots))

    def reset_accumulated_samples(self):
        check(_lib.lib().trhip_pt_reset_accumulation(self.h, 0))

    def reset_sample_counter(self):
        check(_lib.lib().trhip_pt_reset_accumulation(self.h, 1))

    def run(self, color_target, viewports=1, stream=None):
        tw, th = get_distribution_target_size(self.distribution)
        check(_lib.lib().trhip_pt_render(self.h, _ptr(color_target), tw, th, viewports, stream))

    TARGETS = {"color": (4, np.float32), "diffuse": (4, np.float32), "reflection": (4, np.float32), "albedo": (4, np.float32),
               "material": (4, np.float32), "normal": (2, np.float32), "pos": (4, np.float32), "instance_id": (1, np.int32),
               "screen_motion": (2, np.float32)}

    def run_targets(self, targets: dict, viewports=1, stream=None):
        unknown = set(targets) - set(self.TARGETS)
        if unknown:
            raise ValueError(f"unknown gbuffer targets: {sorted(unknown)}")
        t = _lib.PtTargetsC()
        for name, buf in targets.items():
            setattr(t, name, _ptr(buf))
        tw, th = get_distribution_target_size(self.distribution)
        check(_lib.lib().trhip_pt_render_targets(self.h, C.byref(t), tw, th, viewports, stream))

    def set_profiling(self, count_work=False, detailed_timing=False):
        check(_lib.lib().trhip_pt_set_profiling(self.h, int(count_work), int(detailed_timing)))

    def counters(self) -> dict:
        c = CountersC()
        check(_lib.lib().trhip_pt_get_counters(self.h, C.byref(c)))
        return {n: int(getattr(c, n)) for n, _ in CountersC._fields_}

    def reset_counters(self):
        check(_lib.lib().trhip_pt_reset_counters(self.h))

    def light_counters(self) -> dict:
        c = LightCountersC()
        check(_lib.lib().trhip_pt_get_light_counters(self.h, C.byref(c)))
        return {n: int(getattr(c, n)) for n, _ in LightCountersC._fields_}

    def max_stack_depth(self) -> int:
        d = C.c_uint32(0)
        check(_lib.lib().trhip_pt_get_max_stack_depth(self.h, C.byref(d)))
        return int(d.value)

    def set_terminal_query(self, mode: int):
        check(_lib.lib().trhip_pt_set_terminal_query(self.h, mode))

    def terminal_counters(self) -> dict:
        c = TerminalCountersC()
        check(_lib.lib().trhip_pt_get_terminal_counters(self.h, C.byref(c)))
        return {n: int(getattr(c, n)) for n, _ in TerminalCountersC._fields_ if n != "pad"}

    def timings(self) -> dict:
        t = TimingsC()
        check(_lib.lib().trhip_pt_get_timings(self.h, C.byref(t)))
        return {n: float(getattr(t, n)) for n, _ in TimingsC._fields_}

    def program(self) -> dict:
        from ._lib import ProgramInfoC
        p = ProgramInfoC()
        if not hasattr(_lib.lib(), "trhip_pt_get_program"):
            return {"kind": "general", "ieee": False, "identity": 0, "key": "unknown: the library predates trhip_pt_get_program"}
        check(_lib.lib().trhip_pt_get_program(self.h, C.byref(p)))
        return {"kind": ("general", "cli", "compiled")[p.kind], "ieee": bool(p.ieee), "identity": int(p.identity), "key": p.key.decode()}

    def phase_counters(self) -> dict:
        from ._lib import PhaseCountersC
        p = PhaseCountersC()
        check(_lib.lib().trhip_pt_get_phase_counters(self.h, C.byref(p)))
        out = {n: int(getattr(p, n)) for n, _ in PhaseCountersC._fields_ if n != "lane_node_phase_hist"}
        out["lane_node_phase_hist"] = [int(x) for x in p.lane_node_phase_hist]
        return out

    def close(self):
        if self.h:
            _lib.lib().trhip_pt_destroy(self.h)
            self.h = None

    def __del__(self):
        try:
            self.close()
        except Exception:
            pass


class DirectStage(PathTracerStage):
    _create = "trhip_direct_create"


class FeatureStage:

    def __init__(self, ctx: Context, scene_stage: SceneStage, feature: int, distribution: DistributionParams, projection=0,
                 min_ray_dist=1e-4, default_value=(np.nan,) * 4):
        self.ctx, self.ss, self.feature, self.distribution = ctx, scene_stage, feature, distribution
        self.projection, self.min_ray_dist, self.default_value = projection, min_ray_dist, default_value

    def run(self, color_target, viewport=0, stream=None):
        tw, th = get_distribution_target_size(self.distribution)
        d = _dist_c(self.distribution)
        dv = (C.c_float * 4)(*self.default_value)
        check(_lib.lib().trhip_feature_render(self.ctx.h, self.feature, C.byref(d), self.projection, viewport, self.min_ray_dist, dv,
                                              _ptr(color_target), tw, th, stream))


class StitchStage:

    def __init__(self, ctx: Context, size, blend_ratio=1.0):
        self.ctx, self.size, self.blend_ratio = ctx, tuple(size), blend_ratio

    def set_blend_ratio(self, r):
        self.blend_ratio = r

    def run_one(self, partial_dist: DistributionParams, partial, primary, viewports=1, stream=None):
        pw, ph = get_distribution_target_size(partial_dist)
        d = _dist_c(partial_dist)
        check(_lib.lib().trhip_stitch(self.ctx.h, C.byref(d), _ptr(partial), pw, ph, _ptr(primary), viewports, self.blend_ratio, stream))


    def run_all(self, partial_dists, partials, primary, viewports=1, stream=None):
        n = len(partial_dists)
        if n == 0:
            return
        key = tuple((id(p), d.index, d.count, d.strategy) for d, p in zip(partial_dists, partials))
        if getattr(self, "_batch_key", None) != key:
            ds = (DistributionC * n)(*[_dist_c(d) for d in partial_dists])
            ptrs = (C.c_void_p * n)(*[_ptr(p) for p in partials])
            sizes = [get_distribution_target_size(d) for d in partial_dists]
            pws = (C.c_uint32 * n)(*[w for w, _ in sizes])
            phs = (C.c_uint32 * n)(*[h for _, h in sizes])
            self._batch_key, self._batch_args = key, (ds, ptrs, pws, phs)
        ds, ptrs, pws, phs = self._batch_args
        check(_lib.lib().trhip_stitch_batch(self.ctx.h, n, ds, ptrs, pws, phs, _ptr(primary), viewports, self.blend_ratio, stream))


class TonemapStage:
# ... 283 lines not shown

def _sh_grid_data_dict(g) -> dict:
    return dict(transform=np.array(g.transform, dtype=np.float32).reshape(4, 4).T, normal_transform=np.array(g.normal_transform, dtype=np.float32).reshape(4, 4).T,
                grid_size=tuple(g.grid_size), mix_ratio=float(g.mix_ratio), cell_scale=np.array(g.cell_scale, dtype=np.float32),
                rotation_x=float(g.rotation_x), rotation_y=float(g.rotation_y))


def sh_grid_parameters(grid: ShGrid, samples_per_probe: int, frame_counter: int, history_length: int, temporal_ratio: float) -> dict:
    t = np.ascontiguousarray(np.asarray(grid.transform, dtype=np.float64).T, dtype=np.float32).reshape(16)
    sc = np.asarray(grid.scaling, dtype=np.float32).reshape(3)
    res = (C.c_uint32 * 3)(*[int(r) for r in grid.resolution])
    g = _lib.ShGridDataC()
    check(_lib.lib().trhip_sh_pack_grid_data(t.ctypes.data_as(C.POINTER(C.c_float)), sc.ctypes.data_as(C.POINTER(C.c_float)), res, int(samples_per_probe),
                                             int(frame_counter) & 0xFFFFFFFF, int(history_length), float(temporal_ratio), C.byref(g)))
    return _sh_grid_data_dict(g)


class ShPathTracerStage(_PostStage):

    PREFIX, TIMINGS = "sh", _lib.ShTimingsC

    def __init__(self, ctx: Context, scene_stage: Optional[SceneStage], grid: ShGrid, options: Optional[dict] = None):
        self.options = sh_options(**(options or {}))
        self.ctx, self.scene_stage, self.grid = ctx, scene_stage, grid
        o = self.options
        self.order, self.samples = int(o["sh_order"]), int(o["samples_per_probe"])
        self.resolution = tuple(int(r) for r in grid.resolution)
        path = make_options(**{k: o[k] for k in ("max_bounces", "min_ray_dist", "rng_seed", "sampler", "film", "film_radius", "mis_mode",
                                                 "russian_roulette_delta", "indirect_clamping", "regularization_gamma", "nee_point",
                                                 "nee_directional", "nee_envmap", "nee_triangles", "bounce_mode", "tri_light_mode")})
        opt = _lib.ShOptionsC(self.order, (C.c_uint32 * 3)(*[max(r, 0) for r in self.resolution]), max(self.samples, 0), float(o["temporal_ratio"]))
        self._create(getattr(ctx, "h", None), C.byref(path), C.byref(opt))
        self.set_transform(grid.transform, grid.scaling)

    def set_transform(self, transform, scaling):
        t = np.ascontiguousarray(np.asarray(transform, dtype=np.float64).T, dtype=np.float32).reshape(16)
        sc = np.asarray(scaling, dtype=np.float32).reshape(3)
        check(_lib.lib().trhip_sh_set_transform(self.h, t.ctypes.data_as(C.POINTER(C.c_float)), sc.ctypes.data_as(C.POINTER(C.c_float))))

    def set_frame_counter(self, frame_counter: int):
        check(_lib.lib().trhip_sh_set_frame_counter(self.h, frame_counter))

    def reset_history(self):
        check(_lib.lib().trhip_sh_reset_history(self.h))

    def set_lanes(self, lanes: int):
        check(_lib.lib().trhip_sh_set_lanes(self.h, lanes))

    def set_batch_probes(self, probes: int):
        check(_lib.lib().trhip_sh_set_batch_probes(self.h, probes))

    def set_shading_arithmetic(self, ieee: bool):
        check(_lib.lib().trhip_sh_set_shading_arithmetic(self.h, 1 if ieee else 0))

    def grid_data(self) -> dict:
        g = _lib.ShGridDataC()
        check(_lib.lib().trhip_sh_get_grid_data(self.h, C.byref(g)))
        return _sh_grid_data_dict(g)

    def run(self, stream=None):
        check(_lib.lib().trhip_sh_render(self.h, stream))

    @property
    def shape(self):
        rx, ry, rz = self.resolution
        return (rz, ry * sh_coef_count(self.order), rx, 4)

    def download(self, name: str = "grid") -> np.ndarray:
        if name == "grid":
            return self._download(_lib.SH_GRID, self.shape)
        if name == "half":
            return self._download(_lib.SH_GRID_HALF, self.shape, np.float16)
        raise KeyError(name)

    def device_grids(self):
        a, b = C.c_void_p(), C.c_void_p()
        check(_lib.lib().trhip_sh_get_grids(self.h, C.byref(a), C.byref(b)))
        return a.value, b.value

    def counters(self) -> dict:
        c = CountersC()
        check(_lib.lib().trhip_sh_get_counters(self.h, C.byref(c)))
        return {n: getattr(c, n) for n, _ in c._fields_}

    def set_profiling(self, count_work=False, detailed_timing=False):
        check(_lib.lib().trhip_sh_set_profiling(self.h, int(count_work), int(detailed_timing)))

    def reset_counters(self):
        check(_lib.lib().trhip_sh_reset_counters(self.h))


class ShRenderer:

    def __init__(self, ctx: Context, scene_stage: SceneStage, grids, options: Optional[dict] = None):
        if not grids:
            raise ValueError("ShRenderer: the scene has no light-probe grid (TR_data.light_probe of type GRID)")
        self.stages = [ShPathTracerStage(ctx, scene_stage, g, options) for g in grids]

    def render(self, stream=None):
        for st in self.stages:
            st.run(stream)

    def download(self, name: str = "grid"):
        return [st.download(name) for st in self.stages]

    def close(self):
        for st in self.stages:
            st.close()


def dshgi_pick_grid(grids, position) -> int:
    n = len(grids)
    if n == 0:
        return -1
    t = np.ascontiguousarray([np.asarray(g.transform, dtype=np.float64).T for g in grids], dtype=np.float32).reshape(n * 16)
    sc = np.ascontiguousarray([g.scaling for g in grids], dtype=np.float32).reshape(n * 3)
    res = np.ascontiguousarray([g.resolution for g in grids], dtype=np.uint32).reshape(n * 3)
    rad = np.ascontiguousarray([g.radius for g in grids], dtype=np.float32)
    pos = np.ascontiguousarray(position, dtype=np.float32).reshape(3)
    fp, index = C.POINTER(C.c_float), C.c_int32(-1)
    check(_lib.lib().trhip_dshgi_pick_grid(t.ctypes.data_as(fp), sc.ctypes.data_as(fp), res.ctypes.data_as(C.POINTER(C.c_uint32)), rad.ctypes.data_as(fp), n,
                                           pos.ctypes.data_as(fp), C.byref(index)))
    return index.value


def dshgi_instance_grids(grids, instances: np.ndarray) -> np.ndarray:
    return np.array([dshgi_pick_grid(grids, inst["model"][3][:3]) for inst in instances], dtype=np.int32)


def brdf_integration_table(ctx: "Context", size=256, samples=1024, stream=None) -> "DeviceBuffer":
    buf = ctx.alloc(size * size * 8)
    check(_lib.lib().trhip_brdf_integration_generate(ctx.h, size, samples, buf.data_ptr(), stream))
    return buf


def load_brdf_integration(path: str) -> np.ndarray:
    from .exr import load_exr
    img = load_exr(path)
    if img.shape[2] < 2:
        raise ValueError(f"{path}: {img.shape[2]} channel; a BRDF-integration table has R (scale) and G (bias)")
    return np.ascontiguousarray(img[..., :2], dtype=np.float32)


class DshgiStage(_PostStage):

    PREFIX, TIMINGS = "dshgi", _lib.DshgiTimingsC

    def __init__(self, ctx: Context, scene_stage: Optional[SceneStage], size, layers=1, order=2, use_probe_visibility=False, record_surface=False,
                 projection=0, min_ray_dist=1e-4):
        self.ctx, self.scene_stage, self.size, self.layers = ctx, scene_stage, tuple(size), int(layers)
        self.order, self.projection, self.min_ray_dist = int(order), int(projection), float(min_ray_dist)
        opt = _lib.DshgiOptionsC(self.order, int(bool(use_probe_visibility)), int(bool(record_surface)))
        self._create(getattr(ctx, "h", None), C.byref(opt), max(int(self.size[0]), 0), max(int(self.size[1]), 0), max(self.layers, 0))

    def set_grids(self, grids, images):
        n = len(grids)
        arr = (_lib.DshgiGridC * max(n, 1))()
        for g, img, a in zip(grids, images, arr):
            a.grid_half_dev = _ptr(img)
            a.resolution = (C.c_uint32 * 3)(*[int(r) for r in g.resolution])
            a.transform = (C.c_float * 16)(*np.asarray(g.transform, dtype=np.float64).T.astype(np.float32).reshape(16).tolist())
            a.scaling = (C.c_float * 3)(*[float(s) for s in g.scaling])
        check(_lib.lib().trhip_dshgi_set_grids(self.h, arr, n))

    def set_instance_grids(self, instance_grids):
        a = np.ascontiguousarray(instance_grids, dtype=np.int32)
# ... 843 lines not shown
```

Measured before the change: 3955.

## Fuse primary ray generation into first-bounce closest-hit trace kernel

Adds a primary-start mode where the bounce-0 closest-hit kernel generates camera rays itself, storing the path state and tracing straight from registers, so the separate raygen launch and its buffer round-trip go away. It uses a persistent-wave scheme with an atomic work counter, which is why bounce counters must be zeroed up front; the resolve kernel now clears them for the next frame instead of a memset. The mode is auto-enabled for the default CLI shading set with one sample per pass and no two-level scene. It adds extra register pressure to the trace kernel and disables merged raygen when active.

```diff
diff --git a/include/trhip.h b/include/trhip.h
--- a/include/trhip.h
+++ b/include/trhip.h
@@ -227,6 +227,11 @@
 int trhip_pt_set_terminal_query(trhip_pt* pt, int mode);
 typedef struct trhip_terminal_counters { uint64_t blocked_rays, fallback_rays; uint32_t in_effect, emitter_triangles, threshold, pad; } trhip_terminal_counters;
 int trhip_pt_get_terminal_counters(trhip_pt* pt, trhip_terminal_counters* out);
+#define TRHIP_PRIMARY_START_AUTO 0
+#define TRHIP_PRIMARY_START_OFF 1
+int trhip_pt_set_primary_start(trhip_pt* pt, int mode);
+typedef struct trhip_primary_start_info { int32_t mode, in_effect, last_frame, pad; } trhip_primary_start_info;
+int trhip_pt_get_primary_start(trhip_pt* pt, trhip_primary_start_info* out);
 int trhip_calibrate_valu(trhip_device* dev, float* ginst_per_s);
 int trhip_calibrate_l1(trhip_device* dev, float* gaccesses_per_s);
 
@@ -415,6 +420,7 @@
 #define TRHIP_SH_GRID_HALF 1
 int trhip_sh_download(trhip_sh* stage, int which, void* host, size_t bytes);
 int trhip_sh_get_counters(trhip_sh* stage, trhip_counters* out);
+int trhip_sh_get_primary_start(trhip_sh* stage, trhip_primary_start_info* out);
 int trhip_sh_get_timings(trhip_sh* stage, trhip_sh_timings* out);
 int trhip_sh_set_profiling(trhip_sh* stage, int count_work, int detailed_timing);
 int trhip_sh_reset_counters(trhip_sh* stage);
diff --git a/tauray_amd/_lib.py b/tauray_amd/_lib.py
--- a/tauray_amd/_lib.py
+++ b/tauray_amd/_lib.py
@@ -62,6 +62,13 @@
 
 TERMINAL_QUERY_AUTO, TERMINAL_QUERY_OFF = 0, 1
 HIT_BLOCKED = -2
+
+
+PRIMARY_START_AUTO, PRIMARY_START_OFF = 0, 1
+
+
+class PrimaryStartInfoC(C.Structure):
+    _fields_ = [("mode", C.c_int32), ("in_effect", C.c_int32), ("last_frame", C.c_int32), ("pad", C.c_int32)]
 
 
 class PtOptionsC(C.Structure):
@@ -291,6 +298,8 @@
     "trhip_pt_get_light_counters": (_i, [_vp, C.POINTER(LightCountersC)]),
     "trhip_pt_set_terminal_query": (_i, [_vp, _i]),
     "trhip_pt_get_terminal_counters": (_i, [_vp, C.POINTER(TerminalCountersC)]),
+    "trhip_pt_set_primary_start": (_i, [_vp, _i]),
+    "trhip_pt_get_primary_start": (_i, [_vp, C.POINTER(PrimaryStartInfoC)]),
     "trhip_pt_get_max_stack_depth": (_i, [_vp, C.POINTER(C.c_uint32)]),
     "trhip_trace_terminal": (_i, [_vp, _u32, _vp, _vp, _vp, _vp, _vp]),
     "trhip_stitch_batch": (_i, [_vp, _u32, _vp, _vp, _vp, _vp, _vp, _u32, C.c_float, _vp]),
@@ -385,6 +394,7 @@
     "trhip_sh_download": (_i, [_vp, _i, _vp, C.c_size_t]),
     "trhip_sh_get_counters": (_i, [_vp, C.POINTER(CountersC)]),
     "trhip_sh_get_timings": (_i, [_vp, C.POINTER(ShTimingsC)]),
+    "trhip_sh_get_primary_start": (_i, [_vp, C.POINTER(PrimaryStartInfoC)]),
     "trhip_sh_set_profiling": (_i, [_vp, _i, _i]),
     "trhip_sh_reset_counters": (_i, [_vp]),
     "trhip_dshgi_create": (_i, [_vp, C.POINTER(DshgiOptionsC), _u32, _u32, _u32, C.POINTER(_vp)]),
diff --git a/tauray_amd/csrc/api.hip b/tauray_amd/csrc/api.hip
--- a/tauray_amd/csrc/api.hip
+++ b/tauray_amd/csrc/api.hip
@@ -948,6 +948,21 @@
     pt->stage->terminal_query = mode;
     return 0;
 }
+int trhip_pt_set_primary_start(trhip_pt* pt, int mode) {
+    if (!pt) return set_error("null trhip_pt");
+    if (mode != TRHIP_PRIMARY_START_AUTO && mode != TRHIP_PRIMARY_START_OFF)
+        return set_error("trhip_pt_set_primary_start: unknown mode " + std::to_string(mode) + " (0 auto, 1 off)");
+    pt->stage->primary_start = mode;
+    return 0;
+}
+int trhip_pt_get_primary_start(trhip_pt* pt, trhip_primary_start_info* out) {
+    if (!pt) return set_error("null trhip_pt");
+    if (!out) return set_error("trhip_pt_get_primary_start: null output");
+    const int e = pt->stage->primary_start_in_effect();
+    if (e < 0) return set_error("trhip_pt_get_primary_start: TRHIP_PRIMARY_START is not auto or off");
+    out->mode = pt->stage->primary_start; out->in_effect = e; out->last_frame = pt->stage->last_primary_start; out->pad = 0;
+    return 0;
+}
 int trhip_pt_get_terminal_counters(trhip_pt* pt, trhip_terminal_counters* out) {
     if (!pt) return set_error("null trhip_pt");
     if (!out) return set_error("trhip_pt_get_terminal_counters: null output");
diff --git a/tauray_amd/csrc/path_tracer.hip b/tauray_amd/csrc/path_tracer.hip
--- a/tauray_amd/csrc/path_tracer.hip
+++ b/tauray_amd/csrc/path_tracer.hip
@@ -58,6 +58,39 @@
     flush_trace_counters<COUNT>(P, pb, overflow, 1000 + bounce, rays, 0u, st, max_vis);
     TL(__syncthreads(); for (uint i = threadIdx.x; i < (KB / 64) * TL_WORDS; i += KB) if (s_tl[i]) atomicAdd(&g_timeline[i % TL_WORDS], (unsigned long long)s_tl[i]);)
 }
+
+__global__ __launch_bounds__(KB, TR_CLOSEST_WAVES) void k_trace_closest_primary(SceneView sv, PtParams P, PathBuffers pb, uint* bc) {
+    sv.wide_textures = 0;
+    __shared__ int s_stack_rows[TR_STACK_WORDS];
+    int* const s_stack = s_stack_rows + TR_STACK_ROW0;
+    __shared__ int s_owner[(KB / 64) * TR_OWNER_WORDS];
+    const uint n = P.n_ids;
+    TraceStats st = {};
+    uint rays = 0, max_vis = 0;
+    int overflow = 0;
+    const uint wave_id = (blockIdx.x * KB + threadIdx.x) >> 6, n_waves = (gridDim.x * KB) >> 6;
+    bool first = true;
+    while (true) {
+        uint base = 0;
+        if (first) base = wave_id * 64u;
+        else {
+            if (n <= n_waves * 64u) break;
+            if ((threadIdx.x & 63) == 0) base = n_waves * 64u + atomicAdd(&bc[BC_CUR_CLOSEST], 64u);
+            base = __shfl(base, 0);
+        }
+        first = false;
+        if (base >= n) break;
+        const PrimaryRay pr = primary_ray<SpecCli>(sv, pb, base + (threadIdx.x & 63), n);
+        uint tid = threadIdx.x;
+        asm volatile("" : "+v"(tid));
+        const QuadCtx qc = make_quad_ctx_of(s_stack, s_owner, pb, tid);
+        closest_lane<false, false, false, true>(sv, P, pb, 0, nullptr, base + (tid & 63), n, s_stack + tid, qc, st, overflow, max_vis, rays, nullptr, nullptr, nullptr, &pr);
+    }
+    flush_trace_counters<false>(P, pb, overflow, 1000, rays, 0u, st, max_vis);
+}
+static_assert(__is_same(decltype(&k_trace_closest_primary), void (*)(SceneView, PtParams, PathBuffers, uint*)) &&
+              __builtin_offsetof(PrimaryKernArgs, sv) == 0 && __builtin_offsetof(PrimaryKernArgs, P) == kernarg_next(0, sizeof(SceneView), alignof(PtParams)),
+              "PrimaryKernArgs is not the head of k_trace_closest_primary's argument layout");
 
 template <bool COUNT, bool WIDE = true, bool TWO_LEVEL = false>
 __global__ __launch_bounds__(KB, TWO_LEVEL ? TR_SHADOW_WAVES_2L : TR_SHADOW_WAVES) void k_trace_shadow(SceneView sv, PtParams P, PathBuffers pb, uint* bc) {
@@ -487,6 +520,7 @@
     hipStream_t lane_stream[PT_LANES] = {};
     hipEvent_t lane_join[PT_LANES] = {};
     hipEvent_t pass_done[PT_LANES] = {};
+    bool lane_zeroed[PT_LANES] = {};
     hipEvent_t get_event() {
         if (!pool.empty()) { hipEvent_t e = pool.back(); pool.pop_back(); return e; }
         hipEvent_t e; (void)hipEventCreateWithFlags(&e, hipEventDisableSystemFence); return e;
@@ -529,6 +563,7 @@
         HIPCHK(hipMalloc(&pb.counters, PT_LANES * CNT_WORDS * sizeof(uint)));
         HIPCHK(hipMemset(pb.counters, 0, PT_LANES * CNT_WORDS * sizeof(uint)));
         HIPCHK(hipMalloc(&pb.bounce, (size_t)PT_LANES * BC_STRIDE * ((size_t)opt.max_bounces + 2u) * sizeof(uint)));
+        for (bool& z : impl->lane_zeroed) z = false;
     }
     if (!impl->ev_init) { for (auto& e : impl->ev) HIPCHK(hipEventCreateWithFlags(&e, hipEventDisableSystemFence)); impl->ev_init = true; }
     if (n <= impl->capacity && (!lobe_sums || pb.sum_diffuse)) return 0;
@@ -556,10 +591,14 @@
     return 0;
 }
 
+bool PtStage::shades_with_cli_set() const {
+    static const bool cli_instances = !(getenv("TRHIP_SHADE_CLI") && atoi(getenv("TRHIP_SHADE_CLI")) == 0);
+    return cli_instances && !probe_mode && is_cli_default_set(opt) && scene->shade_tris != nullptr && scene->wide_textures == 0;
+}
+
 PtStage::Program PtStage::choose_program() {
-    static const bool cli_instances = !(getenv("TRHIP_SHADE_CLI") && atoi(getenv("TRHIP_SHADE_CLI")) == 0);
     const bool wide = scene->wide_textures != 0;
-    const bool cli_set = cli_instances && !probe_mode && is_cli_default_set(opt) && scene->shade_tris != nullptr && !wide;
+    const bool cli_set = shades_with_cli_set();
     static const bool shade_fast_env = !(getenv("TRHIP_SHADE_FAST") && atoi(getenv("TRHIP_SHADE_FAST")) == 0);
     const bool shade_fast = ieee_shading < 0 ? shade_fast_env : ieee_shading == 0;
     static const bool specialize_env = !(getenv("TRHIP_SPECIALIZE") && atoi(getenv("TRHIP_SPECIALIZE")) == 0);
@@ -658,6 +697,9 @@
     const int tq_in_effect = terminal_query_in_effect();
     if (tq_in_effect < 0) return set_error("trhip_pt_render: TRHIP_TERMINAL_QUERY is not auto or off");
     const bool terminal_query = tq_in_effect != 0;
+    const int ps_in_effect = primary_start_in_effect();
+    if (ps_in_effect < 0) return set_error("trhip_pt_render: TRHIP_PRIMARY_START is not auto or off");
+    const bool primary_start = ps_in_effect != 0;
     const Program prog = choose_program();
     const bool wide = prog.wide, cli_set = prog.cli_set, shade_fast = prog.shade_fast;
     const SpecKernels *spec_shade = prog.shade, *spec_raygen = prog.raygen;
@@ -774,6 +816,18 @@
         else (void)hipGetLastError();
     }
     HIPCHK(hipEventRecord(ev[0], stream));
+    const int bounce_lanes = direct ? 1 : std::min(n_lanes, (int)PT_LANES);
+    if (primary_start) {
+        bool all_zero = true;
+        for (int l = 0; l < bounce_lanes; ++l) all_zero = all_zero && impl->lane_zeroed[l];
+        if (!all_zero) {
+            HIPCHK(hipMemsetAsync(pb.bounce, 0, (size_t)PT_LANES * P.bounce_words * sizeof(uint), stream));
+            for (bool& z : impl->lane_zeroed) z = true;
+        }
+    }
+    bool lane_was_zeroed[PT_LANES];
+    for (int l = 0; l < PT_LANES; ++l) lane_was_zeroed[l] = impl->lane_zeroed[l];
+    for (int l = 0; l < bounce_lanes; ++l) impl->lane_zeroed[l] = false;
     if (direct) {
         if (!pb.sh_cweight) HIPCHK(hipMalloc(&pb.sh_cweight, impl->capacity * 16));
         PtParams LP = P;
@@ -809,6 +863,7 @@
         }
         HIPCHK(hipEventRecord(ev[1], stream));
         HIPCHK(hipGetLastError());
+        last_primary_start = 0;
         timing_pending = true;
         impl->frames++;
         frame_counter++;
@@ -871,7 +926,7 @@
             for (int s = 0; s < opt.samples_per_pass; ++s) {
                 LP.sample_in_pass = (uint)s;
                 LP.rng_sample = shard_sample_base + shard_sample_stride * (LP.previous_samples + LP.sample_in_pass);
-                if ((only == -2 || only == -1) && !merged_raygen) timed(T_RAYGEN, ls, [&] {
+                if ((only == -2 || only == -1) && !merged_raygen && !primary_start) timed(T_RAYGEN, ls, [&] {
                     launch_raygen(blocks_all, ls, LP, lb);
                 });
                 for (int bounce = 0; bounce < opt.max_bounces; ++bounce) {
@@ -884,6 +939,8 @@
                         hipLaunchKernelGGL((wide ? k_trace_fused_terminal<true> : k_trace_fused_terminal<false>), dim3(blocks_f), dim3(KB), 0, ls, sv, LP, lb, bounce, q, bc, bc - BC_STRIDE, qn);
                     } else if (fused && bounce > 0) {
                         hipLaunchKernelGGL((two_level ? k_trace_fused<true, true> : (wide ? k_trace_fused<true> : k_trace_fused<false>)), dim3(blocks_f), dim3(KB), 0, ls, sv, LP, lb, bounce, q, bc, bc - BC_STRIDE);
+                    } else if (primary_start && bounce == 0) {
+                        hipLaunchKernelGGL(k_trace_closest_primary, dim3(std::min(blocks_all, closest_cap)), dim3(KB), 0, ls, sv, LP, lb, bc);
                     } else {
                         timed(T_CLOSEST, ls, [&] {
                             if (tq) {
@@ -942,7 +999,7 @@
     static const char* order_env = getenv("TRHIP_ENQUEUE");
     const bool interleave = order_env ? strcmp(order_env, "lanes") != 0 : (impl->prev_frame_ms > 0.0f && impl->prev_frame_ms < 3.0f);
     static const bool merged_raygen_enabled = !(getenv("TRHIP_MERGED_RAYGEN") && atoi(getenv("TRHIP_MERGED_RAYGEN")) == 0);
-    merged_raygen = merged_raygen_enabled && interleave && !sample_lanes && lanes_used > 1 && lanes_used == n_lanes && passes == 1 &&
+    merged_raygen = merged_raygen_enabled && !primary_start && interleave && !sample_lanes && lanes_used > 1 && lanes_used == n_lanes && passes == 1 &&
                                opt.samples_per_pass == 1;
     if (merged_raygen) {
         PtParams RP = lane_ctx[0].LP;
@@ -985,6 +1042,8 @@
     }
     HIPCHK(hipEventRecord(ev[1], stream));
     HIPCHK(hipGetLastError());
+    for (int l = 0; l < bounce_lanes; ++l) impl->lane_zeroed[l] = l < lanes_used ? !probe : lane_was_zeroed[l];
+    last_primary_start = primary_start ? 1 : 0;
     timing_pending = true;
     impl->frames++;
     frame_counter += frame_batch;
@@ -1070,6 +1129,22 @@
             scene->sphere_light_count() == 0) ? 1 : 0;
 }
 
+int PtStage::primary_start_in_effect() const {
+    int mode = primary_start;
+    if (mode < 0) {
+        const char* e = getenv("TRHIP_PRIMARY_START");
+        std::string v = e ? e : "";
+        for (char& c : v) c = (char)tolower((unsigned char)c);
+        if (v.empty() || v == "auto") mode = TRHIP_PRIMARY_START_AUTO;
+        else if (v == "off") mode = TRHIP_PRIMARY_START_OFF;
+        else return -1;
+    }
+    if (mode != TRHIP_PRIMARY_START_AUTO) return 0;
+    return (!direct && !probe_mode && count_work == 0 && detailed_timing == 0 && opt.samples_per_pass == 1 && shades_with_cli_set() &&
+            !scene->two_level) ? 1 : 0;
+}
+
+
 int PtStage::get_terminal_counters(trhip_terminal_counters* out, hipStream_t stream) {
     memset(out, 0, sizeof(*out));
     out->in_effect = terminal_query_in_effect() > 0 ? 1u : 0u;
diff --git a/tauray_amd/csrc/pt.h b/tauray_amd/csrc/pt.h
--- a/tauray_amd/csrc/pt.h
+++ b/tauray_amd/csrc/pt.h
@@ -38,6 +38,8 @@
     int get_terminal_counters(trhip_terminal_counters* out, hipStream_t stream);
     int get_program(trhip_program_info* out);
     int terminal_query_in_effect() const;
+    int primary_start_in_effect() const;
+    bool shades_with_cli_set() const;
 
     DeviceScene* scene;
     trhip_pt_options opt;
@@ -56,6 +58,8 @@
     int ieee_shading = -1;
     int specialize = -1;
     int terminal_query = -1;
+    int primary_start = -1;
+    int last_primary_start = -1;
     bool direct = false;
     bool probe_mode = false;
     const ShProbeBatch* probes = nullptr;
diff --git a/tauray_amd/csrc/resolve_kernel.h b/tauray_amd/csrc/resolve_kernel.h
--- a/tauray_amd/csrc/resolve_kernel.h
+++ b/tauray_amd/csrc/resolve_kernel.h
@@ -67,6 +67,7 @@
     if (i < P.n_ids) accumulate_sample_path(P, pb, i + P.id_offset);
 }
 __global__ __launch_bounds__(KB) void k_resolve(PtParams P, PathBuffers pb) {
+    if (blockIdx.x == 0) for (uint k = threadIdx.x; k < P.bounce_words; k += KB) pb.bounce[k] = 0;
     const uint i = blockIdx.x * KB + threadIdx.x;
     if (i < P.n_ids) resolve_path(P, pb, i + P.id_offset);
 }
diff --git a/tauray_amd/csrc/sh_probes.hip b/tauray_amd/csrc/sh_probes.hip
--- a/tauray_amd/csrc/sh_probes.hip
+++ b/tauray_amd/csrc/sh_probes.hip
@@ -352,6 +352,14 @@
     return s->pt->get_counters(out, s->last_stream);
 }
 
+int trhip_sh_get_primary_start(trhip_sh* s, trhip_primary_start_info* out) {
+    if (!s || !out) return set_error("trhip_sh_get_primary_start: null argument");
+    const int e = s->pt->primary_start_in_effect();
+    if (e < 0) return set_error("trhip_sh_get_primary_start: TRHIP_PRIMARY_START is not auto or off");
+    out->mode = s->pt->primary_start; out->in_effect = e; out->last_frame = s->pt->last_primary_start; out->pad = 0;
+    return 0;
+}
+
 int trhip_sh_set_profiling(trhip_sh* s, int count_work, int detailed_timing) {
     if (!s) return set_error("trhip_sh_set_profiling: null stage");
     s->pt->count_work = count_work; s->pt->detailed_timing = detailed_timing;
diff --git a/tauray_amd/csrc/shade_kernel.h b/tauray_amd/csrc/shade_kernel.h
--- a/tauray_amd/csrc/shade_kernel.h
+++ b/tauray_amd/csrc/shade_kernel.h
@@ -185,6 +185,46 @@
     }
 };
 #endif
+struct PathStart {
+    bool valid;
+    f3 origin, dir;
+    u4 rng;
+    uint seed;
+    uint sobol_index;
+};
+TR_DEV PathStart path_start(const SceneView& sv, const PtParams& P, uint i) {
+    PathStart s;
+    s.origin = F3(0); s.dir = F3(0); s.rng = u4{0, 0, 0, 0}; s.seed = 0; s.sobol_index = 0;
+    uint lx, ly, lz;
+    launch_coord(P.L, i, lx, ly, lz);
+    int px, py;
+    s.valid = get_pixel_pos(P.L, lx, ly, px, py);
+    if (!s.valid) return s;
+    LocalSampler ls = init_local_sampler(u4{(uint)px, (uint)py, global_viewport(P, lz), P.rng_sample}, sample_counter_of(P, lz),
+                                         P.rng_seed, P.opt.sampler);
+    f2 cam_offset = F2(0.0f);
+    if (P.opt.film != 0) {
+        f4 r = u4_to_unit(pcg4d(ls.rs));
+        if (P.opt.film == 1) cam_offset = F2(r.x, r.y) * 2.0f - 1.0f;
+        else cam_offset = sample_blackman_harris_concentric_disk(F2(r.x, r.y)) * 2.0f;
+        cam_offset = cam_offset * (2.0f * P.opt.film_radius);
+    }
+    f2 dof_u = F2(0.5f);
+    if (P.opt.depth_of_field) { f4 r = u4_to_unit(pcg4d(ls.rs)); dof_u = F2(r.x, r.y); }
+    get_screen_camera_ray(P.L, px, py, sv.cameras[global_viewport(P, lz)], P.opt.projection, P.opt.depth_of_field != 0, cam_offset, dof_u, s.origin, s.dir);
+    s.seed = pcg4d(ls.rs).x;
+    s.sobol_index = ls.sobol_index;
+    s.rng = ls.rs;
+    return s;
+}
+TR_DEV void store_path_start(const PathBuffers& pb, uint i, const PathStart& s) {
+    pb.misc[i] = u4{s.seed, s.sobol_index, i, s.valid ? 0u : 1u};
+    if (!s.valid) return;
+    pb.org_pdf[i] = F4(s.origin, 0.0f);
+    pb.dir_reg[i] = F4(s.dir, 1.0f);
+    pb.atten_alpha[i] = F4(1, 1, 1, 1);
+    pb.rng[i] = s.rng;
+}
 struct ShadeOut {
     bool alive = false;
     bool want_shadow = false;
@@ -449,36 +489,11 @@
     uint i = blockIdx.x * KB + threadIdx.x;
     if (i >= P.n_ids) return;
     i += P.id_offset;
-    uint lx, ly, lz;
-    launch_coord(P.L, i, lx, ly, lz);
-    int px, py;
-    bool valid = get_pixel_pos(P.L, lx, ly, px, py);
-    u4 misc = {0, 0, i, valid ? 0u : 1u};
     if (P.sample_in_pass == 0 && !P.fused_resolve) {
         pb.sum_color[i] = F4(0, 0, 0, 1);
         if (pb.sum_diffuse) { pb.sum_diffuse[i] = F4(0); pb.sum_reflection[i] = F4(0); }
     }
-    if (!valid) { pb.misc[i] = misc; return; }
-    LocalSampler ls = init_local_sampler(u4{(uint)px, (uint)py, global_viewport(P, lz), P.rng_sample}, sample_counter_of(P, lz),
-                                         P.rng_seed, P.opt.sampler);
-    f2 cam_offset = F2(0.0f);
-    if (P.opt.film != 0) {
-        f4 r = u4_to_unit(pcg4d(ls.rs));
-        if (P.opt.film == 1) cam_offset = F2(r.x, r.y) * 2.0f - 1.0f;
-        else cam_offset = sample_blackman_harris_concentric_disk(F2(r.x, r.y)) * 2.0f;
-        cam_offset = cam_offset * (2.0f * P.opt.film_radius);
-    }
-    f2 dof_u = F2(0.5f);
-    if (P.opt.depth_of_field) { f4 r = u4_to_unit(pcg4d(ls.rs)); dof_u = F2(r.x, r.y); }
-    f3 origin, dir;
-    get_screen_camera_ray(P.L, px, py, sv.cameras[global_viewport(P, lz)], P.opt.projection, P.opt.depth_of_field != 0, cam_offset, dof_u, origin, dir);
-    misc.x = pcg4d(ls.rs).x;
-    misc.y = ls.sobol_index;
-    pb.org_pdf[i] = F4(origin, 0.0f);
-    pb.dir_reg[i] = F4(dir, 1.0f);
-    pb.atten_alpha[i] = F4(1, 1, 1, 1);
-    pb.rng[i] = ls.rs;
-    pb.misc[i] = misc;
+    store_path_start(pb, i, path_start(sv, P, i));
 }
 template <typename S = SpecGeneral>
 __global__ __launch_bounds__(KB) void k_raygen(SceneView sv, PtParams P, PathBuffers pb) { raygen_paths<S>(sv, P, pb); }
diff --git a/tauray_amd/csrc/trace_lanes.h b/tauray_amd/csrc/trace_lanes.h
--- a/tauray_amd/csrc/trace_lanes.h
+++ b/tauray_amd/csrc/trace_lanes.h
@@ -2,16 +2,35 @@
 #include "trace.h"
 #include "trace_quad.h"
 #include "pt_state.h"
+#include "shade_kernel.h"
 
 namespace tr {
 
 namespace {
 
 struct TerminalCounts { uint blocked, fallback; };
-template <bool COUNT, bool TWO_LEVEL = false, bool TERMINAL = false>
+struct PrimaryKernArgs { SceneView sv; PtParams P; };
+struct PrimaryRay { bool valid; uint id, seed; f3 origin, dir; };
+template <typename S>
+TR_DEV PrimaryRay primary_ray(const SceneView& sv, const PathBuffers& pb, uint qi, uint n) {
+    PrimaryRay r = {false, 0u, 0u, F3(0), F3(0)};
+    if (qi >= n) return r;
+    typedef const PrimaryKernArgs __attribute__((address_space(4)))* KernArgPtr;
+    KernArgPtr ka = (KernArgPtr)__builtin_amdgcn_kernarg_segment_ptr();
+    asm volatile("" : "+s"(ka));
+    PtParams P;
+    load_kernarg(P, &ka->P);
+    S::pin(P);
+    r.id = qi + P.id_offset;
+    const PathStart s = path_start(sv, P, r.id);
+    store_path_start(pb, r.id, s);
+    r.valid = s.valid; r.seed = s.seed; r.origin = s.origin; r.dir = s.dir;
+    return r;
+}
+template <bool COUNT, bool TWO_LEVEL = false, bool TERMINAL = false, bool PRIMARY = false>
 TR_DEV void closest_lane(const SceneView& sv, const PtParams& P, const PathBuffers& pb, int bounce, const uint* queue, uint qi, uint n, int* lds_stack,
                          const QuadCtx& qc, TraceStats& st, int& overflow, uint& max_vis, uint& rays, uint* next_queue = nullptr, uint* next_count = nullptr,
-                         TerminalCounts* tc = nullptr) {
+                         TerminalCounts* tc = nullptr, const PrimaryRay* pr = nullptr) {
     bool valid = qi < n;
     uint id = 0;
     u4 misc = {0, 0, 0, 1};
@@ -38,6 +57,8 @@
         return;
     }
     TL(const unsigned long long tl_chunk = tl_now();)
+    if constexpr (PRIMARY) { valid = pr->valid; id = pr->id; misc.x = pr->seed; o = F4(pr->origin, 0.0f); d = F4(pr->dir, 1.0f); }
+    else
     if (valid) { id = queue ? queue[qi] : qi + P.id_offset; misc = pb.misc[id]; o = pb.org_pdf[id]; d = pb.dir_reg[id]; valid = !(misc.w & 1u); }
     TL(tl_data_arrived(); tl_misc(qc.tl, 3, tl_now() - tl_chunk);)
     for (int b = 0; b < bounce; ++b) pcg(misc.x);
@@ -76,6 +97,15 @@
     TL(tl_misc(qc.tl, 5, tl_now() - tl_chunk);)
 }
 
+TR_DEV QuadCtx make_quad_ctx_of(int* s_stack, int* s_owner, const PathBuffers& pb, uint tid) {
+    QuadCtx qc;
+    TL(qc.tl = nullptr;)
+    const uint wave = tid >> 6;
+    qc.wave_stack = s_stack + (tid & ~63u);
+    qc.owner_tab = s_owner + wave * TR_OWNER_WORDS;
+    qc.spill = pb.qspill + ((size_t)blockIdx.x * (KB / 64) + wave) * (16u * TR_QSPILL);
+    return qc;
+}
 TR_DEV QuadCtx make_quad_ctx(int* s_stack, int* s_owner, const PathBuffers& pb TL(, uint* s_tl = nullptr)) {
     QuadCtx qc;
     TL(qc.tl = s_tl ? s_tl + (threadIdx.x >> 6) * TL_WORDS : nullptr;)
diff --git a/tauray_amd/renderer.py b/tauray_amd/renderer.py
--- a/tauray_amd/renderer.py
+++ b/tauray_amd/renderer.py
@@ -527,6 +527,14 @@
         check(_lib.lib().trhip_pt_get_terminal_counters(self.h, C.byref(c)))
         return {n: int(getattr(c, n)) for n, _ in TerminalCountersC._fields_ if n != "pad"}
 
+    def set_primary_start(self, mode: int):
+        check(_lib.lib().trhip_pt_set_primary_start(self.h, mode))
+
+    def primary_start(self) -> dict:
+        p = _lib.PrimaryStartInfoC()
+        check(_lib.lib().trhip_pt_get_primary_start(self.h, C.byref(p)))
+        return {"mode": int(p.mode), "in_effect": bool(p.in_effect), "last_frame": int(p.last_frame)}
+
     def timings(self) -> dict:
         t = TimingsC()
         check(_lib.lib().trhip_pt_get_timings(self.h, C.byref(t)))
@@ -976,6 +984,11 @@
         c = CountersC()
         check(_lib.lib().trhip_sh_get_counters(self.h, C.byref(c)))
         return {n: getattr(c, n) for n, _ in c._fields_}
+
+    def primary_start(self) -> dict:
+        p = _lib.PrimaryStartInfoC()
+        check(_lib.lib().trhip_sh_get_primary_start(self.h, C.byref(p)))
+        return {"mode": int(p.mode), "in_effect": bool(p.in_effect), "last_frame": int(p.last_frame)}
 
     def set_profiling(self, count_work=False, detailed_timing=False):
         check(_lib.lib().trhip_sh_set_profiling(self.h, int(count_work), int(detailed_timing)))
```

Result: faster. 4076, median of 6 (+3.0%).
